# nktoan/h-edit

Hardware: AMD Instinct MI355X
Metric: edited images/sec (512^2, 50 steps, K Langevin) (higher is better)
Workload: dtype bf16

## Files before the change

h-edit_amd/csrc/c_api.hip:

```cpp
#include "../../include/hedit.h"
#include <exception>
#include <map>
#include <mutex>
#include <new>
#include <set>
#include <utility>

#include "common.h"
#include "kernels.h"

static thread_local std::string g_last_error;
void hedit_set_error(const std::string& msg) { g_last_error = msg; }

int hedit_abi_catch() noexcept {
  try {
    try {
      throw;
    } catch (const std::bad_alloc&) {
      g_last_error = "out of host memory inside libhedit_hip";
    } catch (const std::exception& e) {
      g_last_error = std::string("C++ exception inside libhedit_hip: ") + e.what();
    } catch (...) {
      g_last_error = "unknown C++ exception inside libhedit_hip";
    }
// ... 133 lines not shown
int hedit_k_gemm_plan_splits(int M, int N, int K, int chunk_kt) { return gemm_plan_splits(M, N, K, chunk_kt); }

int hedit_k_gemm(const void* A, const void* W, const float* bias, const void* residual, void* C, int M, int N,
                 int K, int lda, int ldc, int ldr, int mode, int Hin, int Win, int Cin, int Hout, int Wout,
                 int splits, void* partial_ws, void* stream) try {
  ARG_CHECK(A && W && C, "gemm args");
  GemmParams p{};
  p.A = reinterpret_cast<const bf16_t*>(A);
  p.W = reinterpret_cast<const bf16_t*>(W);
  p.M = M; p.N = N; p.K = K; p.lda = lda; p.mode = mode;
  p.Hin = Hin; p.Win = Win; p.Cin = Cin; p.Hout = Hout; p.Wout = Wout;
  p.bias = bias;
  p.residual = reinterpret_cast<const bf16_t*>(residual);
  p.ldr = ldr;
  p.C = reinterpret_cast<bf16_t*>(C);
  p.ldc = ldc;
  if (splits < 0) {
    const int kt = K / 64;
    const int s = gemm_pick_splits(M, N, K, -splits);
    p.chunk_kt = (kt + s - 1) / s;
    return gemm_launch(p, 1, nullptr, S(stream));
  }
  const int s = gemm_pick_splits(M, N, K, splits);
  return gemm_launch(p, s, reinterpret_cast<float*>(partial_ws), S(stream));
} catch (...) { return hedit_abi_catch(); }

int hedit_k_conv_gn(const void* A, const void* W, const float* bias, const void* residual, void* C, int M, int N, int K, int ldc,
                    int ldr, int mode, int Hin, int Win, int Cin, int Hout, int Wout, int splits, void* partial_ws, float* gn_part,
                    void* stream) try {
  ARG_CHECK(A && W && C && gn_part, "conv_gn args");
  GemmParams p{};
  p.A = reinterpret_cast<const bf16_t*>(A);
  p.W = reinterpret_cast<const bf16_t*>(W);
  p.M = M; p.N = N; p.K = K; p.lda = Cin; p.mode = mode;
  p.Hin = Hin; p.Win = Win; p.Cin = Cin; p.Hout = Hout; p.Wout = Wout;
  p.bias = bias;
  p.residual = reinterpret_cast<const bf16_t*>(residual);
  p.ldr = ldr;
  p.C = reinterpret_cast<bf16_t*>(C);
  p.ldc = ldc;
  p.gn_part = gn_part;
  if (splits < 0) {
    const int kt = K / 64;
    const int s = gemm_pick_splits(M, N, K, -splits);
    p.chunk_kt = (kt + s - 1) / s;
    return gemm_launch(p, 1, nullptr, S(stream));
  }
  const int s = gemm_pick_splits(M, N, K, splits);
  return gemm_launch(p, s, reinterpret_cast<float*>(partial_ws), S(stream));
} catch (...) { return hedit_abi_catch(); }

int hedit_k_groupnorm_from_parts(const void* x, void* y, const float* gamma, const float* beta, int B, int HW, int C, int G,
                                 float eps, int silu, const float* part_a, int ca, const float* part_b, int cb, void* ws,
                                 void* stream) try {
  ARG_CHECK(x && y && gamma && beta && part_a && ws, "groupnorm_from_parts args");
  return groupnorm_from_parts_launch(reinterpret_cast<const bf16_t*>(x), reinterpret_cast<bf16_t*>(y), gamma, beta, B, HW, C, G,
                                     eps, silu, part_a, ca, part_b, cb, reinterpret_cast<float*>(ws), S(stream));
} catch (...) { return hedit_abi_catch(); }

int hedit_k_pack_geglu(const float* w, const float* bias, void* w_packed_bf16, float* bias_packed, int inner, int K,
                       void* stream) try {
  ARG_CHECK(w && w_packed_bf16, "pack_geglu args");
  int rc = pack_geglu_rows_launch(w, reinterpret_cast<bf16_t*>(w_packed_bf16), nullptr, 2 * inner, K, S(stream));
  if (rc != HEDIT_OK || !bias) return rc;
  ARG_CHECK(bias_packed, "pack_geglu: bias_packed");
  return pack_geglu_rows_launch(bias, nullptr, bias_packed, 2 * inner, 1, S(stream));
} catch (...) { return hedit_abi_catch(); }

int hedit_k_gemm_geglu(const void* A, const void* w_packed, const float* bias_packed, void* C, int M, int inner, int K,
                       int lda, int ldc, void* stream) try {
  ARG_CHECK(A && w_packed && C, "gemm_geglu args");
  GemmParams p{};
  p.A = reinterpret_cast<const bf16_t*>(A);
  p.W = reinterpret_cast<const bf16_t*>(w_packed);
  p.M = M; p.N = 2 * inner; p.K = K; p.lda = lda; p.mode = 0;
  p.bias = bias_packed;
  p.C = reinterpret_cast<bf16_t*>(C);
  p.ldc = ldc;
  p.geglu = 1;
  return gemm_launch(p, 1, nullptr, S(stream));
} catch (...) { return hedit_abi_catch(); }

int hedit_k_ffn_channels(void) { return ffn_fused_channels(); }
size_t hedit_k_ffn_stream_bytes(int with_outer_layers) { return ffn_stream_bytes(with_outer_layers, with_outer_layers); }
size_t hedit_k_ffn_bias_bytes(void) { return ffn_bias_bytes(); }

int hedit_k_ffn_pack(const float* w1, const float* b1, const float* w2, const float* w_pre, const float* w_post, void* stream_out,
                     float* bias1_out, void* stream) try {
  ARG_CHECK(w1 && b1 && w2 && stream_out && bias1_out && ((w_pre == nullptr) == (w_post == nullptr)), "ffn_pack args");
  const int outer = w_pre != nullptr;
  bf16_t* so = reinterpret_cast<bf16_t*>(stream_out);
  int rc = ffn_pack_launch(w1, 1, outer, outer, so, S(stream));
  if (rc == HEDIT_OK) rc = ffn_pack_launch(w2, 2, outer, outer, so, S(stream));
  if (rc == HEDIT_OK && outer) rc = ffn_pack_launch(w_pre, 0, 1, 1, so, S(stream));
  if (rc == HEDIT_OK && outer) rc = ffn_pack_launch(w_post, 3, 1, 1, so, S(stream));
  if (rc != HEDIT_OK) return rc;
  return ffn_pack_bias_launch(b1, bias1_out, S(stream));
} catch (...) { return hedit_abi_catch(); }

int hedit_k_ffn_fused(const void* x, int64_t ldx, const float* gamma, const float* beta, float eps, const void* w_stream,
                      const float* bias1_packed, const float* bias2, void* out, int64_t ldo, int M, int C, void* stream) try {
  FfnParams f{};
  f.x = reinterpret_cast<const bf16_t*>(x); f.ldx = (long)ldx; f.gamma = gamma; f.beta = beta; f.eps = eps;
  f.stream = reinterpret_cast<const bf16_t*>(w_stream); f.bias1p = bias1_packed; f.bias2 = bias2;
  f.out = reinterpret_cast<bf16_t*>(out); f.ldo = (long)ldo; f.M = M; f.C = C;
  return ffn_fused_launch(f, S(stream));
} catch (...) { return hedit_abi_catch(); }

int hedit_k_ffn_chain(const void* a, int64_t lda, const void* t1, int64_t ldt1, const void* x, int64_t ldx, const float* bias_pre,
                      const float* gamma, const float* beta, float eps, const void* w_stream, const float* bias1_packed, const float* bias2,
                      const float* bias_post, void* out, int64_t ldo, int M, int C, void* stream) try {
  ARG_CHECK(a && t1 && x, "ffn_chain args");
  FfnParams f{};
  f.a = reinterpret_cast<const bf16_t*>(a); f.lda = (long)lda;
  f.x = reinterpret_cast<const bf16_t*>(t1); f.ldx = (long)ldt1;
  f.r2 = reinterpret_cast<const bf16_t*>(x); f.ldr2 = (long)ldx;
  f.bias_pre = bias_pre; f.bias_post = bias_post;
  f.gamma = gamma; f.beta = beta; f.eps = eps;
  f.stream = reinterpret_cast<const bf16_t*>(w_stream); f.bias1p = bias1_packed; f.bias2 = bias2;
  f.out = reinterpret_cast<bf16_t*>(out); f.ldo = (long)ldo; f.M = M; f.C = C;
  return ffn_fused_launch(f, S(stream));
} catch (...) { return hedit_abi_catch(); }

size_t hedit_k_lin_chain_stream_bytes(int n_out) { return lin_chain_stream_bytes(n_out == 3 ? 4 : 2); }

int hedit_k_lin_chain_pack(const float* w_pre, const float* w0, const float* w1, const float* w2, float scale0, void* stream_out,
                           void* stream) try {
  ARG_CHECK(w_pre && w0 && stream_out && ((w1 == nullptr) == (w2 == nullptr)), "lin_chain_pack args");
  const int layers = w1 ? 4 : 2;
  bf16_t* so = reinterpret_cast<bf16_t*>(stream_out);
  int rc = lin_chain_pack_launch(w_pre, 0, 1.f, layers, so, S(stream));
  if (rc == HEDIT_OK) rc = lin_chain_pack_launch(w0, 1, scale0, layers, so, S(stream));
  if (rc == HEDIT_OK && w1) rc = lin_chain_pack_launch(w1, 2, 1.f, layers, so, S(stream));
  if (rc == HEDIT_OK && w1) rc = lin_chain_pack_launch(w2, 3, 1.f, layers, so, S(stream));
  return rc;
} catch (...) { return hedit_abi_catch(); }

int hedit_k_lin_chain(const void* a, int64_t lda, const void* r1, int64_t ldr1, const float* gn_ss, int rows_per_image,
                      const float* bias_pre, const float* gamma, const float* beta, float eps, const void* w_stream, void* out_mid,
                      int64_t ldmid, void* out_q, int64_t ldq, void* out_k, int64_t ldk, void* out, int64_t ldo, int M, int C,
                      void* stream) try {
  LinChainParams c{};
  c.a = reinterpret_cast<const bf16_t*>(a); c.lda = (long)lda; c.r1 = reinterpret_cast<const bf16_t*>(r1); c.ldr1 = (long)ldr1;
  c.bias_pre = bias_pre; c.gamma = gamma; c.beta = beta; c.eps = eps; c.stream = reinterpret_cast<const bf16_t*>(w_stream);
  c.out_mid = reinterpret_cast<bf16_t*>(out_mid); c.ldmid = (long)ldmid; c.out = reinterpret_cast<bf16_t*>(out); c.ldo = (long)ldo;
  c.M = M; c.C = C; c.gn_ss = gn_ss; c.rows_per_image = rows_per_image;
  c.out_q = reinterpret_cast<bf16_t*>(out_q); c.ldq = (long)ldq; c.out_k = reinterpret_cast<bf16_t*>(out_k); c.ldk = (long)ldk;
  return lin_chain_launch(c, S(stream));
} catch (...) { return hedit_abi_catch(); }

int hedit_storage_is_f16(void) { return HEDIT_F16; }

int hedit_test_set_flags(int flags) try {
  ARG_CHECK(flags >= 0 && flags <= 15, "hedit_test_set_flags: bit 0 drained ring waits, bit 1 exact self-attention pass, bit 2 pixel-UNet GroupNorm statistics path flipped, bit 3 no persistent linear kernel");
  g_test_flags.store(flags, std::memory_order_relaxed);
  return HEDIT_OK;
} catch (...) { return hedit_abi_catch(); }

int hedit_k_lin_chain_sched(const void* a, int64_t lda, const void* r1, int64_t ldr1, const float* gn_ss, int rows_per_image,
                            const float* bias_pre, const float* gamma, const float* beta, float eps, const void* w_stream, void* out_mid,
                            int64_t ldmid, void* out_q, int64_t ldq, void* out_k, int64_t ldk, void* out, int64_t ldo, int M, int C,
                            int sched, void* stream) try {
  LinChainParams c{};
  c.a = reinterpret_cast<const bf16_t*>(a); c.lda = (long)lda; c.r1 = reinterpret_cast<const bf16_t*>(r1); c.ldr1 = (long)ldr1;
  c.bias_pre = bias_pre; c.gamma = gamma; c.beta = beta; c.eps = eps; c.stream = reinterpret_cast<const bf16_t*>(w_stream);
  c.out_mid = reinterpret_cast<bf16_t*>(out_mid); c.ldmid = (long)ldmid; c.out = reinterpret_cast<bf16_t*>(out); c.ldo = (long)ldo;
  c.M = M; c.C = C; c.gn_ss = gn_ss; c.rows_per_image = rows_per_image;
  c.out_q = reinterpret_cast<bf16_t*>(out_q); c.ldq = (long)ldq; c.out_k = reinterpret_cast<bf16_t*>(out_k); c.ldk = (long)ldk;
  return lin_chain_launch_sched(c, sched, S(stream));
} catch (...) { return hedit_abi_catch(); }

size_t hedit_k_groupnorm_ws_bytes(int B, int HW, int C) { return groupnorm_ws_bytes(B, HW, C); }

int hedit_k_groupnorm_affine(const void* x, const float* gamma, const float* beta, int B, int HW, int C, int G, float eps, void* ws,
                             float* ss_out, void* stream) try {
  ARG_CHECK(x && gamma && beta && ws && ss_out, "groupnorm_affine args");
  const float* ss = nullptr;
  int rc = groupnorm_affine_launch(reinterpret_cast<const bf16_t*>(x), gamma, beta, B, HW, C, G, eps, reinterpret_cast<float*>(ws), S(stream), &ss);
  if (rc != HEDIT_OK) return rc;
  HIP_TRY(hipMemcpyAsync(ss_out, ss, (size_t)B * C * 2 * sizeof(float), hipMemcpyDeviceToDevice, S(stream)));
  return HEDIT_OK;
} catch (...) { return hedit_abi_catch(); }

int hedit_k_groupnorm(const void* x, void* y, const float* gamma, const float* beta, int B, int HW, int C, int G,
                      float eps, int silu, void* ws, void* stream) try {
  ARG_CHECK(x && y && gamma && beta && ws, "groupnorm args");
  return groupnorm_launch(reinterpret_cast<const bf16_t*>(x), reinterpret_cast<bf16_t*>(y), gamma, beta, B, HW, C, G,
                          eps, silu, reinterpret_cast<float*>(ws), S(stream));
} catch (...) { return hedit_abi_catch(); }

int hedit_k_layernorm(const void* x, void* y, const float* gamma, const float* beta, int64_t rows, int C, float eps,
                      void* stream) try {
  ARG_CHECK(x && y && gamma && beta, "layernorm args");
  return layernorm_launch(reinterpret_cast<const bf16_t*>(x), reinterpret_cast<bf16_t*>(y), gamma, beta, (long)rows, C, eps, S(stream));
} catch (...) { return hedit_abi_catch(); }

int hedit_k_geglu(const void* x, void* y, int64_t rows, int inner, void* stream) try {
  ARG_CHECK(x && y, "geglu args");
  return geglu_launch(reinterpret_cast<const bf16_t*>(x), reinterpret_cast<bf16_t*>(y), (long)rows, inner, S(stream));
} catch (...) { return hedit_abi_catch(); }

int hedit_k_self_attn(const void* q, int ldq, const void* k, int ldk, const void* vt, int64_t ldvt, void* out, int ldo,
                      int B, int N, int heads, int d, const int32_t* qk_src, const int32_t* kv_src, void* stream) try {
  ARG_CHECK(q && k && vt && out, "self_attn args");
  SelfAttnParams p{};
  p.q = reinterpret_cast<const bf16_t*>(q); p.ldq = ldq;
  p.k = reinterpret_cast<const bf16_t*>(k); p.ldk = ldk;
  p.vt = reinterpret_cast<const bf16_t*>(vt); p.ldvt = (long)ldvt;
  p.out = reinterpret_cast<bf16_t*>(out); p.ldo = ldo;
  p.B = B; p.N = N; p.heads = heads; p.d = d; p.qk_src = qk_src; p.kv_src = kv_src;
  return self_attn_launch(p, S(stream));
} catch (...) { return hedit_abi_catch(); }

int hedit_k_cross_attn(const void* q, int ldq, const void* k, int ldk, const void* vt, int64_t ldvt, void* out, int ldo,
                       int B, int N, int heads, int d, const hedit_p2p_plan* plan, float* store, void* stream) try {
  ARG_CHECK(q && k && vt && out && plan, "cross_attn args");
  CrossAttnParams p{};
  p.q = reinterpret_cast<const bf16_t*>(q); p.ldq = ldq;
  p.k = reinterpret_cast<const bf16_t*>(k); p.ldk = ldk;
  p.vt = reinterpret_cast<const bf16_t*>(vt); p.ldvt = (long)ldvt;
  p.out = reinterpret_cast<bf16_t*>(out); p.ldo = ldo;
  p.B = B; p.N = N; p.heads = heads; p.d = d;
  p.n_pairs = plan->n_pairs; p.pair_src = plan->pair_src; p.pair_tar = plan->pair_tar;
  p.mixT = reinterpret_cast<const bf16_t*>(plan->mixT); p.bvec = plan->bvec;
  p.singles = plan->singles; p.n_single = plan->n_single;
  p.store = store;
  return cross_attn_launch(p, S(stream));
} catch (...) { return hedit_abi_catch(); }

int hedit_k_attn_probs(const void* q, int ldq, const void* k, int ldk, float* probs, int B, int N, int M, int kstride,
                       int heads, int d, void* stream) try {
  ARG_CHECK(q && k && probs, "attn_probs args");
  AttnProbsParams p{};
  p.q = reinterpret_cast<const bf16_t*>(q); p.ldq = ldq;
  p.k = reinterpret_cast<const bf16_t*>(k); p.ldk = ldk;
  p.probs = probs; p.B = B; p.N = N; p.M = M; p.kstride = kstride; p.heads = heads; p.d = d;
  return attn_probs_launch(p, S(stream));
} catch (...) { return hedit_abi_catch(); }

int hedit_k_attn_apply(const float* probs, const void* vt, int64_t ldvt, void* out, int ldo, int B, int N, int M,
                       int kstride, int heads, int d, void* stream) try {
  ARG_CHECK(probs && vt && out, "attn_apply args");
  AttnProbsParams p{};
  p.probs = const_cast<float*>(probs);
  p.vt = reinterpret_cast<const bf16_t*>(vt); p.ldvt = (long)ldvt;
  p.out = reinterpret_cast<bf16_t*>(out); p.ldo = ldo;
  p.B = B; p.N = N; p.M = M; p.kstride = kstride; p.heads = heads; p.d = d;
  return attn_apply_launch(p, S(stream));
} catch (...) { return hedit_abi_catch(); }

int hedit_k_pack_conv3x3(const float* w, void* out, int O, int I, void* stream) try {
  ARG_CHECK(w && out, "pack args");
  return pack_conv3x3_launch(w, reinterpret_cast<bf16_t*>(out), O, I, S(stream));
} catch (...) { return hedit_abi_catch(); }

int hedit_k_f32_to_bf16(const float* x, void* y, int64_t n, void* stream) try {
  ARG_CHECK(x && y, "cast args");
  return f32_to_bf16_launch(x, reinterpret_cast<bf16_t*>(y), (long)n, S(stream));
} catch (...) { return hedit_abi_catch(); }

int hedit_k_groupnorm_stats(const void* x, void* y, const float* gamma, const float* beta, int B, int HW, int C, int G,
                            float eps, int silu, void* ws, float* stats, void* stream) try {
  ARG_CHECK(x && y && gamma && beta && ws && stats, "groupnorm_stats args");
  return groupnorm_launch(reinterpret_cast<const bf16_t*>(x), reinterpret_cast<bf16_t*>(y), gamma, beta, B, HW, C, G,
                          eps, silu, reinterpret_cast<float*>(ws), S(stream), stats);
} catch (...) { return hedit_abi_catch(); }

size_t hedit_k_groupnorm_bwd_ws_bytes(int B, int HW, int C) { return groupnorm_bwd_ws_bytes(B, HW, C); }

int hedit_k_groupnorm_bwd(const void* x, const void* dy, const void* add, void* dx, const float* gamma, const float* beta,
                          const float* stats, int B, int HW, int C, int G, int silu, void* ws, void* stream) try {
  ARG_CHECK(x && dy && dx && gamma && beta && stats && ws, "groupnorm_bwd args");
  return groupnorm_bwd_launch(reinterpret_cast<const bf16_t*>(x), reinterpret_cast<const bf16_t*>(dy),
                              reinterpret_cast<const bf16_t*>(add), reinterpret_cast<bf16_t*>(dx), gamma, beta, stats, B, HW, C,
                              G, silu, reinterpret_cast<float*>(ws), S(stream));
} catch (...) { return hedit_abi_catch(); }

int hedit_k_softmax_rows(const float* s, void* p, int64_t rows, int N, float scale, void* stream) try {
  ARG_CHECK(s && p, "softmax_rows args");
  return softmax_rows_launch(s, reinterpret_cast<bf16_t*>(p), (long)rows, N, scale, S(stream));
} catch (...) { return hedit_abi_catch(); }

int hedit_k_softmax_blockdiag(const float* s, void* p, int64_t rows, int T, int ld, float scale, void* stream) try {
  ARG_CHECK(s && p, "softmax_blockdiag args");
  return softmax_blockdiag_launch(s, reinterpret_cast<bf16_t*>(p), (long)rows, T, ld, scale, S(stream));
} catch (...) { return hedit_abi_catch(); }

int hedit_k_softmax_bwd(const void* p, const float* dp, void* ds, int64_t rows, int N, float scale, void* stream) try {
  ARG_CHECK(p && dp && ds, "softmax_bwd args");
  return softmax_bwd_launch(reinterpret_cast<const bf16_t*>(p), dp, reinterpret_cast<bf16_t*>(ds), (long)rows, N, scale, S(stream));
} catch (...) { return hedit_abi_catch(); }

int hedit_k_transpose(const void* src, void* dst, int R, int C, void* stream) try {
  ARG_CHECK(src && dst, "transpose args");
  return transpose_bf16_launch(reinterpret_cast<const bf16_t*>(src), reinterpret_cast<bf16_t*>(dst), R, C, S(stream));
} catch (...) { return hedit_abi_catch(); }

int hedit_k_sum2x2(const void* du, void* dx, int B, int H, int W, int C, void* stream) try {
  ARG_CHECK(du && dx, "sum2x2 args");
  return sum2x2_launch(reinterpret_cast<const bf16_t*>(du), reinterpret_cast<bf16_t*>(dx), B, H, W, C, S(stream));
} catch (...) { return hedit_abi_catch(); }

int hedit_k_pack_conv3x3_dgrad(const float* w, void* out, int O, int I, void* stream) try {
  ARG_CHECK(w && out, "pack args");
  return pack_conv3x3_dgrad_launch(w, reinterpret_cast<bf16_t*>(out), O, I, S(stream));
} catch (...) { return hedit_abi_catch(); }

// ... 110 lines not shown
```

h-edit_amd/csrc/norm.hip:

```cpp
#include <stdlib.h>
#include "common.h"
#include "kernels.h"

namespace {


constexpr int GN_MAXV = 2;

__global__ __launch_bounds__(256) void gn_partial_kernel(const bf16_t* __restrict__ x, float* __restrict__ part,
                                                         int HW, int C, int G, int nslab) {
  extern __shared__ float lds[];
  const int CV = C / 8;
  const int slab = blockIdx.x, b = blockIdx.y;
  const int pix_per = (HW + nslab - 1) / nslab;
  const int p0 = slab * pix_per;
  int p1 = p0 + pix_per;
  if (p1 > HW) p1 = HW;
  const int R = CV <= 256 ? 256 / CV : 1;
  const int r = CV <= 256 ? threadIdx.x / CV : 0;
  const int cv0 = CV <= 256 ? threadIdx.x % CV : threadIdx.x;
  const bool active = r < R;
  float s[GN_MAXV][8], q[GN_MAXV][8];
#pragma unroll
  for (int v = 0; v < GN_MAXV; ++v)
// ... 407 lines not shown

__global__ __launch_bounds__(256) void pack_conv3x3_kernel(const float* __restrict__ w, bf16_t* __restrict__ out, int O, int I) {
  const long total = (long)O * 9 * I;
  for (long idx = (long)blockIdx.x * 256 + threadIdx.x; idx < total; idx += (long)gridDim.x * 256) {
    const int i = (int)(idx % I);
    const long t = idx / I;
    const int tap = (int)(t % 9);
    const int o = (int)(t / 9);
    out[idx] = f32_to_bf16(w[((long)o * I + i) * 9 + tap]);
  }
}

__global__ __launch_bounds__(256) void pack_geglu_rows_kernel(const float* __restrict__ w, bf16_t* __restrict__ ob, float* __restrict__ of,
                                                              int rows, int K) {
  const long total = (long)rows * K;
  const int half = rows / 2;
  for (long idx = (long)blockIdx.x * 256 + threadIdx.x; idx < total; idx += (long)gridDim.x * 256) {
    const int k = (int)(idx % K);
    const int r = (int)(idx / K);
    const int t = r >> 5, u = r & 31;
    const int src = u < 16 ? t * 16 + u : half + t * 16 + (u - 16);
    const float v = w[(long)src * K + k];
    if (ob) ob[idx] = f32_to_bf16(v);
    if (of) of[idx] = v;
  }
}

__global__ __launch_bounds__(256) void gemv_kernel(const bf16_t* __restrict__ W, const float* __restrict__ x, const float* __restrict__ b0,
                                                   const float* __restrict__ b1, float* __restrict__ out, int N, int K, int silu) {
  const int lane = threadIdx.x & 63;
  const int n = blockIdx.x * 4 + (threadIdx.x >> 6);
  if (n >= N) return;
  float acc = 0.f;
  for (int k = lane * 8; k < K; k += 512) {
    uint4 u = *reinterpret_cast<const uint4*>(W + (long)n * K + k);
    float w[8];
    unpack8(u, w);
#pragma unroll
    for (int j = 0; j < 8; ++j) {
      float xv = x[k + j];
      if (silu) xv = silu_f(xv);
      acc += w[j] * xv;
    }
  }
  acc = wave_sum(acc);
  if (lane == 0) out[n] = acc + (b0 ? b0[n] : 0.f) + (b1 ? b1[n] : 0.f);
}

__global__ void timestep_embed_kernel(float t, float* out, int dim) {
  const int half = dim / 2;
  for (int i = threadIdx.x; i < half; i += blockDim.x) {
    const float fr = expf(-9.210340371976184f * (float)i / (float)half);
    const float a = t * fr;
    out[i] = cosf(a);
    out[half + i] = sinf(a);
  }
}

__global__ void timestep_embed_ddpm_kernel(float t, float* out, int dim) {
  const int half = dim / 2;
  for (int i = threadIdx.x; i < half; i += blockDim.x) {
    const float fr = expf(-9.210340371976184f / (float)(half - 1) * (float)i);
    const float a = t * fr;
    out[i] = sinf(a);
    out[half + i] = cosf(a);
  }
  if ((dim & 1) && threadIdx.x == 0) out[dim - 1] = 0.f;
}

constexpr int CI_PIX = 128;
__global__ __launch_bounds__(256) void conv_in_kernel(const float* __restrict__ x, const float* __restrict__ w, const float* __restrict__ bias,
                                                      bf16_t* __restrict__ y, int B, int Cin, int H, int Wd, int Cout) {
  extern __shared__ float lds[];
  const int K = Cin * 9;
  float* sw = lds;
  float* sx = lds + (long)K * Cout;
  for (int i = threadIdx.x; i < K * Cout; i += 256) {
    const int co = i / K, k = i - co * K;
    sw[k * Cout + co] = w[i];
  }
  const long pix0 = (long)blockIdx.x * CI_PIX;
  const long npix = (long)B * H * Wd;
  for (int i = threadIdx.x; i < CI_PIX * K; i += 256) {
    const int k = i / CI_PIX, pl = i - k * CI_PIX;
    const long pix = pix0 + pl;
    float v = 0.f;
    if (pix < npix) {
      const int ox = (int)(pix % Wd), oy = (int)((pix / Wd) % H), b = (int)(pix / ((long)Wd * H));
      const int ci = k / 9, tap = k - ci * 9;
      const int iy = oy + tap / 3 - 1, ix = ox + tap % 3 - 1;
      if ((unsigned)iy < (unsigned)H && (unsigned)ix < (unsigned)Wd) v = x[(((long)b * Cin + ci) * H + iy) * Wd + ix];
    }
    sx[k * CI_PIX + pl] = v;
  }
  __syncthreads();
  const int CV = Cout / 8;
  for (int i = threadIdx.x; i < (CI_PIX / 4) * CV; i += 256) {
    const int pg = i / CV, cv = i - pg * CV;
    float acc[4][8];
#pragma unroll
    for (int q = 0; q < 4; ++q)
#pragma unroll
      for (int j = 0; j < 8; ++j) acc[q][j] = bias[cv * 8 + j];
    for (int k = 0; k < K; ++k) {
      const float4 xv = *reinterpret_cast<const float4*>(sx + k * CI_PIX + pg * 4);
      const float4 w0 = *reinterpret_cast<const float4*>(sw + k * Cout + cv * 8);
      const float4 w1 = *reinterpret_cast<const float4*>(sw + k * Cout + cv * 8 + 4);
      const float xq[4] = {xv.x, xv.y, xv.z, xv.w};
#pragma unroll
      for (int q = 0; q < 4; ++q) {
        acc[q][0] += xq[q] * w0.x; acc[q][1] += xq[q] * w0.y; acc[q][2] += xq[q] * w0.z; acc[q][3] += xq[q] * w0.w;
        acc[q][4] += xq[q] * w1.x; acc[q][5] += xq[q] * w1.y; acc[q][6] += xq[q] * w1.z; acc[q][7] += xq[q] * w1.w;
      }
    }
#pragma unroll
    for (int q = 0; q < 4; ++q) {
      const long pix = pix0 + pg * 4 + q;
      if (pix < npix) *reinterpret_cast<uint4*>(y + pix * Cout + cv * 8) = pack8(acc[q]);
    }
  }
}

__global__ __launch_bounds__(256) void conv_out_kernel(const bf16_t* __restrict__ x, const bf16_t* __restrict__ w, const float* __restrict__ bias,
                                                       float* __restrict__ y, int B, int H, int Wd, int C, int Cout) {
  const int lane = threadIdx.x & 63;
  const long pix = (long)blockIdx.x * 4 + (threadIdx.x >> 6);
  if (pix >= (long)B * H * Wd) return;
  const int ox = (int)(pix % Wd);
  const int oy = (int)((pix / Wd) % H);
  const int b = (int)(pix / ((long)Wd * H));
  const int CV = C / 8;
  float acc[4] = {0.f, 0.f, 0.f, 0.f};
  for (int idx = lane; idx < 9 * CV; idx += 64) {
    const int tap = idx / CV, cv = idx - tap * CV;
    const int iy = oy + tap / 3 - 1, ix = ox + tap % 3 - 1;
    if ((unsigned)iy >= (unsigned)H || (unsigned)ix >= (unsigned)Wd) continue;
    uint4 u = *reinterpret_cast<const uint4*>(x + (((long)b * H + iy) * Wd + ix) * C + cv * 8);
    float f[8];
    unpack8(u, f);
    for (int co = 0; co < Cout; ++co) {
      uint4 uw = *reinterpret_cast<const uint4*>(w + ((long)co * 9 + tap) * C + cv * 8);
      float ww[8];
      unpack8(uw, ww);
#pragma unroll
      for (int j = 0; j < 8; ++j) acc[co] += f[j] * ww[j];
    }
  }
  for (int co = 0; co < Cout; ++co) {
    float v = wave_sum(acc[co]);
    if (lane == 0) y[(((long)b * Cout + co) * H + oy) * Wd + ox] = v + bias[co];
  }
}

__global__ __launch_bounds__(256) void gn_small_kernel(const bf16_t* __restrict__ x, bf16_t* __restrict__ y,
                                                       const float* __restrict__ gamma, const float* __restrict__ beta,
                                                       int HW, int C, int G, float eps, int silu, float* __restrict__ stats) {
  extern __shared__ uint32_t gs_pairs[];
  __shared__ float red[8];
  const int g = blockIdx.x, b = blockIdx.y, tid = threadIdx.x;
  const int cpg = C / G, ppp = cpg / 2;
  const int npair = HW * ppp;
  const uint32_t* xin = reinterpret_cast<const uint32_t*>(x + (long)b * HW * C + g * cpg);
  float s = 0.f, q = 0.f;
  for (int i = tid; i < npair; i += 256) {
    const int pix = i / ppp, j = i - pix * ppp;
    const uint32_t u = xin[(long)pix * (C / 2) + j];
    gs_pairs[i] = u;
    const float a = st_lo(u), c = st_hi(u);
    s += a; s += c;
    q += a * a; q += c * c;
  }
  s = wave_sum(s);
  q = wave_sum(q);
  if ((tid & 63) == 0) { red[(tid >> 6) * 2] = s; red[(tid >> 6) * 2 + 1] = q; }
  __syncthreads();
  s = ((red[0] + red[2]) + red[4]) + red[6];
  q = ((red[1] + red[3]) + red[5]) + red[7];
  const float n = (float)HW * (float)cpg;
  const float m = s / n;
  float var = q / n - m * m;
  var = var < 0.f ? 0.f : var;
  const float rstd = rsqrtf(var + eps);
  if (stats && tid == 0) *reinterpret_cast<float2*>(stats + ((long)b * G + g) * 2) = make_float2(m, rstd);
  uint32_t* yout = reinterpret_cast<uint32_t*>(y + (long)b * HW * C + g * cpg);
  for (int i = tid; i < npair; i += 256) {
    const int pix = i / ppp, j = i - pix * ppp;
    const uint32_t u = gs_pairs[i];
    const int c0 = g * cpg + 2 * j;
    const float sc0 = rstd * gamma[c0], sc1 = rstd * gamma[c0 + 1];
    float a = st_lo(u) * sc0 + (beta[c0] - m * sc0);
    float c = st_hi(u) * sc1 + (beta[c0 + 1] - m * sc1);
    if (silu) { a = silu_f(a); c = silu_f(c); }
    yout[(long)pix * (C / 2) + j] = pack_bf16x2(a, c);
  }
}

__global__ __launch_bounds__(256) void gn_fold_kernel(const float* __restrict__ pa, int npa, const float* __restrict__ pb, int npb,
                                                      float* __restrict__ out, int units, int ppg) {
  __shared__ float red[8];
  const int g = blockIdx.x, b = blockIdx.y, tid = threadIdx.x;
  const int total = units * ppg;
  float s = 0.f, q = 0.f;
  for (int e = tid; e < total; e += 256) {
    const int u = e / ppg, j = e - u * ppg;
    const int pr = g * ppg + j;
    const long row = (long)b * units + u;
    const float2 v = pr < npa ? *reinterpret_cast<const float2*>(pa + (row * npa + pr) * 2)
                              : *reinterpret_cast<const float2*>(pb + (row * npb + (pr - npa)) * 2);
    s += v.x;
    q += v.y;
  }
  s = wave_sum(s);
  q = wave_sum(q);
  if ((tid & 63) == 0) { red[(tid >> 6) * 2] = s; red[(tid >> 6) * 2 + 1] = q; }
  __syncthreads();
  if (tid == 0) {
    s = ((red[0] + red[2]) + red[4]) + red[6];
    q = ((red[1] + red[3]) + red[5]) + red[7];
    *reinterpret_cast<float2*>(out + ((long)b * gridDim.x + g) * 2) = make_float2(s, q);
  }
}

int gn_nslab(int B, int HW, int C) {
  (void)B;
  const int CV = C / 8;
  const int R = CV <= 256 ? 256 / CV : 1;
  int n = HW / (R * 8);
  int cap = HW / 256;
  cap = cap < 32 ? 32 : (cap > 64 ? 64 : cap);
  if (HW >= 512 * 512) cap = 128;
  if (n > cap) n = cap;
  if (n < 1) n = 1;
  return n;
}

}

size_t groupnorm_ws_bytes(int B, int HW, int C) {
  const int nslab = gn_nslab(B, HW, C);
  return ((size_t)B * nslab * 64 * 2 + (size_t)B * C * 2) * sizeof(float);
}

int groupnorm_launch(const bf16_t* x, bf16_t* y, const float* gamma, const float* beta, int B, int HW,
                     int C, int G, float eps, int silu, float* ws, hipStream_t st, float* stats) {
  ARG_CHECK(C % 8 == 0 && C % G == 0 && G <= 64, "groupnorm: C % 8, C % G, G <= 64");
  ARG_CHECK(C / 8 <= 256 * GN_MAXV, "groupnorm: C too large");
  if (HW < 1024 && (C / G) % 2 == 0 && (size_t)HW * (C / G) * 2 <= 60 * 1024) {
    hipLaunchKernelGGL(gn_small_kernel, dim3(G, B), dim3(256), (size_t)HW * (C / G) * 2, st, x, y, gamma, beta, HW, C, G, eps, silu, stats);
    LAUNCH_CHECK();
    return HEDIT_OK;
  }
  const int nslab = gn_nslab(B, HW, C);
  float* part = ws;
  float* ss = ws + (size_t)B * nslab * 64 * 2;
  const int CV = C / 8;
  const int R = CV <= 256 ? 256 / CV : 1;
  const size_t lds = (size_t)R * C * 2 * sizeof(float);
  ARG_CHECK(lds <= 64 * 1024, "groupnorm: LDS");
  hipLaunchKernelGGL(gn_partial_kernel, dim3(nslab, B), dim3(256), lds, st, x, part, HW, C, G, nslab);
  LAUNCH_CHECK();
  const long total_v = (long)B * HW * CV;
  const bool rows_form = CV <= 256 && HW >= 1024;
  if (!rows_form || stats) {
    hipLaunchKernelGGL(gn_finalize_kernel, dim3(B), dim3(256), 0, st, part, gamma, beta, ss, HW, C, G, nslab, eps, stats);
    LAUNCH_CHECK();
  }
  if (rows_form) {
    int ns = (int)(4096 / (B > 0 ? B : 1)) + 1;
    const int max_ns = HW / (R * 8) > 0 ? HW / (R * 8) : 1;
    if (ns > max_ns) ns = max_ns;
    {
      int pix = HW / ns / (4 * R) * (4 * R);
      if (pix < 4 * R) pix = 4 * R;
      ns = (HW + pix - 1) / pix;
    }
    hipLaunchKernelGGL(gn_apply_rows_kernel, dim3(ns, B), dim3(256), 0, st, x, y, part, gamma, beta, HW, C, G, nslab, eps, silu, ns);
    LAUNCH_CHECK();
    return HEDIT_OK;
  }
  hipLaunchKernelGGL(gn_apply_kernel, dim3(ew_grid(total_v)), dim3(256), 0, st, x, y, ss, total_v, HW, C, silu);
  LAUNCH_CHECK();
  return HEDIT_OK;
}

bool groupnorm_from_parts_supported(int HW, int C, int G) {
  return HW >= 1024 && HW % 128 == 0 && C % 8 == 0 && C / 8 <= 256 && C % G == 0 && (C / G) % 2 == 0 && G <= 64;
}
size_t groupnorm_from_parts_ws_bytes(int B) { return (size_t)B * 64 * 2 * sizeof(float); }

int groupnorm_from_parts_launch(const bf16_t* x, bf16_t* y, const float* gamma, const float* beta, int B, int HW, int C, int G,
                                float eps, int silu, const float* part_a, int ca, const float* part_b, int cb, float* ws,
                                hipStream_t st) {
  ARG_CHECK(groupnorm_from_parts_supported(HW, C, G), "groupnorm_from_parts: shape");
  ARG_CHECK(part_a && ca > 0 && ca % 2 == 0 && cb >= 0 && cb % 2 == 0 && ca + cb == C && (cb == 0) == (part_b == nullptr),
            "groupnorm_from_parts: the pair statistics must cover the C channels");
  hipLaunchKernelGGL(gn_fold_kernel, dim3(G, B), dim3(256), 0, st, part_a, ca / 2, part_b, cb / 2, ws, HW / 128, C / G / 2);
  LAUNCH_CHECK();
  const int CV = C / 8, R = 256 / CV;
  int ns = (int)(4096 / (B > 0 ? B : 1)) + 1;
  const int max_ns = HW / (R * 8) > 0 ? HW / (R * 8) : 1;
  if (ns > max_ns) ns = max_ns;
  int pix = HW / ns / (4 * R) * (4 * R);
  if (pix < 4 * R) pix = 4 * R;
  ns = (HW + pix - 1) / pix;
  hipLaunchKernelGGL(gn_apply_rows_kernel, dim3(ns, B), dim3(256), 0, st, x, y, ws, gamma, beta, HW, C, G, 1, eps, silu, ns);
  LAUNCH_CHECK();
  return HEDIT_OK;
}

int groupnorm_affine_launch(const bf16_t* x, const float* gamma, const float* beta, int B, int HW, int C, int G, float eps,
                            float* ws, hipStream_t st, const float** ss_out) {
  ARG_CHECK(C % 8 == 0 && C % G == 0 && G <= 64, "groupnorm: C % 8, C % G, G <= 64");
  ARG_CHECK(C / 8 <= 256 * GN_MAXV, "groupnorm: C too large");
  const int nslab = gn_nslab(B, HW, C);
  float* part = ws;
  float* ss = ws + (size_t)B * nslab * 64 * 2;
  const int CV = C / 8;
  const int R = CV <= 256 ? 256 / CV : 1;
  const size_t lds = (size_t)R * C * 2 * sizeof(float);
  ARG_CHECK(lds <= 64 * 1024, "groupnorm: LDS");
  hipLaunchKernelGGL(gn_partial_kernel, dim3(nslab, B), dim3(256), lds, st, x, part, HW, C, G, nslab);
  LAUNCH_CHECK();
  hipLaunchKernelGGL(gn_finalize_kernel, dim3(B), dim3(256), 0, st, part, gamma, beta, ss, HW, C, G, nslab, eps, (float*)nullptr);
  LAUNCH_CHECK();
  *ss_out = ss;
  return HEDIT_OK;
}

static int ln_narrow_lanes(int C) {
  if (C % 64 == 0 && C / 64 <= LNN_MAXV) return 8;
  if (C % 128 == 0 && C / 128 <= LNN_MAXV) return 16;
  if (C % 256 == 0 && C / 256 <= LNN_MAXV) return 32;
  return 0;
}

bool splitk_reduce_ln_supported(int C) { return C % 8 == 0 && ln_narrow_lanes(C) != 0; }

int splitk_reduce_ln_launch(const float* partial, int splits, const float* bias, const bf16_t* residual, int ldr, bf16_t* out,
                            bf16_t* y, const float* gamma, const float* beta, long rows, int C, float eps, hipStream_t st) {
  const int lanes = ln_narrow_lanes(C);
  ARG_CHECK(lanes != 0 && splits >= 1, "splitk_reduce_ln: unsupported row width");
  const LnReduce rd{partial, splits, bias, residual, ldr};
  if (lanes == 8) hipLaunchKernelGGL((layernorm_narrow_kernel<8, true>), dim3(cdiv(rows, 32)), dim3(256), 0, st, out, y, gamma, beta, rows, C, eps, rd);
  else if (lanes == 16) hipLaunchKernelGGL((layernorm_narrow_kernel<16, true>), dim3(cdiv(rows, 16)), dim3(256), 0, st, out, y, gamma, beta, rows, C, eps, rd);
  else hipLaunchKernelGGL((layernorm_narrow_kernel<32, true>), dim3(cdiv(rows, 8)), dim3(256), 0, st, out, y, gamma, beta, rows, C, eps, rd);
  LAUNCH_CHECK();
  return HEDIT_OK;
}

int layernorm_launch(const bf16_t* x, bf16_t* y, const float* gamma, const float* beta, long rows, int C,
                     float eps, hipStream_t st) {
  ARG_CHECK(C % 8 == 0 && C / 8 <= 64 * LN_MAXV, "layernorm: C");
  const LnReduce none{};
  bf16_t* xx = const_cast<bf16_t*>(x);
  switch (ln_narrow_lanes(C)) {
    case 8:
      hipLaunchKernelGGL((layernorm_narrow_kernel<8, false>), dim3(cdiv(rows, 32)), dim3(256), 0, st, xx, y, gamma, beta, rows, C, eps, none);
      LAUNCH_CHECK();
      return HEDIT_OK;
    case 16:
      hipLaunchKernelGGL((layernorm_narrow_kernel<16, false>), dim3(cdiv(rows, 16)), dim3(256), 0, st, xx, y, gamma, beta, rows, C, eps, none);
      LAUNCH_CHECK();
      return HEDIT_OK;
    case 32:
      hipLaunchKernelGGL((layernorm_narrow_kernel<32, false>), dim3(cdiv(rows, 8)), dim3(256), 0, st, xx, y, gamma, beta, rows, C, eps, none);
      LAUNCH_CHECK();
      return HEDIT_OK;
    default: break;
  }
  hipLaunchKernelGGL(layernorm_kernel, dim3(cdiv(rows, 4)), dim3(256), 0, st, x, y, gamma, beta, rows, C, eps);
  LAUNCH_CHECK();
  return HEDIT_OK;
}

int geglu_launch(const bf16_t* x, bf16_t* y, long rows, int inner, hipStream_t st) {
  ARG_CHECK(inner % 8 == 0, "geglu: inner % 8");
  hipLaunchKernelGGL(geglu_kernel, dim3(ew_grid(rows * (inner / 8))), dim3(256), 0, st, x, y, rows, inner);
  LAUNCH_CHECK();
  return HEDIT_OK;
}

int concat_launch(const bf16_t* a, int ca, const bf16_t* b, int cb, bf16_t* y, long rows, hipStream_t st, const RowMap* b_map,
                  int rows_per_image) {
  ARG_CHECK(ca % 8 == 0 && cb % 8 == 0, "concat: channels % 8");
  if (b_map) {
    ARG_CHECK(rows_per_image > 0 && rows % rows_per_image == 0 && rows / rows_per_image <= HEDIT_ROWMAP_MAX, "concat: row map");
    hipLaunchKernelGGL(concat_mapped_kernel, dim3(ew_grid(rows * (((a ? ca : 0) + cb) / 8))), dim3(256), 0, st, a, ca, b, cb, y, rows,
                       rows_per_image, *b_map);
    LAUNCH_CHECK();
    return HEDIT_OK;
  }
  if (a == nullptr) {
    hipLaunchKernelGGL(concat_right_kernel, dim3(ew_grid(rows * (cb / 8))), dim3(256), 0, st, b, ca, cb, y, rows);
    LAUNCH_CHECK();
    return HEDIT_OK;
  }
  hipLaunchKernelGGL(concat_kernel, dim3(ew_grid(rows * ((ca + cb) / 8))), dim3(256), 0, st, a, ca, b, cb, y, rows);
  LAUNCH_CHECK();
  return HEDIT_OK;
}

// ... 241 lines not shown
```

h-edit_amd/csrc/unet.hip:

```cpp
#include <array>
#include <map>
#include <string>
#include <vector>

#include "exec.h"
#include "kernels.h"
#include "store.h"

namespace {

struct Res {
  int cin, cout, temb_off;
  float *n1g, *n1b, *n2g, *n2b, *conv2_b, *sc_b;
  bf16_t *conv1, *conv2, *sc_w;
  bf16_t *conv1_t = nullptr, *conv2_t = nullptr, *sc_t = nullptr;
};

struct Attn {
  int C;
  float *gn_g, *gn_b, *pin_b, *ln1g, *ln1b, *ln2g, *ln2b, *ln3g, *ln3b, *o1_b, *o2_b, *ff1_b, *ff2_b, *pout_b;
  bf16_t *pin, *w_qk, *w_v1, *w_o1, *w_q2, *w_k2, *w_v2, *w_o2, *ff1, *ff2, *pout;
  bf16_t *frs = nullptr, *k1s = nullptr, *ffs = nullptr;
  float* ff1_bp = nullptr;
  int ctx_off = 0;
// ... 425 lines not shown
      f.store_self_idx++;
    }
  }
  f.ar.free(qk);
  f.ar.free(vt);
  TRY(aalloc(f, &t1, M * C));
  TRY(aalloc(f, &q2, M * C));
  if (chain) {
    LinChainParams lc{};
    lc.a = ao; lc.lda = C; lc.r1 = t0; lc.ldr1 = C; lc.bias_pre = a.o1_b;
    lc.gamma = a.ln2g; lc.beta = a.ln2b; lc.eps = 1e-5f; lc.stream = a.k1s;
    lc.out_mid = t1; lc.ldmid = C; lc.out = q2; lc.ldo = C; lc.M = (int)M; lc.C = C;
    ProfScope ps(f, PK_LINEAR, 2.0 * M * 2.0 * C * C, 8.0 * M * C + 4.0 * C * C);
    chain_prof(f, ps, M, C, 2, 130);
    RUN(f, lin_chain_launch(lc, f.st));
  } else {
    TRY(aalloc(f, &tn, M * C));
    TRY(linear_ln(f, ao, (int)M, C, a.w_o1, C, a.o1_b, t0, t1, a.ln2g, a.ln2b, 1e-5f, tn));
    TRY(linear(f, tn, (int)M, C, a.w_q2, C, nullptr, nullptr, q2, C));
    f.ar.free(tn);
  }
  f.ar.free(ao);
  f.ar.free(t0);
  *t1_out = t1;
  *q2_out = q2;
  return HEDIT_OK;
}

int transformer_rest(Fwd& f, const Attn& a, const bf16_t* x, bf16_t* t1, bf16_t* q2, int H, int W, bf16_t** out,
                     bf16_t* dst = nullptr, int ldd = 0) {
  const int C = a.C, N = H * W, B = f.B, heads = f.h->cfg.heads, d = C / heads;
  const size_t M = (size_t)B * N;
  const hedit_p2p_plan* pl = (f.plan && f.plan->mode > 0) ? f.plan : nullptr;
  bf16_t *tn, *ao, *k2, *vt2, *t2, *gf, *t3, *y;
  const bool chain = a.ffs != nullptr;
  const int MC = B * HEDIT_CTXP;
  k2 = const_cast<bf16_t*>(f.k2_all) + a.ctx_off;
  vt2 = const_cast<bf16_t*>(f.vt2_all) + (size_t)a.ctx_off * MC;
  const int ldk2 = f.h->ctx_n;
  TRY(aalloc(f, &ao, M * C));
  {
    CrossAttnParams cp{};
    cp.q = q2; cp.ldq = C; cp.k = k2; cp.ldk = ldk2; cp.vt = vt2; cp.ldvt = MC; cp.out = ao; cp.ldo = C;
    cp.B = B; cp.N = N; cp.heads = heads; cp.d = d;
    const bool stored_layer = N <= 1024;
    if (pl) {
      cp.n_pairs = pl->n_pairs; cp.pair_src = pl->pair_src; cp.pair_tar = pl->pair_tar;
      cp.mixT = reinterpret_cast<const bf16_t*>(pl->mixT); cp.bvec = pl->bvec;
      cp.singles = pl->singles; cp.n_single = pl->n_single;
      cp.store = (pl->mode == 2 && stored_layer && pl->h_store && f.store_idx < pl->n_store) ? pl->h_store[f.store_idx] : nullptr;
    } else {
      cp.n_pairs = 0; cp.singles = f.h->iota; cp.n_single = B;
    }
    if (stored_layer) f.store_idx++;
    if (f.h->hook) {
      TRY(hooked_attention(f, cp.q, cp.ldq, cp.k, cp.ldk, cp.vt, cp.ldvt, ao, C, N, HEDIT_MAXW, HEDIT_CTXP, heads, d, 1));
    } else {
      ProfScope ps(f, PK_CROSS_ATTN, 4.0 * B * (double)N * HEDIT_MAXW * C, 4.0 * M * C + 4.0 * MC * C);
      RUN(f, cross_attn_launch(cp, f.st));
    }
  }
  f.ar.free(q2);
  if (chain) {
    if (dst) {
      y = dst;
    } else {
      TRY(aalloc(f, &y, M * C));
    }
    FfnParams fp{};
    fp.a = ao; fp.lda = C; fp.x = t1; fp.ldx = C; fp.r2 = x; fp.ldr2 = C;
    fp.bias_pre = a.o2_b; fp.bias_post = a.pout_b;
    fp.gamma = a.ln3g; fp.beta = a.ln3b; fp.eps = 1e-5f;
    fp.stream = a.ffs; fp.bias1p = a.ff1_bp; fp.bias2 = a.ff2_b; fp.out = y; fp.ldo = dst ? ldd : C; fp.M = (int)M; fp.C = C;
    {
      ProfScope ps(f, PK_LINEAR, 2.0 * M * 14.0 * C * C, 8.0 * M * C + 28.0 * C * C);
      chain_prof(f, ps, M, C, 14, 128);
      RUN(f, ffn_fused_launch(fp, f.st));
    }
    f.ar.free(ao);
    f.ar.free(t1);
    *out = y;
    return HEDIT_OK;
  }
  TRY(aalloc(f, &t2, M * C));
  TRY(aalloc(f, &tn, M * C));
  TRY(linear_ln(f, ao, (int)M, C, a.w_o2, C, a.o2_b, t1, t2, a.ln3g, a.ln3b, 1e-5f, tn));
  f.ar.free(ao);
  f.ar.free(t1);
  TRY(aalloc(f, &gf, M * 4 * C));
  {
    GemmParams gp{};
    gp.A = tn; gp.W = a.ff1; gp.M = (int)M; gp.N = 8 * C; gp.K = C; gp.lda = C; gp.mode = 0;
    gp.bias = a.ff1_b; gp.residual = nullptr; gp.ldr = 0; gp.C = gf; gp.ldc = 4 * C; gp.geglu = 1;
    ProfScope ps(f, PK_LINEAR, 2.0 * gp.M * gp.N * gp.K, gemm_alg_bytes(f, gp));
    RUN(f, gemm_launch(gp, 1, nullptr, f.st));
  }
  f.ar.free(tn);
  TRY(aalloc(f, &t3, M * C));
  TRY(linear(f, gf, (int)M, 4 * C, a.ff2, C, a.ff2_b, t2, t3, C));
  f.ar.free(gf);
  f.ar.free(t2);

  if (dst) {
    y = dst;
  } else {
    TRY(aalloc(f, &y, M * C));
  }
  TRY(linear(f, t3, (int)M, C, a.pout, C, a.pout_b, x, y, dst ? ldd : C));
  f.ar.free(t3);
  *out = y;
  return HEDIT_OK;
}

int transformer(Fwd& f, const Attn& a, const bf16_t* x, int H, int W, bf16_t** out, bf16_t* dst = nullptr, int ldd = 0) {
  bf16_t *t1, *q2;
  TRY(transformer_stem(f, a, x, H, W, &t1, &q2));
  return transformer_rest(f, a, x, t1, q2, H, W, out, dst, ldd);
}

struct Skip { bf16_t* p; int C; bool per_latent = false; };

bool stem_shareable(const hedit_unet* h, const hedit_p2p_plan* plan, int D, int B, int N0) {
  if (D >= B || h->hook || h->down.empty() || !h->down[0].has_attn) return false;
  const hedit_p2p_plan* pl = (plan && plan->mode > 0) ? plan : nullptr;
  if (!pl) return true;
  if (pl->feat_src && pl->feat_resblock <= 0) return false;
  if (pl->kv_src && pl->kv_first_block <= 0) return false;
  if (pl->qk_src && N0 <= (pl->qk_max_tokens > 0 ? pl->qk_max_tokens : 1024) && pl->qk_first_block <= 0) return false;
  if (pl->mode == 2 && pl->h_store_self && pl->n_store_self > 0 && N0 <= 1024) return false;
  return true;
}

int broadcast_stem(Fwd& f, size_t row_elems, bf16_t** x, bf16_t** t1, bf16_t** q2, int D) {
  bf16_t** narrow[3] = {x, t1, q2};
  bf16_t* wide[3];
  const void* src[3];
  void* dst[3];
  for (int i = 0; i < 3; ++i) {
    TRY(aalloc(f, &wide[i], (size_t)f.B * row_elems));
    src[i] = *narrow[i];
    dst[i] = wide[i];
  }
  {
    ProfScope ps(f, PK_OTHER, 0.0, 3.0 * (D + f.B) * (double)row_elems * sizeof(bf16_t));
    RUN(f, gather_rows_launch(src, dst, 3, f.B, (long)(row_elems * sizeof(bf16_t)), *f.map, f.st));
  }
  for (int i = 0; i < 3; ++i) {
    f.ar.free(*narrow[i]);
    *narrow[i] = wide[i];
  }
  return HEDIT_OK;
}

int forward_impl(hedit_unet* h, const float* x, float t, const float* ctx, int B, int H0, int W0,
                 const hedit_p2p_plan* plan, float* eps_out, void* ws, size_t ws_bytes, hipStream_t st,
                 bool dry, size_t* peak, int D = 0, const RowMap* map = nullptr) {
  const hedit_unet_cfg& c = h->cfg;
  Fwd f;
  f.h = h; f.B = B; f.st = st; f.plan = plan; f.map = map;
  f.ar.base = reinterpret_cast<char*>(ws); f.ar.cap = ws_bytes; f.ar.dry = dry;
  const int ch0 = c.block_out_channels[0];

  if (!dry && h->iota_cap < B) {
    hedit_set_error("batch larger than " + std::to_string(h->iota_cap) + " rows");
    return HEDIT_ERR_ARG;
  }

  bf16_t* ctxb;
  TRY(aalloc(f, &ctxb, (size_t)B * HEDIT_CTXP * c.cross_attention_dim));
  RUN(f, ctx_pad_launch(ctx, ctxb, B, c.cross_attention_dim, st));
  f.ctxb = ctxb;
  {
    const int MC = B * HEDIT_CTXP;
    bf16_t *k2a, *vt2a;
    TRY(aalloc(f, &k2a, (size_t)MC * h->ctx_n));
    TRY(aalloc(f, &vt2a, (size_t)MC * h->ctx_n));
    TRY(linear(f, ctxb, MC, c.cross_attention_dim, h->wk2_all, h->ctx_n, nullptr, nullptr, k2a, h->ctx_n));
    TRY(linear(f, h->wv2_all, h->ctx_n, c.cross_attention_dim, ctxb, MC, nullptr, nullptr, vt2a, MC, 2));
    f.k2_all = k2a;
    f.vt2_all = vt2a;
  }

  float *te0, *te1, *te2, *temb_all;
  TRY(aalloc(f, &te0, (size_t)ch0));
  TRY(aalloc(f, &te1, (size_t)h->temb_dim));
  TRY(aalloc(f, &te2, (size_t)h->temb_dim));
  TRY(aalloc(f, &temb_all, (size_t)h->temb_total));
  RUN(f, timestep_embed_launch(t, te0, ch0, st));
  RUN(f, gemv_launch(h->te1_w, te0, h->te1_b, nullptr, te1, h->temb_dim, ch0, 0, st));
  RUN(f, gemv_launch(h->te2_w, te1, h->te2_b, nullptr, te2, h->temb_dim, h->temb_dim, 1, st));
  RUN(f, gemv_launch(h->temb_w_all, te2, h->temb_b_all, h->conv1_b_all, temb_all, h->temb_total, h->temb_dim, 1, st));
  f.temb_all = temb_all;

  int H = H0, W = W0;
  const bool share = D > 0 && stem_shareable(h, plan, D, B, H0 * W0);
  float* xrows = nullptr;
  if (D > 0 && !share) {
    const size_t img = (size_t)c.in_channels * H * W;
    TRY(aalloc(f, &xrows, (size_t)B * img));
    const void* src[1] = {x};
    void* dst[1] = {xrows};
    ProfScope ps(f, PK_OTHER, 0.0, (double)(D + B) * img * sizeof(float));
    RUN(f, gather_rows_launch(src, dst, 1, B, (long)(img * sizeof(float)), *map, st));
    x = xrows;
  }
  bf16_t* cur;
  {
    BatchScope rows(f, share ? D : B);
    TRY(aalloc(f, &cur, (size_t)f.B * H * W * ch0));
    RUN(f, conv_in_launch(x, h->conv_in_w, h->conv_in_b, cur, f.B, c.in_channels, H, W, ch0, st));
  }
  if (xrows) f.ar.free(xrows);
  std::vector<Skip> skips;
  skips.push_back({cur, ch0, share});

  for (int i = 0; i < c.n_levels; ++i) {
    Block& blk = h->down[i];
    for (size_t j = 0; j < blk.res.size(); ++j) {
      const bool stem = share && i == 0 && j == 0;
      bf16_t *y, *t1 = nullptr, *q2 = nullptr;
      {
        BatchScope rows(f, stem ? D : B);
        TRY(resblock(f, blk.res[j], cur, H, W, &y));
        if (blk.has_attn) {
          f.place = 0;
          TRY(transformer_stem(f, blk.attn[j], y, H, W, &t1, &q2));
        }
      }
      cur = y;
      if (stem) TRY(broadcast_stem(f, (size_t)H * W * blk.ch, &cur, &t1, &q2, D));
      if (blk.has_attn) {
        bf16_t* z;
        TRY(transformer_rest(f, blk.attn[j], cur, t1, q2, H, W, &z));
        f.ar.free(cur);
        cur = z;
      }
      skips.push_back({cur, blk.ch});
    }
    if (blk.has_sampler) {
      bf16_t* y;
      TRY(aalloc(f, &y, (size_t)B * (H / 2) * (W / 2) * blk.ch));
      TRY(conv3x3(f, cur, H, W, blk.ch, blk.samp_w, blk.ch, blk.samp_b, nullptr, y, 2));
      H /= 2; W /= 2;
      cur = y;
      skips.push_back({cur, blk.ch});
    }
  }

  {
    bf16_t *y, *z, *w;
    TRY(resblock(f, h->mid_res[0], cur, H, W, &y));
    f.place = 1;
    TRY(transformer(f, h->mid_attn, y, H, W, &z));
    f.ar.free(y);
    TRY(resblock(f, h->mid_res[1], z, H, W, &w));
    f.ar.free(z);
    cur = w;
  }
  int cur_c = c.block_out_channels[c.n_levels - 1];

  bool in_cat = false;
  bf16_t* cat_next = nullptr;
  for (int i = 0; i < c.n_levels; ++i) {
    Block& blk = h->up[i];
    for (size_t j = 0; j < blk.res.size(); ++j) {
      Skip s = skips.back();
      skips.pop_back();
      bf16_t* cat;
      const size_t M = (size_t)B * H * W;
      if (in_cat) {
        cat = cat_next;
        { ProfScope ps(f, PK_OTHER, 0.0); RUN(f, concat_launch(nullptr, cur_c, s.p, s.C, cat, (long)M, st, s.per_latent ? f.map : nullptr, H * W)); }
      } else {
        TRY(aalloc(f, &cat, M * (cur_c + s.C)));
        { ProfScope ps(f, PK_OTHER, 0.0); RUN(f, concat_launch(cur, cur_c, s.p, s.C, cat, (long)M, st, s.per_latent ? f.map : nullptr, H * W)); }
        f.ar.free(cur);
      }
      f.ar.free(s.p);
      const bool last_res = j + 1 == blk.res.size();
      const bool to_cat = !last_res;
      bf16_t* dst = nullptr;
      int ldd = 0;
      if (to_cat) {
        ldd = blk.ch + skips.back().C;
        TRY(aalloc(f, &dst, M * ldd));
      }
      bf16_t* y;
      if (blk.has_attn) {
        TRY(resblock(f, blk.res[j], cat, H, W, &y));
        f.ar.free(cat);
        bf16_t* z;
        f.place = 2;
        TRY(transformer(f, blk.attn[j], y, H, W, &z, dst, ldd));
        f.ar.free(y);
        cur = z;
      } else {
        TRY(resblock(f, blk.res[j], cat, H, W, &y, dst, ldd));
        f.ar.free(cat);
        cur = y;
      }
      cur_c = blk.ch;
      in_cat = to_cat;
      cat_next = dst;
    }
    if (blk.has_sampler) {
      const size_t M4 = (size_t)B * H * W * 4;
      const int ldd = blk.ch + skips.back().C;
      bf16_t* dst;
      TRY(aalloc(f, &dst, M4 * ldd));
      TRY(conv3x3(f, cur, H, W, blk.ch, blk.samp_w, blk.ch, blk.samp_b, nullptr, dst, 3, ldd));
      f.ar.free(cur);
      H *= 2; W *= 2;
      cur = dst;
      in_cat = true;
      cat_next = dst;
    }
  }

  {
    bf16_t* a;
    TRY(aalloc(f, &a, (size_t)B * H * W * ch0));
    TRY(groupnorm(f, cur, a, h->gn_out_g, h->gn_out_b, H * W, ch0, 1e-5f, 1));
    if (c.out_channels != 4 || ch0 % 64 != 0) {
      RUN(f, conv_out_launch(a, h->conv_out_w, h->conv_out_b, eps_out, B, H, W, ch0, c.out_channels, st));
    } else {
      float* prod;
      const size_t M = (size_t)B * H * W;
      TRY(aalloc(f, &prod, M * 4));
      GemmParams p{};
      p.mode = 1; p.Hin = H; p.Win = W; p.Cin = ch0; p.Hout = H; p.Wout = W;
      p.A = a; p.W = h->conv_out_w; p.M = (int)M; p.N = 4; p.K = 9 * ch0; p.lda = ch0; p.raw_f32 = prod; p.ldc = 4;
      TRY(run_gemm(f, p));
      RUN(f, rows_to_nchw_launch(prod, h->conv_out_b, eps_out, B, (long)H * W, 4, 4, st));
// ... 25 lines not shown
    ARG_CHECK(cfg->block_out_channels[i] % 64 == 0, "block_out_channels % 64");
    ARG_CHECK(cfg->block_out_channels[i] % cfg->norm_num_groups == 0, "channels % groups");
    const int d = cfg->block_out_channels[i] / cfg->heads;
    ARG_CHECK(d == 32 || d == 40 || d == 64 || d == 80 || d == 160, "head dim must be one of 32,40,64,80,160");
  }
  TRY(gemm_prepare());
  if (grad) ARG_CHECK(cfg->in_channels <= 4, "the input-gradient pass needs in_channels <= 4");
  hedit_unet* h = new hedit_unet();
  h->cfg = *cfg;
  h->grad = grad;
  const int* ch = cfg->block_out_channels;
  const int L = cfg->layers_per_block, n = cfg->n_levels;
  h->temb_dim = ch[0] * 4;

  int total = 0;
  {
    int outc = ch[0];
    for (int i = 0; i < n; ++i) { outc = ch[i]; total += L * outc; }
    total += 2 * ch[n - 1];
    for (int i = 0; i < n; ++i) total += (L + 1) * ch[n - 1 - i];
  }
  h->temb_total = total;
  h->temb_w_all = dalloc<bf16_t>(h, (size_t)total * h->temb_dim);
  h->temb_b_all = dalloc<float>(h, total);
  h->conv1_b_all = dalloc<float>(h, total);

  h->conv_in_w = f32conv(h, "conv_in.weight", ch[0], cfg->in_channels, 3);
  if (grad) {
    h->conv_in_t = twin<bf16_t>(h, Pack::Conv3Dgrad, (size_t)4 * 9 * ch[0]);
    if (h->conv_in_t && hipMemset(h->conv_in_t, 0, (size_t)4 * 9 * ch[0] * sizeof(bf16_t)) != hipSuccess) h->alloc_failed = true;
  }
  h->conv_in_b = vec(h, "conv_in.bias", ch[0]);
  h->te1_w = lin(h, "time_embedding.linear_1.weight", h->temb_dim, ch[0]);
  h->te1_b = vec(h, "time_embedding.linear_1.bias", h->temb_dim);
  h->te2_w = lin(h, "time_embedding.linear_2.weight", h->temb_dim, h->temb_dim);
  h->te2_b = vec(h, "time_embedding.linear_2.bias", h->temb_dim);

  for (int i = 0; i < n; ++i) {
    if (cfg->down_has_attn[i]) h->ctx_n += L * ch[i];
    if (cfg->up_has_attn[i]) h->ctx_n += (L + 1) * ch[n - 1 - i];
  }
  h->ctx_n += ch[n - 1];
  h->wk2_all = dalloc<bf16_t>(h, (size_t)h->ctx_n * cfg->cross_attention_dim);
  h->wv2_all = dalloc<bf16_t>(h, (size_t)h->ctx_n * cfg->cross_attention_dim);
  if (ctx) h->wkv2_t = dalloc<bf16_t>(h, (size_t)2 * h->ctx_n * cfg->cross_attention_dim);

  int toff = 0;
  int outc = ch[0];
  for (int i = 0; i < n; ++i) {
    const int inc = outc;
    outc = ch[i];
    Block b;
    b.ch = outc;
    b.has_attn = cfg->down_has_attn[i] != 0;
    const std::string pre = "down_blocks." + std::to_string(i);
    for (int j = 0; j < L; ++j) {
      b.res.push_back(make_res(h, pre + ".resnets." + std::to_string(j), j == 0 ? inc : outc, outc, toff));
      if (b.has_attn) b.attn.push_back(make_attn(h, pre + ".attentions." + std::to_string(j), outc));
    }
    if (i != n - 1) {
      b.has_sampler = true;
      b.samp_w = conv3(h, pre + ".downsamplers.0.conv.weight", outc, outc);
      if (grad) b.samp_t = twin<bf16_t>(h, Pack::Conv3S2Dgrad, (size_t)outc * outc * 9);
      b.samp_b = vec(h, pre + ".downsamplers.0.conv.bias", outc);
    }
    h->down.push_back(b);
  }
  h->mid_attn = make_attn(h, "mid_block.attentions.0", ch[n - 1]);
  h->mid_res[0] = make_res(h, "mid_block.resnets.0", ch[n - 1], ch[n - 1], toff);
  h->mid_res[1] = make_res(h, "mid_block.resnets.1", ch[n - 1], ch[n - 1], toff);
  outc = ch[n - 1];
  for (int i = 0; i < n; ++i) {
    const int prev = outc;
    outc = ch[n - 1 - i];
    const int inp = ch[n - 1 - (i + 1 < n ? i + 1 : n - 1)];
    Block b;
    b.ch = outc;
    b.has_attn = cfg->up_has_attn[i] != 0;
    const std::string pre = "up_blocks." + std::to_string(i);
    for (int j = 0; j < L + 1; ++j) {
      const int skip = j == L ? inp : outc;
      const int rin = j == 0 ? prev : outc;
      b.res.push_back(make_res(h, pre + ".resnets." + std::to_string(j), rin + skip, outc, toff));
      if (b.has_attn) b.attn.push_back(make_attn(h, pre + ".attentions." + std::to_string(j), outc));
    }
    if (i != n - 1) {
      b.has_sampler = true;
      b.samp_w = conv3(h, pre + ".upsamplers.0.conv.weight", outc, outc);
      if (grad) b.samp_t = twin<bf16_t>(h, Pack::Conv3Dgrad, (size_t)outc * outc * 9);
      b.samp_b = vec(h, pre + ".upsamplers.0.conv.bias", outc);
    }
    h->up.push_back(b);
  }
  h->gn_out_g = vec(h, "conv_norm_out.weight", ch[0]);
  h->gn_out_b = vec(h, "conv_norm_out.bias", ch[0]);
  h->conv_out_w = conv3(h, "conv_out.weight", cfg->out_channels, ch[0]);
  if (grad) {
    h->conv_out_t = twin<float>(h, Pack::FlipOIHW, (size_t)cfg->out_channels * ch[0] * 9);
    h->zero_bias = dalloc<float>(h, ch[0]);
    if (h->zero_bias && hipMemset(h->zero_bias, 0, ch[0] * sizeof(float)) != hipSuccess) h->alloc_failed = true;
  }
  h->conv_out_b = vec(h, "conv_out.bias", cfg->out_channels);

  {
    constexpr int IOTA = 16384;
    std::vector<int32_t> v(IOTA);
    for (int i = 0; i < IOTA; ++i) v[i] = i;
    h->iota = dalloc<int32_t>(h, IOTA);
    if (h->iota && hipMemcpy(h->iota, v.data(), IOTA * sizeof(int32_t), hipMemcpyHostToDevice) != hipSuccess) h->alloc_failed = true;
    h->iota_cap = IOTA;
  }
  if (h->ctx_next != h->ctx_n || toff != total) {
    hedit_set_error(h->ctx_next != h->ctx_n ? "internal: stacked context-projection plan mismatch" : "internal: time-embedding plan mismatch");
    hedit_unet_destroy(h);
    return HEDIT_ERR_STATE;
  }
  return handle_created(h, out);
}

extern "C" {

int hedit_unet_create(const hedit_unet_cfg* cfg, hedit_unet** out) try {
  return create_impl(cfg, out, false);
} catch (...) { return hedit_abi_catch(); }

int hedit_unet_create_grad(const hedit_unet_cfg* cfg, hedit_unet** out) try {
  return create_impl(cfg, out, true);
} catch (...) { return hedit_abi_catch(); }

int hedit_unet_create_grad_ctx(const hedit_unet_cfg* cfg, hedit_unet** out) try {
  return create_impl(cfg, out, true, true);
} catch (...) { return hedit_abi_catch(); }

int hedit_unet_param_bf16_exact(const hedit_unet* h, int i) try {
  return store_param_bf16_exact(h, i);
} catch (...) { (void)hedit_abi_catch(); return 0; }

size_t hedit_unet_workspace_bytes(hedit_unet* h, int B, int height, int width) try {
  if (!h) return 0;
  const std::array<int, 4> key{B, height, width, h->hook ? 1 : 0};
  auto it = h->ws_cache.find(key);
  if (it != h->ws_cache.end()) return it->second;
  size_t need = 0;
  for (int D = 0; D <= (B <= HEDIT_ROWMAP_MAX ? B : 0); ++D) {
    size_t peak = 0;
    if (forward_impl(h, nullptr, 0.f, nullptr, B, height, width, nullptr, nullptr, nullptr, 0, nullptr, true, &peak, D) != HEDIT_OK) return 0;
    if (peak > need) need = peak;
  }
  need += 4096;
  h->ws_cache[key] = need;
  return need;
} catch (...) { (void)hedit_abi_catch(); return 0; }

static int forward_checks(hedit_unet* h, const float* x, const float* ctx, int B, int height, int width, const hedit_p2p_plan* plan,
                          float* eps_out, void* workspace) {
  ARG_CHECK(h && x && ctx && eps_out && workspace, "null");
  ARG_CHECK(B >= 1, "B");
  const int div = 1 << (h->cfg.n_levels - 1);
  ARG_CHECK(height % div == 0 && width % div == 0, "latent size must be divisible by 2^(levels-1)");
  const int lowest = (height / div) * (width / div);
  ARG_CHECK(lowest % 64 == 0, "lowest-resolution level must have a multiple of 64 tokens");
  TRY(store_require_loaded(h, "UNet"));
  ARG_CHECK(!(h->hook && plan && plan->mode > 0), "an attention hook excludes the in-kernel edits of a plan (pass plan = NULL)");
  if (plan && plan->mode > 0) {
    ARG_CHECK(plan->n_pairs >= 0 && plan->n_pairs + plan->n_single > 0, "plan rows");
    ARG_CHECK(plan->n_pairs == 0 || (plan->pair_src && plan->pair_tar && plan->mixT && plan->bvec), "plan tables");
  }
  return HEDIT_OK;
}

int hedit_unet_forward(hedit_unet* h, const float* x, float t, const float* ctx, int B, int height, int width,
                       const hedit_p2p_plan* plan, float* eps_out, void* workspace, size_t workspace_bytes,
                       void* stream) try {
  TRY(forward_checks(h, x, ctx, B, height, width, plan, eps_out, workspace));
  return forward_impl(h, x, t, ctx, B, height, width, plan, eps_out, workspace, workspace_bytes,
                      reinterpret_cast<hipStream_t>(stream), false, nullptr);
} catch (...) { return hedit_abi_catch(); }

int hedit_unet_forward_shared(hedit_unet* h, const float* x, int D, const int* row_latent, float t, const float* ctx, int B,
                              int height, int width, const hedit_p2p_plan* plan, float* eps_out, void* workspace,
                              size_t workspace_bytes, void* stream) try {
  TRY(forward_checks(h, x, ctx, B, height, width, plan, eps_out, workspace));
  ARG_CHECK(row_latent && D >= 1 && D <= 65535, "row map");
  if (B > HEDIT_ROWMAP_MAX) {
    hedit_set_error("batch larger than " + std::to_string(HEDIT_ROWMAP_MAX) + " rows (the row map of shared latents)");
    return HEDIT_ERR_ARG;
  }
  ARG_CHECK(reinterpret_cast<uintptr_t>(x) % 16 == 0, "x must be 16-byte aligned");
  RowMap map{};
  for (int r = 0; r < B; ++r) {
    ARG_CHECK(row_latent[r] >= 0 && row_latent[r] < D, "row_latent entries must lie in [0, D)");
    map.src[r] = (uint16_t)row_latent[r];
  }
  return forward_impl(h, x, t, ctx, B, height, width, plan, eps_out, workspace, workspace_bytes,
                      reinterpret_cast<hipStream_t>(stream), false, nullptr, D, &map);
} catch (...) { return hedit_abi_catch(); }

size_t hedit_unet_grad_workspace_bytes(hedit_unet* h, int B, int height, int width) try {
  if (!h || !h->grad || check_grad_shape(h, B, height, width) != HEDIT_OK) return 0;
  GradTape T;
  tape_init(T, h, B, height, width, nullptr, 0, nullptr, true);
  float dummy = 0.f;
  int rc = forward_keep_impl(h, T, nullptr, 0.f, nullptr, nullptr);
  if (rc == HEDIT_OK) rc = backward_impl(h, T, &dummy, &dummy);
  if (h->wkv2_t) {
    if (rc == HEDIT_OK) rc = backward_impl(h, T, &dummy, &dummy, &dummy);
    if (rc == HEDIT_OK) rc = backward_impl(h, T, &dummy, nullptr, &dummy);
  }
  return dry_run_bytes(rc, T.f.ar.peak);
} catch (...) { (void)hedit_abi_catch(); return 0; }

int hedit_unet_forward_keep(hedit_unet* h, const float* x, float t, const float* ctx, int B, int height, int width, float* eps,
                            void* workspace, size_t workspace_bytes, void* stream) try {
  ARG_CHECK(h && x && ctx && eps && workspace, "null");
  TRY(check_grad_shape(h, B, height, width));
  TRY(check_grad_handle(h, "hedit_unet_forward_keep"));
  drop_tape(h);
  GradTape* T = new GradTape();
  tape_init(*T, h, B, height, width, workspace, workspace_bytes, reinterpret_cast<hipStream_t>(stream), false);
  const int rc = forward_keep_impl(h, *T, x, t, ctx, eps);
  if (rc != HEDIT_OK) {
    delete T;
    return rc;
  }
  h->tape = T;
  h->tape_free = [](void* p) { delete reinterpret_cast<GradTape*>(p); };
  return HEDIT_OK;
} catch (...) { return hedit_abi_catch(); }

int hedit_unet_backward(hedit_unet* h, const float* d_eps, float* d_x, void* workspace, void* stream) try {
  ARG_CHECK(h && d_eps && d_x && workspace, "null");
  TRY(check_grad_handle(h, "hedit_unet_backward"));
  if (!h->tape) {
    hedit_set_error("hedit_unet_backward: no forward is being kept (call hedit_unet_forward_keep first)");
    return HEDIT_ERR_STATE;
  }
  GradTape* T = reinterpret_cast<GradTape*>(h->tape);
  if (T->ws != workspace) {
    hedit_set_error("hedit_unet_backward: not the workspace the kept forward ran in");
    return HEDIT_ERR_ARG;
  }
  T->f.st = reinterpret_cast<hipStream_t>(stream);
  const int rc = backward_impl(h, *T, d_eps, d_x);
  if (rc != HEDIT_OK) drop_tape(h);
  return rc;
} catch (...) { return hedit_abi_catch(); }

int hedit_unet_backward_ctx(hedit_unet* h, const float* d_eps, float* d_x, float* d_ctx, void* workspace, void* stream) try {
  ARG_CHECK(h && d_eps && d_ctx && workspace, "null");
  TRY(check_grad_handle(h, "hedit_unet_backward_ctx"));
  if (!h->wkv2_t) {
    hedit_set_error("hedit_unet_backward_ctx: this handle has no context-gradient weights (create it with hedit_unet_create_grad_ctx)");
    return HEDIT_ERR_STATE;
  }
  if (!h->tape) {
    hedit_set_error("hedit_unet_backward_ctx: no forward is being kept (call hedit_unet_forward_keep first)");
    return HEDIT_ERR_STATE;
  }
  GradTape* T = reinterpret_cast<GradTape*>(h->tape);
  if (T->ws != workspace) {
    hedit_set_error("hedit_unet_backward_ctx: not the workspace the kept forward ran in");
    return HEDIT_ERR_ARG;
  }
  T->f.st = reinterpret_cast<hipStream_t>(stream);
  const int rc = backward_impl(h, *T, d_eps, d_x, d_ctx);
  if (rc != HEDIT_OK) drop_tape(h);
  return rc;
} catch (...) { return hedit_abi_catch(); }

void hedit_unet_release(hedit_unet* h) try {
  if (h) drop_tape(h);
} catch (...) { (void)hedit_abi_catch(); }

int hedit_unet_vjp(hedit_unet* h, const float* x, float t, const float* ctx, const float* d_eps, int B, int height, int width,
                   float* d_x, float* eps, void* workspace, size_t workspace_bytes, void* stream) try {
  ARG_CHECK(h && x && ctx && d_eps && d_x && eps && workspace, "null");
  TRY(check_grad_shape(h, B, height, width));
  TRY(check_grad_handle(h, "hedit_unet_vjp"));
  drop_tape(h);
  GradTape T;
  tape_init(T, h, B, height, width, workspace, workspace_bytes, reinterpret_cast<hipStream_t>(stream), false);
  TRY(forward_keep_impl(h, T, x, t, ctx, eps));
  return backward_impl(h, T, d_eps, d_x);
} catch (...) { return hedit_abi_catch(); }

int hedit_prof_enable(hedit_unet* h, int on, int max_records) try {
  ARG_CHECK(h, "null");
  if (on && (int)h->prof_pool.size() < 2 * max_records) {
    const size_t want = (size_t)2 * max_records;
    while (h->prof_pool.size() < want) {
      hipEvent_t e;
      HIP_TRY(hipEventCreate(&e));
      h->prof_pool.push_back(e);
    }
  }
  h->prof_on = on != 0;
  return HEDIT_OK;
} catch (...) { return hedit_abi_catch(); }

int hedit_prof_reset(hedit_unet* h) try {
  ARG_CHECK(h, "null");
  h->prof_recs.clear();
  h->prof_next = 0;
  return HEDIT_OK;
} catch (...) { return hedit_abi_catch(); }

int hedit_prof_collect(hedit_unet* h, int kind, double* total_ms, double* total_flops, int64_t* count) try {
  ARG_CHECK(h && total_ms && total_flops && count && kind >= 0 && kind < PK_COUNT, "prof args");
  double ms = 0, fl = 0;
  int64_t n = 0;
  for (auto& r : h->prof_recs) {
    if (r.kind != kind) continue;
    float t = 0.f;
    HIP_TRY(hipEventElapsedTime(&t, h->prof_pool[r.e0], h->prof_pool[r.e1]));
    ms += t;
    fl += r.flops;
    ++n;
  }
  *total_ms = ms; *total_flops = fl; *count = n;
  return HEDIT_OK;
} catch (...) { return hedit_abi_catch(); }

int hedit_prof_records(hedit_unet* h, double* rows, int max_rows, int* n_rows) try {
  ARG_CHECK(h && rows && n_rows && max_rows >= 0, "prof args");
  int n = 0;
  for (auto& r : h->prof_recs) {
    if (n >= max_rows) break;
    float t = 0.f;
    HIP_TRY(hipEventElapsedTime(&t, h->prof_pool[r.e0], h->prof_pool[r.e1]));
    double* o = rows + (size_t)n * 8;
    o[0] = r.kind; o[1] = t; o[2] = r.flops; o[3] = r.bytes; o[4] = r.m; o[5] = r.n; o[6] = r.k; o[7] = r.tag;
    ++n;
  }
  *n_rows = n;
  return HEDIT_OK;
} catch (...) { return hedit_abi_catch(); }

int hedit_prof_collect_bytes(hedit_unet* h, int kind, double* total_bytes) try {
  ARG_CHECK(h && total_bytes && kind >= 0 && kind < PK_COUNT, "prof args");
  double b = 0;
  for (auto& r : h->prof_recs)
    if (r.kind == kind) b += r.bytes;
  *total_bytes = b;
  return HEDIT_OK;
} catch (...) { return hedit_abi_catch(); }

static void store_layers(const hedit_unet* h, int height, int width, std::vector<std::pair<int, int>>& v) {
  const hedit_unet_cfg& c = h->cfg;
// ... 42 lines not shown
```

h-edit_amd/hedit/_lib.py:

```python
import ctypes as C
import os

_HERE = os.path.dirname(os.path.abspath(__file__))
STORAGE = os.environ.get("HEDIT_STORAGE", "bf16").lower()
if STORAGE not in ("bf16", "f16"):
    raise ValueError(f"HEDIT_STORAGE must be bf16 or f16, not {STORAGE!r}")
LIB_PATH = os.path.join(_HERE, "libhedit_hip_f16.so" if STORAGE == "f16" else "libhedit_hip.so")
HEDIT_MAX_LEVELS = 8


class UnetCfg(C.Structure):
    _fields_ = [("in_channels", C.c_int), ("out_channels", C.c_int), ("sample_size", C.c_int),
                ("n_levels", C.c_int),
                ("block_out_channels", C.c_int * HEDIT_MAX_LEVELS),
                ("down_has_attn", C.c_int * HEDIT_MAX_LEVELS),
                ("up_has_attn", C.c_int * HEDIT_MAX_LEVELS),
                ("layers_per_block", C.c_int), ("cross_attention_dim", C.c_int),
                ("heads", C.c_int), ("norm_num_groups", C.c_int)]


class VaeCfg(C.Structure):
    _fields_ = [("in_channels", C.c_int), ("latent_channels", C.c_int), ("n_levels", C.c_int),
                ("block_out_channels", C.c_int * 4), ("layers_per_block", C.c_int),
                ("norm_num_groups", C.c_int)]


class DdpmCfg(C.Structure):
    _fields_ = [("in_channels", C.c_int), ("out_ch", C.c_int), ("ch", C.c_int), ("n_levels", C.c_int),
                ("ch_mult", C.c_int * 8), ("attn_level", C.c_int * 8), ("num_res_blocks", C.c_int),
                ("image_size", C.c_int)]


class VitCfg(C.Structure):
    _fields_ = [(n, C.c_int) for n in ("width", "layers", "heads", "patch_size", "input_resolution")]


class TextCfg(C.Structure):
    _fields_ = [(n, C.c_int) for n in ("width", "layers", "heads", "vocab_size", "context_length", "proj_dim")]


class ClipImgCfg(C.Structure):
    _fields_ = [(n, C.c_int) for n in ("width", "layers", "heads", "patch_size", "input_resolution", "embed_dim")]


class DinoCfg(C.Structure):
    _fields_ = [(n, C.c_int) for n in ("width", "layers", "heads", "patch_size", "input_resolution", "key_layer")]


class P2PPlan(C.Structure):
    _fields_ = [("mode", C.c_int), ("n_pairs", C.c_int),
                ("pair_src", C.c_void_p), ("pair_tar", C.c_void_p),
                ("singles", C.c_void_p), ("n_single", C.c_int),
                ("qk_src", C.c_void_p), ("mixT", C.c_void_p), ("bvec", C.c_void_p),
                ("h_store", C.POINTER(C.c_void_p)), ("n_store", C.c_int),
                ("kv_src", C.c_void_p), ("kv_first_block", C.c_int),
                ("qk_first_block", C.c_int), ("qk_max_tokens", C.c_int), ("feat_src", C.c_void_p), ("feat_resblock", C.c_int),
                ("h_store_self", C.POINTER(C.c_void_p)), ("n_store_self", C.c_int)]


class StepCoef(C.Structure):
    _fields_ = [(n, C.c_float) for n in ("sqrt_ab_t", "sqrt_1m_ab_t", "sqrt_ab_prev", "dir_coef",
                                         "noise_coef", "w_src", "w_hat", "w_tar", "coeff", "w_rec")]


def _family(name, cfg, finalizes, workspace_args):
    sigs = {"create": (C.c_int, ([C.POINTER(cfg)] if cfg else []) + [C.POINTER(C.c_void_p)]),
            "destroy": (None, [C.c_void_p]),
            "num_params": (C.c_int, [C.c_void_p]),
            "param_name": (C.c_char_p, [C.c_void_p, C.c_int]),
            "param_shape": (C.c_int, [C.c_void_p, C.c_int, C.POINTER(C.c_int), C.POINTER(C.c_int)]),
            "load": (C.c_int, [C.c_void_p, C.c_char_p, C.c_void_p, C.c_size_t, C.c_void_p]),
            "missing": (C.c_int, [C.c_void_p]),
            "workspace_bytes": (C.c_size_t, [C.c_void_p] + workspace_args)}
    if finalizes:
        sigs["finalize"] = (C.c_int, [C.c_void_p, C.c_void_p])
    return {f"hedit_{name}_{k}": v for k, v in sigs.items()}


_SIGS = {    "hedit_last_error": (C.c_char_p, []),
    "hedit_version": (C.c_int, []),
    **_family("unet", UnetCfg, False, [C.c_int] * 3),
    "hedit_unet_param_bf16_exact": (C.c_int, [C.c_void_p, C.c_int]),
    "hedit_unet_forward": (C.c_int, [C.c_void_p, C.c_void_p, C.c_float, C.c_void_p, C.c_int, C.c_int,
                                     C.c_int, C.POINTER(P2PPlan), C.c_void_p, C.c_void_p, C.c_size_t,
                                     C.c_void_p]),
    "hedit_unet_forward_shared": (C.c_int, [C.c_void_p, C.c_void_p, C.c_int, C.POINTER(C.c_int), C.c_float, C.c_void_p, C.c_int,
                                            C.c_int, C.c_int, C.POINTER(P2PPlan), C.c_void_p, C.c_void_p, C.c_size_t, C.c_void_p]),
    "hedit_unet_create_grad": (C.c_int, [C.POINTER(UnetCfg), C.POINTER(C.c_void_p)]),
    "hedit_unet_grad_workspace_bytes": (C.c_size_t, [C.c_void_p, C.c_int, C.c_int, C.c_int]),
    "hedit_unet_forward_keep": (C.c_int, [C.c_void_p, C.c_void_p, C.c_float, C.c_void_p, C.c_int, C.c_int, C.c_int, C.c_void_p,
                                          C.c_void_p, C.c_size_t, C.c_void_p]),
    "hedit_unet_backward": (C.c_int, [C.c_void_p, C.c_void_p, C.c_void_p, C.c_void_p, C.c_void_p]),
    "hedit_unet_create_grad_ctx": (C.c_int, [C.POINTER(UnetCfg), C.POINTER(C.c_void_p)]),
    "hedit_unet_backward_ctx": (C.c_int, [C.c_void_p, C.c_void_p, C.c_void_p, C.c_void_p, C.c_void_p, C.c_void_p]),
    "hedit_unet_release": (None, [C.c_void_p]),
    "hedit_unet_vjp": (C.c_int, [C.c_void_p, C.c_void_p, C.c_float, C.c_void_p, C.c_void_p, C.c_int, C.c_int, C.c_int, C.c_void_p,
                                 C.c_void_p, C.c_void_p, C.c_size_t, C.c_void_p]),
    "hedit_unet_set_attn_hook": (C.c_int, [C.c_void_p, C.c_void_p, C.c_void_p]),
    "hedit_unet_num_store_layers": (C.c_int, [C.c_void_p, C.c_int, C.c_int]),
    "hedit_unet_store_layer_info": (C.c_int, [C.c_void_p, C.c_int, C.c_int, C.c_int, C.POINTER(C.c_int),
                                              C.POINTER(C.c_int)]),
    "hedit_prof_enable": (C.c_int, [C.c_void_p, C.c_int, C.c_int]),
    "hedit_prof_reset": (C.c_int, [C.c_void_p]),
    "hedit_prof_collect": (C.c_int, [C.c_void_p, C.c_int, C.POINTER(C.c_double), C.POINTER(C.c_double),
                                     C.POINTER(C.c_int64)]),
    "hedit_prof_collect_bytes": (C.c_int, [C.c_void_p, C.c_int, C.POINTER(C.c_double)]),
    "hedit_prof_records": (C.c_int, [C.c_void_p, C.POINTER(C.c_double), C.c_int, C.POINTER(C.c_int)]),
    "hedit_step_base": (C.c_int, [C.c_void_p, C.c_void_p, C.c_void_p, C.c_void_p, C.c_int, C.c_int,
                                  C.c_int, C.POINTER(StepCoef), C.c_void_p]),
    "hedit_step_pair": (C.c_int, [C.c_void_p, C.c_void_p, C.c_void_p, C.c_void_p, C.c_void_p, C.c_int, C.c_int, C.c_int,
                                  C.POINTER(StepCoef), C.c_void_p]),
    "hedit_step_invert": (C.c_int, [C.c_void_p, C.c_void_p, C.c_void_p, C.c_void_p, C.c_void_p, C.c_int, C.c_int,
                                    C.POINTER(StepCoef), C.c_void_p]),
    "hedit_step_update": (C.c_int, [C.c_void_p, C.c_void_p, C.c_void_p, C.c_void_p, C.c_int64, C.c_void_p,
                                    C.c_void_p, C.c_void_p, C.c_int, C.c_int, C.c_int, C.POINTER(StepCoef),
                                    C.c_void_p]),
    "hedit_step_tweedie": (C.c_int, [C.c_void_p, C.c_void_p, C.c_int64, C.c_void_p, C.c_void_p, C.c_int, C.c_int,
                                     C.c_float, C.c_float, C.c_float, C.c_float, C.c_void_p]),
    "hedit_step_style": (C.c_int, [C.c_void_p, C.c_void_p, C.c_void_p, C.c_void_p, C.c_int64, C.c_void_p, C.c_void_p,
                                   C.c_void_p, C.c_int, C.c_int, C.c_float, C.c_float, C.c_float, C.c_float, C.c_void_p]),
    "hedit_step_ef_seed": (C.c_int, [C.c_void_p, C.c_void_p, C.c_int, C.c_int, C.c_float, C.c_float, C.c_float, C.c_void_p]),
    "hedit_step_ef_style": (C.c_int, [C.c_void_p, C.c_void_p, C.c_int64, C.c_void_p, C.c_void_p, C.c_void_p, C.c_void_p,
                                      C.c_int, C.c_int, C.c_float, C.c_float, C.c_void_p]),
    "hedit_local_blend": (C.c_int, [C.POINTER(C.c_void_p), C.c_int, C.c_int, C.c_void_p, C.c_void_p, C.c_void_p, C.c_int,
                                    C.c_int, C.c_int, C.c_int, C.c_float, C.c_void_p]),
    "hedit_local_blend_sub": (C.c_int, [C.POINTER(C.c_void_p), C.c_int, C.c_int, C.c_void_p, C.c_void_p, C.c_void_p, C.c_void_p,
                                        C.c_int, C.c_int, C.c_int, C.c_int, C.c_float, C.c_float, C.c_void_p]),
    **_family("ddpm", DdpmCfg, False, [C.c_int]),
    "hedit_ddpm_forward": (C.c_int, [C.c_void_p, C.c_void_p, C.c_float, C.c_int, C.c_void_p, C.c_void_p, C.c_size_t,
                                     C.c_void_p]),
    "hedit_ddpm_create_grad": (C.c_int, [C.POINTER(DdpmCfg), C.POINTER(C.c_void_p)]),
    "hedit_ddpm_grad_workspace_bytes": (C.c_size_t, [C.c_void_p, C.c_int]),
    "hedit_ddpm_forward_keep": (C.c_int, [C.c_void_p, C.c_void_p, C.c_float, C.c_int, C.c_void_p, C.c_void_p, C.c_size_t,
                                          C.c_void_p]),
    "hedit_ddpm_backward": (C.c_int, [C.c_void_p, C.c_void_p, C.c_void_p, C.c_void_p, C.c_void_p]),
    "hedit_ddpm_release": (None, [C.c_void_p]),
    "hedit_ddpm_vjp": (C.c_int, [C.c_void_p, C.c_void_p, C.c_float, C.c_void_p, C.c_int, C.c_void_p, C.c_void_p, C.c_void_p,
                                 C.c_size_t, C.c_void_p]),
    **_family("irse50", None, True, [C.c_int]),
    "hedit_irse50_features": (C.c_int, [C.c_void_p, C.c_void_p, C.c_int, C.c_void_p, C.c_void_p, C.c_size_t, C.c_void_p]),
    "hedit_irse50_cos_fwd_bwd": (C.c_int, [C.c_void_p, C.c_void_p, C.c_void_p, C.c_int, C.c_int, C.c_float, C.c_void_p,
                                           C.c_void_p, C.c_void_p, C.c_size_t, C.c_void_p]),
    **_family("lpips", None, True, [C.c_int] * 3),
    "hedit_lpips_feature_floats": (C.c_size_t, [C.c_int, C.c_int]),
    "hedit_lpips_source": (C.c_int, [C.c_void_p, C.c_void_p, C.c_int, C.c_int, C.c_int, C.c_void_p, C.c_void_p, C.c_size_t,
                                     C.c_void_p]),
    "hedit_lpips_fwd_bwd": (C.c_int, [C.c_void_p, C.c_void_p, C.c_void_p, C.c_int, C.c_int, C.c_int, C.c_int, C.c_float,
                                      C.c_void_p, C.c_void_p, C.c_void_p, C.c_size_t, C.c_void_p]),
    **_family("faceparse", None, True, [C.c_int] * 3),
    "hedit_faceparse_labels": (C.c_int, [C.c_void_p, C.c_void_p, C.c_int, C.c_int, C.c_int, C.c_int, C.c_void_p, C.c_void_p,
                                         C.c_size_t, C.c_void_p]),
    "hedit_face_mask_workspace_bytes": (C.c_size_t, [C.c_int, C.c_int, C.c_int]),
    "hedit_face_mask": (C.c_int, [C.c_void_p, C.c_int, C.c_int, C.c_int, C.c_int, C.c_float, C.c_int, C.c_void_p, C.c_void_p,
                                  C.c_void_p, C.c_size_t, C.c_void_p]),
    **_family("vit", VitCfg, True, [C.c_int]),
    "hedit_vit_gram": (C.c_int, [C.c_void_p, C.c_void_p, C.c_int, C.c_void_p, C.c_void_p, C.c_size_t, C.c_void_p]),
    "hedit_vit_gram_fwd_bwd": (C.c_int, [C.c_void_p, C.c_void_p, C.c_void_p, C.c_int, C.c_int, C.c_float, C.c_void_p, C.c_void_p,
                                         C.c_void_p, C.c_size_t, C.c_void_p]),
    **_family("text", TextCfg, True, [C.c_int] * 2),
    "hedit_text_encode": (C.c_int, [C.c_void_p, C.c_void_p, C.c_int, C.c_int, C.c_void_p, C.c_void_p, C.c_void_p, C.c_void_p,
                                    C.c_size_t, C.c_void_p]),
    **_family("clipimg", ClipImgCfg, True, [C.c_int]),
    "hedit_clipimg_set_slices": (C.c_int, [C.c_void_p, C.c_int]),
    "hedit_clipimg_encode": (C.c_int, [C.c_void_p, C.c_void_p, C.c_int, C.c_void_p, C.c_void_p, C.c_size_t, C.c_void_p]),
    **_family("sqlpips", None, True, [C.c_int] * 3),
    "hedit_sqlpips_distance": (C.c_int, [C.c_void_p, C.c_void_p, C.c_void_p, C.c_int, C.c_int, C.c_int, C.c_void_p, C.c_void_p,
                                         C.c_size_t, C.c_void_p]),
    **_family("dino", DinoCfg, True, [C.c_int] * 2),
    "hedit_dino_set_slices": (C.c_int, [C.c_void_p, C.c_int]),
    "hedit_dino_keys": (C.c_int, [C.c_void_p, C.c_void_p, C.c_int, C.c_int, C.c_void_p, C.c_void_p, C.c_size_t, C.c_void_p]),
    "hedit_dino_structure_distance": (C.c_int, [C.c_void_p, C.c_void_p, C.c_void_p, C.c_int, C.c_int, C.c_void_p, C.c_void_p, C.c_size_t,
                                                C.c_void_p]),
    "hedit_pixel_metrics_workspace_bytes": (C.c_size_t, [C.c_int, C.c_int, C.c_int]),
    "hedit_pixel_metrics": (C.c_int, [C.c_void_p, C.c_void_p, C.c_void_p, C.c_void_p, C.c_int, C.c_int, C.c_int, C.c_void_p, C.c_void_p,
                                      C.c_size_t, C.c_void_p]),
    **_family("vae", VaeCfg, False, [C.c_int] * 4),
    "hedit_vae_decode": (C.c_int, [C.c_void_p, C.c_void_p, C.c_int, C.c_int, C.c_int, C.c_void_p, C.c_void_p,
                                   C.c_size_t, C.c_void_p]),
    "hedit_vae_decode_vjp": (C.c_int, [C.c_void_p, C.c_void_p, C.c_void_p, C.c_int, C.c_int, C.c_int, C.c_void_p,
                                      C.c_void_p, C.c_void_p, C.c_size_t, C.c_void_p]),
    "hedit_vae_decode_keep": (C.c_int, [C.c_void_p, C.c_void_p, C.c_int, C.c_int, C.c_int, C.c_void_p, C.c_void_p,
                                       C.c_size_t, C.c_void_p]),
    "hedit_vae_decode_backward": (C.c_int, [C.c_void_p, C.c_void_p, C.c_void_p, C.c_void_p, C.c_void_p]),
    "hedit_vae_encode": (C.c_int, [C.c_void_p, C.c_void_p, C.c_int, C.c_int, C.c_int, C.c_void_p, C.c_void_p,
                                   C.c_size_t, C.c_void_p]),
    "hedit_axis_mix": (C.c_int, [C.c_void_p, C.c_void_p, C.c_void_p, C.c_void_p, C.c_int, C.c_int64, C.c_int, C.c_int, C.c_int,
                                 C.c_void_p]),
    "hedit_k_gemm_ws_bytes": (C.c_size_t, [C.c_int, C.c_int, C.c_int, C.c_int]),
    "hedit_k_gemm_canonical_chunk": (C.c_int, [C.c_int, C.c_int, C.c_int]),
    "hedit_k_gemm_plan_splits": (C.c_int, [C.c_int, C.c_int, C.c_int, C.c_int]),
    "hedit_k_gemm": (C.c_int, [C.c_void_p, C.c_void_p, C.c_void_p, C.c_void_p, C.c_void_p] + [C.c_int] * 13 +
                     [C.c_void_p, C.c_void_p]),
    "hedit_k_conv_gn": (C.c_int, [C.c_void_p, C.c_void_p, C.c_void_p, C.c_void_p, C.c_void_p] + [C.c_int] * 12 +
                        [C.c_void_p, C.c_void_p, C.c_void_p]),
    "hedit_k_groupnorm_from_parts": (C.c_int, [C.c_void_p, C.c_void_p, C.c_void_p, C.c_void_p, C.c_int, C.c_int, C.c_int, C.c_int,
                                               C.c_float, C.c_int, C.c_void_p, C.c_int, C.c_void_p, C.c_int, C.c_void_p, C.c_void_p]),
    "hedit_k_pack_geglu": (C.c_int, [C.c_void_p, C.c_void_p, C.c_void_p, C.c_void_p, C.c_int, C.c_int, C.c_void_p]),
    "hedit_k_gemm_geglu": (C.c_int, [C.c_void_p, C.c_void_p, C.c_void_p, C.c_void_p, C.c_int, C.c_int, C.c_int,
                                     C.c_int, C.c_int, C.c_void_p]),
    "hedit_test_set_flags": (C.c_int, [C.c_int]),
    "hedit_storage_is_f16": (C.c_int, []),
    "hedit_k_lin_chain_stream_bytes": (C.c_size_t, [C.c_int]),
    "hedit_k_lin_chain_pack": (C.c_int, [C.c_void_p, C.c_void_p, C.c_void_p, C.c_void_p, C.c_float, C.c_void_p, C.c_void_p]),
    "hedit_k_lin_chain": (C.c_int, [C.c_void_p, C.c_int64, C.c_void_p, C.c_int64, C.c_void_p, C.c_int, C.c_void_p, C.c_void_p, C.c_void_p,
                                    C.c_float, C.c_void_p, C.c_void_p, C.c_int64, C.c_void_p, C.c_int64, C.c_void_p, C.c_int64,
                                    C.c_void_p, C.c_int64, C.c_int, C.c_int, C.c_void_p]),
    "hedit_k_lin_chain_sched": (C.c_int, [C.c_void_p, C.c_int64, C.c_void_p, C.c_int64, C.c_void_p, C.c_int, C.c_void_p, C.c_void_p, C.c_void_p,
                                          C.c_float, C.c_void_p, C.c_void_p, C.c_int64, C.c_void_p, C.c_int64, C.c_void_p, C.c_int64,
                                          C.c_void_p, C.c_int64, C.c_int, C.c_int, C.c_int, C.c_void_p]),
    "hedit_k_groupnorm_affine": (C.c_int, [C.c_void_p, C.c_void_p, C.c_void_p, C.c_int, C.c_int, C.c_int, C.c_int, C.c_float, C.c_void_p,
                                           C.c_void_p, C.c_void_p]),
    "hedit_k_ffn_channels": (C.c_int, []),
    "hedit_k_ffn_stream_bytes": (C.c_size_t, [C.c_int]),
    "hedit_k_ffn_bias_bytes": (C.c_size_t, []),
    "hedit_k_ffn_pack": (C.c_int, [C.c_void_p, C.c_void_p, C.c_void_p, C.c_void_p, C.c_void_p, C.c_void_p, C.c_void_p, C.c_void_p]),
    "hedit_k_ffn_chain": (C.c_int, [C.c_void_p, C.c_int64, C.c_void_p, C.c_int64, C.c_void_p, C.c_int64, C.c_void_p, C.c_void_p, C.c_void_p,
                                    C.c_float, C.c_void_p, C.c_void_p, C.c_void_p, C.c_void_p, C.c_void_p, C.c_int64, C.c_int, C.c_int,
                                    C.c_void_p]),
    "hedit_k_ffn_fused": (C.c_int, [C.c_void_p, C.c_int64, C.c_void_p, C.c_void_p, C.c_float, C.c_void_p, C.c_void_p,
                                    C.c_void_p, C.c_void_p, C.c_int64, C.c_int, C.c_int, C.c_void_p]),
    "hedit_k_groupnorm_ws_bytes": (C.c_size_t, [C.c_int, C.c_int, C.c_int]),
    "hedit_k_groupnorm": (C.c_int, [C.c_void_p, C.c_void_p, C.c_void_p, C.c_void_p, C.c_int, C.c_int, C.c_int,
                                    C.c_int, C.c_float, C.c_int, C.c_void_p, C.c_void_p]),
    "hedit_k_layernorm": (C.c_int, [C.c_void_p, C.c_void_p, C.c_void_p, C.c_void_p, C.c_int64, C.c_int,
                                    C.c_float, C.c_void_p]),
    "hedit_k_geglu": (C.c_int, [C.c_void_p, C.c_void_p, C.c_int64, C.c_int, C.c_void_p]),
    "hedit_k_self_attn": (C.c_int, [C.c_void_p, C.c_int, C.c_void_p, C.c_int, C.c_void_p, C.c_int64, C.c_void_p,
                                    C.c_int, C.c_int, C.c_int, C.c_int, C.c_int, C.c_void_p, C.c_void_p, C.c_void_p]),
    "hedit_k_cross_attn": (C.c_int, [C.c_void_p, C.c_int, C.c_void_p, C.c_int, C.c_void_p, C.c_int64, C.c_void_p,
                                     C.c_int, C.c_int, C.c_int, C.c_int, C.c_int, C.POINTER(P2PPlan), C.c_void_p,
                                     C.c_void_p]),
    "hedit_k_attn_probs": (C.c_int, [C.c_void_p, C.c_int, C.c_void_p, C.c_int, C.c_void_p, C.c_int, C.c_int, C.c_int, C.c_int,
                                     C.c_int, C.c_int, C.c_void_p]),
    "hedit_k_attn_apply": (C.c_int, [C.c_void_p, C.c_void_p, C.c_int64, C.c_void_p, C.c_int, C.c_int, C.c_int, C.c_int, C.c_int,
                                     C.c_int, C.c_int, C.c_void_p]),
    "hedit_k_pack_conv3x3": (C.c_int, [C.c_void_p, C.c_void_p, C.c_int, C.c_int, C.c_void_p]),
    "hedit_k_f32_to_bf16": (C.c_int, [C.c_void_p, C.c_void_p, C.c_int64, C.c_void_p]),
    "hedit_k_groupnorm_stats": (C.c_int, [C.c_void_p, C.c_void_p, C.c_void_p, C.c_void_p, C.c_int, C.c_int, C.c_int,
                                          C.c_int, C.c_float, C.c_int, C.c_void_p, C.c_void_p, C.c_void_p]),
    "hedit_k_groupnorm_bwd_ws_bytes": (C.c_size_t, [C.c_int, C.c_int, C.c_int]),
# ... 75 lines not shown
```

h-edit_amd/hedit/engine.py:

```python
import ctypes as C

import torch

from . import _lib


def _f(x):
    return float(x)


class Schedule:

    def __init__(self, scheduler):
        self.s = scheduler
        self.ab = scheduler.alphas_cumprod.float().cpu()
        self.final = scheduler.final_alpha_cumprod.float().cpu() if isinstance(
            scheduler.final_alpha_cumprod, torch.Tensor) else torch.tensor(float(scheduler.final_alpha_cumprod))
        self.T = scheduler.num_inference_steps
        self.n_train = scheduler.config.num_train_timesteps

    def ab_prev(self, t):
        p = t - self.n_train // self.T
        return self.ab[p] if p >= 0 else self.final

    def variance(self, t):
        a_t, a_p = self.ab[t], self.ab_prev(t)
        return ((1 - a_p) / (1 - a_t)) * (1 - a_t / a_p)

    def full_coeff(self, t, t_prev, eta, ddim_inv):
        ab = self.ab
        sig, a = (1 - ab) ** 0.5, ab ** 0.5
        omega = eta * (sig[t_prev] / (sig[t] * a[t_prev])) * ((ab[t_prev] - ab[t]) ** 0.5)
        if ddim_inv:
            omega = 0
        return (1 - ab[t_prev] - omega ** 2) ** 0.5

    def edit_coeff(self, t, t_prev, eta, ddim_inv):
        ab = self.ab
        ratio = (ab ** 0.5)[t_prev] / (ab ** 0.5)[t]
        return self.full_coeff(t, t_prev, eta, ddim_inv) - ((1 - ab) ** 0.5)[t] * ratio

    def step_coef(self, t, t_prev, eta, ddim_inv, cfg, w_rec=0.0, coeff=None):
        a_t, a_p = self.ab[t], self.ab_prev(t)
        var = self.variance(t)
        c = _lib.StepCoef()
        c.sqrt_ab_t = _f(a_t ** 0.5)
        c.sqrt_1m_ab_t = _f((1 - a_t) ** 0.5)
        c.sqrt_ab_prev = _f(a_p ** 0.5)
        c.dir_coef = _f((1 - a_p) ** 0.5) if ddim_inv else _f((1 - a_p - (eta ** 2) * var) ** 0.5)
        c.noise_coef = 0.0 if eta <= 0 else (_f(eta) if ddim_inv else _f(eta * var ** 0.5))
        c.w_src, c.w_hat, c.w_tar = (float(v) for v in cfg)
        c.coeff = _f(self.edit_coeff(t, t_prev, eta, ddim_inv)) if coeff is None else _f(coeff)
        c.w_rec = float(w_rec)
        return c


class HEditEngine:
    def __init__(self, model, share_latents=True):
        self.model = model
        self.share_latents = share_latents
        self.unet = model.unet
        self.lib = _lib.lib()
        self.dev = model.unet.device
        self.style_chunk = 8

    def step_base(self, eps, xt, z, out, n, rows, coef):
        elems = xt[0].numel()
        _lib.check(self.lib.hedit_step_base(_lib.ptr(eps), _lib.ptr(xt), _lib.ptr(z), _lib.ptr(out), n, elems,
                                            rows, C.byref(coef), _lib.cur_stream()))

    def step_update(self, e_u_src, e_c_src, e_u_tar, e_c_tar, x_k, x_base, out, n, k_gt0, coef):
        elems = x_k[0].numel()
        for t_ in (e_u_src, e_c_src, e_u_tar, e_c_tar, x_k, x_base, out):
            assert t_.is_contiguous() and t_.dtype == torch.float32
        _lib.check(self.lib.hedit_step_update(_lib.ptr(e_u_src), _lib.ptr(e_c_src), _lib.ptr(e_u_tar),
                                              _lib.ptr(e_c_tar), elems, _lib.ptr(x_k), _lib.ptr(x_base),
                                              _lib.ptr(out), n, elems, int(k_gt0), C.byref(coef),
                                              _lib.cur_stream()))

    def style_step(self, e_u_src, e_c_src, e_u_tar, e_c_tar, x, tt, cfg_scales, image_encoder, weight):
        vae = self.model.vae
        if vae is None:
            raise RuntimeError("style guidance needs model.vae (hedit.vae.AutoencoderKL)")
        n, elems = x.shape[0], x[0].numel()
        ab = float(self.model.scheduler.alphas_cumprod[tt])
        sab, s1m = ab ** 0.5, (1.0 - ab) ** 0.5
        inv_scale = 1.0 / 0.18215
        for t_ in (e_u_src, e_c_src, e_u_tar, e_c_tar, x):
            assert t_.is_contiguous() and t_.dtype == torch.float32
        z0 = torch.empty_like(x)
        _lib.check(self.lib.hedit_step_tweedie(_lib.ptr(e_u_tar), _lib.ptr(e_c_tar), elems, _lib.ptr(x), _lib.ptr(z0),
                                               n, elems, float(cfg_scales[2]), sab, s1m, inv_scale, _lib.cur_stream()))
        g_z = torch.empty_like(x)
        for lo in range(0, n, self.style_chunk):
            hi = min(n, lo + self.style_chunk)
            g_z[lo:hi] = self._gram_grad(z0[lo:hi], image_encoder, lo)
        out = torch.empty_like(x)
        _lib.check(self.lib.hedit_step_style(_lib.ptr(e_u_src), _lib.ptr(e_c_src), _lib.ptr(e_u_tar), _lib.ptr(e_c_tar),
                                             elems, _lib.ptr(x), _lib.ptr(g_z), _lib.ptr(out), n, elems,
                                             float(cfg_scales[1]), float(cfg_scales[2]), inv_scale / sab, float(weight),
                                             _lib.cur_stream()))
        return out

    def _gram_grad(self, z0, image_encoder, lo):
        m = z0.shape[0]
        shared = not isinstance(image_encoder, (list, tuple))
        encs = [image_encoder] * m if shared else list(image_encoder[lo:lo + m])
        with torch.enable_grad():
            zc = z0.clone().requires_grad_(True)
            img = self.model.vae.decode(zc).sample
            if shared and hasattr(image_encoder, "gram_residual_norms"):
                loss = image_encoder.gram_residual_norms(img).sum()
            elif (not shared) and all(hasattr(e, "gram_residual_norms_each") for e in encs):
                loss = encs[0].gram_residual_norms_each(encs, img).sum()
            elif shared and hasattr(image_encoder, "gram_residuals"):
                loss = torch.linalg.norm(image_encoder.gram_residuals(img), dim=(1, 2)).sum()
            else:
                loss = sum(torch.linalg.norm(encs[i].get_gram_matrix_residual(img[i:i + 1])) for i in range(m))
            return torch.autograd.grad(outputs=loss, inputs=zc)[0]

    def ef_style_step(self, x, x_prev_tar, ctx_uncond, ctx_tar, t, w_tar, image_encoder, weight):
        unet, vae = self.unet, self.model.vae
        missing = [w for w, ok in (("model.unet built with its input-gradient pass (UNet2DConditionModel(grad=True))",
                                    getattr(unet, "grad", False)),
                                   ("model.vae (hedit.vae.AutoencoderKL)", vae is not None)) if not ok]
        if missing:
            raise RuntimeError("ef_style_step needs " + " and ".join(missing))
        n, elems = x.shape[0], x[0].numel()
        for t_ in (x, x_prev_tar, ctx_uncond, ctx_tar):
            assert t_.is_contiguous() and t_.dtype == torch.float32 and t_.shape[0] == n
        ab = float(self.model.scheduler.alphas_cumprod[int(t)])
        sab, s1m = ab ** 0.5, (1.0 - ab) ** 0.5
        inv_scale = 1.0 / 0.18215
        a = inv_scale / sab
        c = -a * s1m
        st = _lib.cur_stream
        out = torch.empty_like(x_prev_tar)
        for lo in range(0, n, self.style_chunk):
            hi = min(n, lo + self.style_chunk)
            m = hi - lo
            xc = x[lo:hi]
            ticket, eps = unet._keep(torch.cat([xc, xc]), float(t), torch.cat([ctx_uncond[lo:hi], ctx_tar[lo:hi]]))
            e_u, e_c = eps[:m], eps[m:]
            z0 = torch.empty_like(xc)
            _lib.check(self.lib.hedit_step_tweedie(_lib.ptr(e_u), _lib.ptr(e_c), elems, _lib.ptr(xc), _lib.ptr(z0), m, elems,
                                                   float(w_tar), sab, s1m, inv_scale, st()))
            g_z = self._gram_grad(z0, image_encoder, lo).contiguous()
            d_eps = torch.empty_like(eps)
            _lib.check(self.lib.hedit_step_ef_seed(_lib.ptr(g_z), _lib.ptr(d_eps), m, elems, float(w_tar), a, c, st()))
            if unet._ticket != ticket:
                raise RuntimeError("hedit.UNet2DConditionModel: the kept forward of this style step was dropped by a later model call")
            dx = torch.empty_like(eps)
            with torch.cuda.device(unet.device):
                _lib.check(self.lib.hedit_unet_backward(unet._h, _lib.ptr(d_eps), _lib.ptr(dx), _lib.ptr(unet._gws), st()))
            unet._release()
            _lib.check(self.lib.hedit_step_ef_style(_lib.ptr(e_u), _lib.ptr(e_c), elems, _lib.ptr(dx), _lib.ptr(g_z),
                                                    _lib.ptr(x_prev_tar[lo:hi]), _lib.ptr(out[lo:hi]), m, elems, a, float(weight),
                                                    st()))
        return out

    def encode(self, prompts):
        if getattr(self.model.text_encoder, "batch_invariant", False):
            tok = self.model.tokenizer(list(prompts), padding="max_length", max_length=self.model.tokenizer.model_max_length,
                                       truncation=True, return_tensors="pt")
            with torch.no_grad():
                return self.model.text_encoder(tok.input_ids)[0].float()
        out = []
        for p in prompts:
            tok = self.model.tokenizer([p], padding="max_length", max_length=self.model.tokenizer.model_max_length,
                                       truncation=True, return_tensors="pt")
            with torch.no_grad():
                out.append(self.model.text_encoder(tok.input_ids.to(self.dev))[0].float())
        return torch.cat(out)

    @torch.no_grad()
    def run(self, xT, zs, prompt_pairs, cfg_scales, controller=None, eta=1.0, p2p=True, implicit=True,
            K=1, w_rec=0.1, after_skip_steps=None, ddim_inv=False, ctx=None, fuse_src_pass=False,
            reuse_orig_eps=False, style=None, rec_pull=True):
        if style is not None and not (p2p and implicit):
            raise ValueError("style guidance is defined for the implicit P2P loop only (n-style h_edit.py)")
        sch = self.model.scheduler
        S = Schedule(sch)
        T = sch.num_inference_steps
        if after_skip_steps is None:
            after_skip_steps = T
        n = xT.shape[0]
        dev = self.dev
        xT = xT.to(device=dev, dtype=torch.float32)
        if zs is not None:
            zs = zs.to(device=dev, dtype=torch.float32).contiguous()
        if ctx is None:
            null = self.encode([""])
            src = self.encode([p[0] for p in prompt_pairs])
            tar = self.encode([p[1] for p in prompt_pairs])
        else:
            null, src, tar = (c.to(device=dev, dtype=torch.float32) for c in ctx)
        nulln = null.expand(n, -1, -1) if null.shape[0] == 1 else null
        ctx_base4 = torch.cat([nulln, nulln, src, src]).contiguous()
        ctx_base2 = torch.cat([nulln, src]).contiguous()
        ctx_edit = torch.cat([nulln, nulln, src, tar]).contiguous()
        ctx_src = src.contiguous()
        ctx_edit5 = torch.cat([nulln, nulln, src, tar, src]).contiguous() if fuse_src_pass else None

        ts = [int(v) for v in sch.timesteps]
        op = ts[-after_skip_steps:]
        ahead = ts[-(after_skip_steps + 1)] if after_skip_steps != T else -1
        xt = torch.cat([xT, xT]).contiguous()
        x_prev = torch.empty_like(xt)
        off = None

        from .p2p.ptp_classes import runs_in_python
        foreign = runs_in_python(controller)
        if foreign:
            if n != 1 or fuse_src_pass or reuse_orig_eps:
                raise ValueError("a foreign controller runs one image at a time, without fuse_src_pass / reuse_orig_eps "
                                 "(it sees the reference's 4-row batch)")
            if not callable(controller):
                raise TypeError("a foreign controller must be callable as controller(attn, is_cross, place_in_unet, save_attn)")
        step_cb = getattr(controller, "step_callback", None) if controller is not None else None
        if step_cb is not None and not callable(step_cb):
            raise TypeError("controller.step_callback must be callable as step_callback(x_t) -> x_t")

        share = self.share_latents

        def unet_rows(parts, blocks, t, ctx_rows, plan=None):
            if not share:
                return self.unet.forward_raw(torch.cat([parts[b] for b in blocks]), t, ctx_rows, plan)
            lat = parts[0] if len(parts) == 1 else torch.cat(parts)
            return self.unet.forward_raw(lat, t, ctx_rows, plan, row_latent=[b * n + j for b in blocks for j in range(n)])

        def p2p_pass(parts, blocks, t, save):
            rows = len(blocks) * n
            if foreign:
                return self.unet.forward_hooked(torch.cat([parts[b] for b in blocks]), t, ctx_edit, controller, save)
            plan = controller._plan(self.unet, rows, xT.shape[2], xT.shape[3], save) if controller is not None else None
            e = unet_rows(parts, blocks, t, ctx_edit5 if rows == 5 * n else ctx_edit, plan)
            if controller is not None:
                controller._after_pass(save)
            return e

        carry = None
        reuse = reuse_orig_eps and p2p and implicit
        for i, t in enumerate(op):
            idx = T - i - (T - after_skip_steps + 1)
            z = zs[idx] if zs is not None else None
            tt = op[i + 1] if i < len(op) - 1 else 0
            eta_i = float(eta[idx]) if isinstance(eta, (list, tuple)) else float(eta)
            coef = S.step_coef(t, tt, eta_i, ddim_inv, cfg_scales, w_rec)

            if (not p2p) and implicit and i == 0 and ahead != -1:
                xe = xt[n:]
                e = unet_rows([xe], (0, 0, 0, 0), t, ctx_edit, off)
                c0 = S.step_coef(t, tt, eta_i, ddim_inv, cfg_scales, w_rec, coeff=S.edit_coeff(ahead, t, eta_i, ddim_inv))
                new = torch.empty_like(xe)
                self.step_update(e[0:n], e[2 * n:3 * n], e[n:2 * n], e[3 * n:], xe, xe, new, n, False, c0)
                xt = torch.cat([xt[:n], new]).contiguous()

            if p2p and reuse and carry is not None:
                e2 = unet_rows([xt[n:]], (0, 0), t, ctx_base2, off)
                e = torch.cat([carry[0], e2[:n], carry[1], e2[n:]])
                self.step_base(e, xt, z, x_prev, n, 4, coef)
            elif p2p:
                e = unet_rows([xt[:n], xt[n:]], (0, 1, 0, 1), t, ctx_base4, off)
                self.step_base(e, xt, z, x_prev, n, 4, coef)
            else:
                e = unet_rows([xt[n:]], (0, 0), t, ctx_base2, off)
                self.step_base(e, xt, z, x_prev, n, 2, coef)
            x_orig, x_base = x_prev[:n], x_prev[n:]

            if not implicit:
                new = torch.empty_like(x_base)
                if p2p:
                    e_src = self.unet.forward_raw(xt[n:].contiguous(), t, ctx_src, off)
                    e = p2p_pass([xt[:n], xt[n:]], (0, 1, 0, 1), t, True)
                    self.step_update(e[n:2 * n], e_src, e[n:2 * n], e[3 * n:], x_base, x_base, new, n, False, coef)
                else:
                    e = unet_rows([xt[n:]], (0, 0, 0, 0), t, ctx_edit, off)
                    self.step_update(e[0:n], e[2 * n:3 * n], e[n:2 * n], e[3 * n:], x_base, x_base, new, n, False, coef)
                x_k = new
            else:
                x_k = x_base.clone()
                for k in range(K):
                    new = torch.empty_like(x_k)
                    if p2p:
                        save = not (k < K - 1 and K > 1)
                        if fuse_src_pass:
                            e = p2p_pass([x_orig, x_k], (0, 1, 0, 1, 1), tt, save)
                            e_src = e[4 * n:]
                        else:
                            e_src = self.unet.forward_raw(x_k, tt, ctx_src, off)
                            e = p2p_pass([x_orig, x_k], (0, 1, 0, 1), tt, save)
                        self.step_update(e[n:2 * n], e_src, e[n:2 * n], e[3 * n:4 * n], x_k, x_base, new, n,
                                         k > 0 and style is None and rec_pull, coef)
                        if style is not None and style[0] is not None:
                            with torch.enable_grad():
                                new = self.style_step(e[n:2 * n], e_src, e[n:2 * n], e[3 * n:4 * n], new, tt, cfg_scales,
                                                      style[0], style[1])
                        if reuse:
                            carry = (e[0:n], e[2 * n:3 * n])
                    else:
                        e = unet_rows([x_k], (0, 0, 0, 0), tt, ctx_edit, off)
                        self.step_update(e[0:n], e[2 * n:3 * n], e[n:2 * n], e[3 * n:], x_k, x_base, new, n, k > 0, coef)
                    x_k = new

            xt = torch.cat([x_orig, x_k]).contiguous()
            if step_cb is not None:
                xt = step_cb(xt)
        return xt[n:].clone(), xt[:n].clone()

    @torch.no_grad()
    def run_pnp(self, xT, zs, prompts, cfg_scales, eta=1.0, K=1, after_skip_steps=None, ddim_inv=True):
        from .plug_n_play.pnp_utils import register_time
        sch = self.model.scheduler
        S = Schedule(sch)
        T = sch.num_inference_steps
        if after_skip_steps is None:
            after_skip_steps = T
        dev = self.dev
        xT = xT.to(device=dev, dtype=torch.float32)
        n = xT.shape[0]
        pairs = [list(prompts[:2])] if isinstance(prompts[0], str) else [list(p[:2]) for p in prompts]
        if len(pairs) != n:
            raise ValueError("one [source, target] prompt pair per image expected")
        if zs is not None:
            zs = zs.to(device=dev, dtype=torch.float32).contiguous()
            if zs.dim() == 4:
                zs = zs[:, None]
        null = self.encode([""]).expand(n, -1, -1)
        src, tar = self.encode([p[0] for p in pairs]), self.encode([p[1] for p in pairs])
        ctx_base4 = torch.cat([null, null, src, src]).contiguous()
        ctx_k2 = torch.cat([null, src]).contiguous()
        ctx_pair = torch.cat([src, tar]).contiguous()
        editor = getattr(self.unet, "_attention_editor", None)
        ts = [int(v) for v in sch.timesteps]
        op = ts[-after_skip_steps:]
        xt = torch.cat([xT, xT]).contiguous()
        x_prev = torch.empty_like(xt)
        H, W = xT.shape[2], xT.shape[3]
        for i, t in enumerate(op):
            idx = T - i - (T - after_skip_steps + 1)
            z = zs[idx] if zs is not None else None
            tt = op[i + 1] if i < len(op) - 1 else 0
            eta_i = float(eta[idx]) if isinstance(eta, (list, tuple)) else float(eta)
            coef = S.step_coef(t, tt, eta_i, ddim_inv, cfg_scales, 0.0)
            register_time(self.model, t)
            e = self.unet.forward_raw(torch.cat([xt, xt]), t, ctx_base4, None)
            self.step_base(e, xt, z, x_prev, n, 4, coef)
            x_orig, x_base = x_prev[:n], x_prev[n:]
            x_k = x_base.clone()
            for _ in range(K):
                register_time(self.model, tt)
                e2 = self.unet.forward_raw(torch.cat([x_k, x_k]), tt, ctx_k2, None)
                plan = editor._plan(self.unet, 2 * n, H, W, True, n_images=n) if editor is not None else None
                ep = self.unet.forward_raw(torch.cat([x_orig, x_k]), tt, ctx_pair, plan)
                if editor is not None:
                    editor._after_pass(True)
                new = torch.empty_like(x_k)
                self.step_update(e2[0:n], e2[n:2 * n], e2[0:n], ep[n:2 * n].contiguous(), x_k, x_base, new, n, False, coef)
                x_k = new
            xt = torch.cat([x_orig, x_k]).contiguous()
        return xt[n:].clone(), xt[:n].clone()

    def step_pair(self, e_u, e_c, xt, z, out, n, kinds, coefs):
        elems = xt[0].numel()
        for t_ in (e_u, e_c, xt, out) + (() if z is None else (z,)):
            assert t_.is_contiguous() and t_.dtype == torch.float32
        arr = (_lib.StepCoef * kinds)(*coefs)
        _lib.check(self.lib.hedit_step_pair(_lib.ptr(e_u), _lib.ptr(e_c), _lib.ptr(xt), _lib.ptr(z), _lib.ptr(out), n, elems,
                                            kinds, arr, _lib.cur_stream()))

    def _pair_coefs(self, S, t, eta_i, ddim_inv, cfg_pair):
        return [S.step_coef(t, 0, eta_i, ddim_inv, (cfg_pair[0], 0.0, 0.0), coeff=0.0),
                S.step_coef(t, 0, 0.0 if ddim_inv else eta_i, ddim_inv, (cfg_pair[-1], 0.0, 0.0), coeff=0.0)]

    @torch.no_grad()
    def run_direct(self, xT, zs, prompt_pairs, cfg_pair, controller=None, eta=1.0, after_skip_steps=None, ddim_inv=False,
                   control=True):
        sch = self.model.scheduler
        S = Schedule(sch)
        T = sch.num_inference_steps
        if after_skip_steps is None:
            after_skip_steps = T
        n = xT.shape[0]
        dev = self.dev
        pairs = [list(p) for p in prompt_pairs]
        if len(pairs) != n or any(len(p) != len(pairs[0]) or len(p) not in (1, 2) for p in pairs):
            raise ValueError("one [source, target] pair (or one [target]) per image expected")
        kinds = len(pairs[0])
        if len(cfg_pair) != kinds:
            raise ValueError("one guidance weight per prompt expected")
        xT = xT.to(device=dev, dtype=torch.float32)
        if zs is not None:
            zs = zs.to(device=dev, dtype=torch.float32).contiguous()
        null = self.encode([""]).expand(n, -1, -1)
        tar = self.encode([p[-1] for p in pairs])
        if kinds == 2:
            ctx = torch.cat([null, null, self.encode([p[0] for p in pairs]), tar]).contiguous()
        else:
            ctx = torch.cat([null, tar]).contiguous()
        controlled = control and kinds == 2 and controller is not None

        from .p2p.ptp_classes import runs_in_python
        foreign = controlled and runs_in_python(controller)
        if foreign:
            if n != 1:
                raise ValueError("a foreign controller runs one image at a time (it sees the reference's 4-row batch)")
            if not callable(controller):
                raise TypeError("a foreign controller must be callable as controller(attn, is_cross, place_in_unet, save_attn)")
        step_cb = getattr(controller, "step_callback", None) if controller is not None else None
        if step_cb is not None and not callable(step_cb):
            raise TypeError("controller.step_callback must be callable as step_callback(x_t) -> x_t")

        ts = [int(v) for v in sch.timesteps]
        op = ts[-after_skip_steps:]
        xt = torch.cat([xT] * kinds).contiguous()
        H, W = xT.shape[2], xT.shape[3]
        for i, t in enumerate(op):
            idx = T - i - (T - after_skip_steps + 1)
            z = zs[idx] if zs is not None else None
            eta_i = float(eta[idx]) if isinstance(eta, (list, tuple)) else float(eta)
            x_in = torch.cat([xt, xt])
            if foreign:
                e = self.unet.forward_hooked(x_in, t, ctx, controller, True)
            elif controlled:
                e = self.unet.forward_raw(x_in, t, ctx, controller._plan(self.unet, 4 * n, H, W, True))
                controller._after_pass(True)
            else:
                e = self.unet.forward_raw(x_in, t, ctx, None)
            coefs = self._pair_coefs(S, t, eta_i, ddim_inv, cfg_pair)
            x_next = torch.empty_like(xt)
            self.step_pair(e[:kinds * n], e[kinds * n:], xt, z, x_next, n, kinds, coefs[:kinds])
            xt = x_next
            if kinds == 2 and step_cb is not None:
                xt = step_cb(xt)
        if kinds == 1:
            if step_cb is not None:
                xt = step_cb(xt)
            return xt.clone(), None
        return xt[n:].clone(), xt[:n].clone()

    @torch.no_grad()
    def run_direct_pnp(self, xT, zs, prompts, cfg_pair, eta=0.0, after_skip_steps=None, ddim_inv=False, uncond="null"):
        from .plug_n_play.pnp_utils import register_time
        if uncond not in ("null", "src"):
            raise ValueError("uncond must be 'null' or 'src'")
        sch = self.model.scheduler
        S = Schedule(sch)
        T = sch.num_inference_steps
        if after_skip_steps is None:
            after_skip_steps = T
        dev = self.dev
        xT = xT.to(device=dev, dtype=torch.float32)
        n = xT.shape[0]
        pairs = [list(prompts[:2])] if isinstance(prompts[0], str) else [list(p[:2]) for p in prompts]
        if len(pairs) != n:
            raise ValueError("one [source, target] prompt pair per image expected")
        if zs is not None:
            zs = zs.to(device=dev, dtype=torch.float32).contiguous()
            if zs.dim() == 4:
                zs = zs[:, None]
# ... 112 lines not shown
```

h-edit_amd/hedit/unet.py:

```python
import ctypes as C
import hashlib
import math

import torch

from . import _lib
from .native import NativeOwner

SD15_CONFIG = dict(in_channels=4, out_channels=4, sample_size=64,
                   block_out_channels=(320, 640, 1280, 1280),
                   down_block_types=("CrossAttnDownBlock2D", "CrossAttnDownBlock2D",
                                     "CrossAttnDownBlock2D", "DownBlock2D"),
                   up_block_types=("UpBlock2D", "CrossAttnUpBlock2D", "CrossAttnUpBlock2D",
                                   "CrossAttnUpBlock2D"),
                   layers_per_block=2, cross_attention_dim=768, attention_head_dim=8,
                   norm_num_groups=32)

TINY_CONFIG = dict(in_channels=4, out_channels=4, sample_size=32,
                   block_out_channels=(64, 128, 128),
                   down_block_types=("CrossAttnDownBlock2D", "CrossAttnDownBlock2D", "DownBlock2D"),
                   up_block_types=("UpBlock2D", "CrossAttnUpBlock2D", "CrossAttnUpBlock2D"),
                   layers_per_block=2, cross_attention_dim=64, attention_head_dim=2,
                   norm_num_groups=32)


class UNetOutput(dict):
    @property
    def sample(self):
        return self["sample"]


class AttnProcessor:
    controller = None


def random_state_dict(param_shapes, seed=0):
    sd = {}
    for name, shape in param_shapes.items():
        hsh = hashlib.sha256(f"{seed}:{name}".encode()).digest()
        g = torch.Generator().manual_seed(int.from_bytes(hsh[:7], "little"))
        if len(shape) >= 2:
            fan_in = 1
            for s in shape[1:]:
                fan_in *= s
            sd[name] = torch.randn(shape, generator=g) / math.sqrt(fan_in)
        elif "norm" in name and name.endswith("weight"):
            sd[name] = 1.0 + 0.1 * torch.randn(shape, generator=g)
        elif "norm" in name:
            sd[name] = 0.1 * torch.randn(shape, generator=g)
        else:
            sd[name] = 0.02 * torch.randn(shape, generator=g)
    return sd


class _EpsGrad(torch.autograd.Function):

    @staticmethod
    def forward(ctx, sample, enc, model, t):
        ctx.model = model
        ctx.ticket, eps = model._keep(sample.detach(), t, enc)
        ctx.shape = sample.shape
        ctx.enc_shape = enc.shape
        return eps

    @staticmethod
    def backward(ctx, g):
        m = ctx.model
        if m._ticket != ctx.ticket:
            raise RuntimeError("hedit.UNet2DConditionModel: the kept forward of this graph was dropped by a later model call")
        g = g.detach().to(dtype=torch.float32).contiguous()
        want_x, want_c = ctx.needs_input_grad[0], ctx.needs_input_grad[1]
        dx = torch.empty(ctx.shape, dtype=torch.float32, device=m.device) if want_x else None
        dc = torch.empty(ctx.enc_shape, dtype=torch.float32, device=m.device) if want_c else None
        with torch.cuda.device(m.device):
            if want_c:
                _lib.check(m._lib.hedit_unet_backward_ctx(m._h, _lib.ptr(g), _lib.ptr(dx) if want_x else None, _lib.ptr(dc),
                                                          _lib.ptr(m._gws), _lib.cur_stream()))
            elif want_x:
                _lib.check(m._lib.hedit_unet_backward(m._h, _lib.ptr(g), _lib.ptr(dx), _lib.ptr(m._gws), _lib.cur_stream()))
        return dx, dc, None, None


class UNet2DConditionModel(NativeOwner):
    _family, _finalizes = "unet", False
    _tickets = 0

    def __init__(self, config=None, device="cuda:0", grad=False):
        cfg = dict(SD15_CONFIG)
        cfg.update(config or {})
        self.config = cfg
        self.device = torch.device(device)
        if self.device.type != "cuda":
            raise RuntimeError("hedit.UNet2DConditionModel runs on the GPU only (HIP kernels)")
        self.in_channels = cfg["in_channels"]
        self.sample_size = cfg["sample_size"]
        c = _lib.UnetCfg()
        c.in_channels, c.out_channels, c.sample_size = cfg["in_channels"], cfg["out_channels"], cfg["sample_size"]
        ch = list(cfg["block_out_channels"])
        c.n_levels = len(ch)
        for i, v in enumerate(ch):
            c.block_out_channels[i] = v
            c.down_has_attn[i] = int(cfg["down_block_types"][i].startswith("CrossAttn"))
            c.up_has_attn[i] = int(cfg["up_block_types"][i].startswith("CrossAttn"))
        c.layers_per_block = cfg["layers_per_block"]
        c.cross_attention_dim = cfg["cross_attention_dim"]
        c.heads = cfg["attention_head_dim"]
        c.norm_num_groups = cfg["norm_num_groups"]
        self._cfg_struct = c
        if isinstance(grad, str) and grad != "context":
            raise ValueError(f'grad must be False, True or "context", got {grad!r}')
        self._native_build(self.device, None, c, create="create_grad_ctx" if grad == "context" else "create_grad" if grad else "create")
        self.grad = bool(grad)
        self.grad_context = grad == "context"
        self._ticket = 0
        self._gws = None
        self.param_shapes = self._native_param_shapes()
        self.bf16_exact = {name for i, name in enumerate(self.param_shapes) if self._lib.hedit_unet_param_bf16_exact(self._h, i)}
        self._procs = {n: AttnProcessor() for n in self._processor_names()}
        self.heads = cfg["attention_head_dim"]

    load_state_dict = NativeOwner._native_load

    def init_random(self, seed=0):
        sd = random_state_dict(self.param_shapes, seed)
        self.load_state_dict(sd)
        return sd

    def zero_grad(self, *a, **k):
        return None

    def _processor_names(self):
        cfg = self.config
        names = []
        L = cfg["layers_per_block"]
        for i, t in enumerate(cfg["down_block_types"]):
            if t.startswith("CrossAttn"):
                for j in range(L):
                    for a in ("attn1", "attn2"):
                        names.append(f"down_blocks.{i}.attentions.{j}.transformer_blocks.0.{a}.processor")
        for a in ("attn1", "attn2"):
            names.append(f"mid_block.attentions.0.transformer_blocks.0.{a}.processor")
        for i, t in enumerate(cfg["up_block_types"]):
            if t.startswith("CrossAttn"):
                for j in range(L + 1):
                    for a in ("attn1", "attn2"):
                        names.append(f"up_blocks.{i}.attentions.{j}.transformer_blocks.0.{a}.processor")
        return names

    @property
    def attn_processors(self):
        return dict(self._procs)

    def set_attn_processor(self, procs):
        if not isinstance(procs, dict):
            procs = {k: procs for k in self._procs}
        for k, p in procs.items():
            if k not in self._procs:
                raise KeyError(f"unknown attention processor name {k}")
            if not hasattr(p, "controller"):
                raise TypeError(
                    f"{type(p).__name__}: a processor is identified by its .controller (None = plain attention, a hedit "
                    "controller = in-kernel edit, any other callable = hooked through hedit_unet_set_attn_hook); processor "
                    "objects that re-implement the attention body itself cannot be run -- the body is the HIP kernels")
            c = p.controller
            if c is not None and not hasattr(c, "_plan") and not callable(c):
                raise TypeError(f"{type(c).__name__}: a foreign controller must be callable as "
                                "controller(attention_probs, is_cross, place_in_unet, save_attn)")
            self._procs[k] = p

    def _controller(self):
        ctrls = {id(p.controller): p.controller for p in self._procs.values() if p.controller is not None}
        if not ctrls:
            return None
        if len(ctrls) != 1 or any(p.controller is None for p in self._procs.values()):
            raise RuntimeError("all attention layers must share one controller "
                               "(use hedit.p2p.ptp_utils.register_attention_control)")
        return next(iter(ctrls.values()))

    def store_layers(self, height, width):
        n = self._lib.hedit_unet_num_store_layers(self._h, height, width)
        out = []
        tok, pl = C.c_int(), C.c_int()
        for i in range(n):
            _lib.check(self._lib.hedit_unet_store_layer_info(self._h, height, width, i, C.byref(tok), C.byref(pl)))
            out.append((tok.value, ("down", "mid", "up")[pl.value]))
        return out

    def _workspace(self, B, H, W):
        need = self._lib.hedit_unet_workspace_bytes(self._h, B, H, W)
        if need == 0:
            raise _lib.HipError("workspace planning failed: " + self._lib.hedit_last_error().decode())
        return self._grow("_ws", need, self.device)

    PROF_KINDS = ("conv3x3_gemm", "linear_gemm", "self_attn", "cross_attn", "norm", "other")

    def prof_enable(self, on, max_records=8192):
        _lib.check(self._lib.hedit_prof_enable(self._h, int(on), max_records))

    def prof_reset(self):
        _lib.check(self._lib.hedit_prof_reset(self._h))

    def prof_collect(self):
        torch.cuda.synchronize(self.device)
        out = {}
        ms, fl, n = C.c_double(), C.c_double(), C.c_int64()
        for i, k in enumerate(self.PROF_KINDS):
            _lib.check(self._lib.hedit_prof_collect(self._h, i, C.byref(ms), C.byref(fl), C.byref(n)))
            out[k] = (ms.value, fl.value, n.value)
        return out

    def prof_collect_bytes(self):
        out = {}
        b = C.c_double()
        for i, k in enumerate(self.PROF_KINDS):
            _lib.check(self._lib.hedit_prof_collect_bytes(self._h, i, C.byref(b)))
            out[k] = b.value
        return out

    def prof_records(self, max_rows=16384):
        import numpy as np
        torch.cuda.synchronize(self.device)
        rows = np.zeros((max_rows, 8), dtype=np.float64)
        n = C.c_int()
        _lib.check(self._lib.hedit_prof_records(self._h, rows.ctypes.data_as(C.POINTER(C.c_double)), max_rows, C.byref(n)))
        return rows[:n.value]

    def forward_raw(self, sample, t, ctx, plan=None, out=None, row_latent=None):
        B, Cc, H, W = sample.shape
        if row_latent is not None:
            B = len(row_latent)
        if sample.dtype != torch.float32 or ctx.dtype != torch.float32:
            raise TypeError("sample and encoder_hidden_states must be float32")
        if ctx.shape != (B, 77, self.config["cross_attention_dim"]):
            raise ValueError(f"encoder_hidden_states must be ({B}, 77, {self.config['cross_attention_dim']}), "
                             f"got {tuple(ctx.shape)}")
        sample = sample.contiguous()
        ctx = ctx.contiguous()
        if out is None:
            out = torch.empty(B, self.config["out_channels"], H, W, dtype=torch.float32, device=sample.device)
        ws = self._workspace(B, H, W)
        if row_latent is None:
            _lib.check(self._lib.hedit_unet_forward(
                self._h, _lib.ptr(sample), C.c_float(float(t)), _lib.ptr(ctx), B, H, W,
                C.byref(plan) if plan is not None else None, _lib.ptr(out), _lib.ptr(ws), ws.numel(),
                _lib.cur_stream()))
            return out
        if sample.data_ptr() % 16:
            sample = sample.clone()
        _lib.check(self._lib.hedit_unet_forward_shared(
            self._h, _lib.ptr(sample), sample.shape[0], (C.c_int * B)(*row_latent), C.c_float(float(t)), _lib.ptr(ctx), B, H, W,
            C.byref(plan) if plan is not None else None, _lib.ptr(out), _lib.ptr(ws), ws.numel(),
            _lib.cur_stream()))
        return out

    def _release(self):
        if self._ticket:
            self._lib.hedit_unet_release(self._h)
            self._ticket = 0

    def _keep(self, sample, t, ctx):
        sample, ctx = sample.contiguous(), ctx.detach().contiguous()
        B, _, H, W = sample.shape
        if ctx.shape != (B, 77, self.config["cross_attention_dim"]):
            raise ValueError(f"encoder_hidden_states must be ({B}, 77, {self.config['cross_attention_dim']}), got {tuple(ctx.shape)}")
        need = self._lib.hedit_unet_grad_workspace_bytes(self._h, B, H, W)
        if need == 0:
            raise _lib.HipError("gradient workspace planning failed: " + self._lib.hedit_last_error().decode())
        self._grow("_gws", need, self.device)
        eps = torch.empty(B, self.config["out_channels"], H, W, dtype=torch.float32, device=self.device)
        with torch.cuda.device(self.device):
            _lib.check(self._lib.hedit_unet_forward_keep(self._h, _lib.ptr(sample), C.c_float(float(t)), _lib.ptr(ctx), B, H, W,
                                                         _lib.ptr(eps), _lib.ptr(self._gws), self._gws.numel(), _lib.cur_stream()))
        UNet2DConditionModel._tickets += 1
        self._ticket = UNet2DConditionModel._tickets
        return self._ticket, eps

    _HOOK_T = C.CFUNCTYPE(C.c_int, C.c_void_p, C.c_void_p, C.c_int, C.c_int, C.c_int, C.c_int, C.c_int, C.c_int, C.c_void_p)

    def forward_hooked(self, sample, t, ctx, controller, save_attn=True, out=None):
        B, _, H, W = sample.shape
        state = {"exc": None}
        places = ("down", "mid", "up")

        def cb(_user, probs, bh, nq, nk, is_cross, place, _layer, _stream):
            try:
                off = int(probs) - self._ws.data_ptr()
                view = self._ws[off:off + bh * nq * nk * 4].view(torch.float32).view(bh, nq, nk)
                attn = view.clone()
                controller(attn, bool(is_cross), places[place], save_attn)
                view.copy_(attn)
                return 0
            except BaseException as e:
                state["exc"] = e
                return 1

        fn = self._HOOK_T(cb)
        _lib.check(self._lib.hedit_unet_set_attn_hook(self._h, C.cast(fn, C.c_void_p), None))
        try:
            try:
                return self.forward_raw(sample, t, ctx, None, out)
            except _lib.HipError:
                if state["exc"] is not None:
                    raise state["exc"]
                raise
        finally:
            _lib.check(self._lib.hedit_unet_set_attn_hook(self._h, None, None))

    def forward(self, sample, timestep=None, encoder_hidden_states=None, cross_attention_kwargs=None,
                return_dict=True):
        kw = dict(cross_attention_kwargs or {})
        use_controller = kw.pop("use_controller", True)
        save_attn = kw.pop("save_attn", True)
        use_editor = kw.pop("use_editor", True)
        if kw:
            raise TypeError(f"unsupported cross_attention_kwargs {sorted(kw)}")
        if isinstance(timestep, torch.Tensor):
            tt = timestep.reshape(-1)
            if tt.numel() > 1 and not bool((tt == tt[0]).all()):
                raise NotImplementedError("per-sample timesteps: the batch must share one timestep")
            t = float(tt[0])
        else:
            t = float(timestep)
        sample = sample.to(device=self.device, dtype=torch.float32)
        ctx = encoder_hidden_states.to(device=self.device, dtype=torch.float32)
        controller = self._controller() if use_controller else None
        if controller is None and use_editor:
            controller = getattr(self, "_attention_editor", None)
        if self.grad:
            self._release()
            ctx_grad = torch.is_grad_enabled() and encoder_hidden_states.requires_grad
            if ctx_grad and not self.grad_context:
                raise NotImplementedError("the gradient with respect to encoder_hidden_states (null-text inversion) is not "
                                          "implemented on this model: the input-gradient pass of grad=True differentiates the "
                                          "sample only (build the model with grad=\"context\")")
            if torch.is_grad_enabled() and (sample.requires_grad or ctx_grad):
                if controller is not None:
                    what = "an attention editor" if controller is getattr(self, "_attention_editor", None) else "a registered controller"
                    raise NotImplementedError(f"{what} is in the way: the input-gradient pass differentiates the plain network "
                                              "only (pass cross_attention_kwargs={'use_controller': False, 'use_editor': False})")
                return UNetOutput(sample=_EpsGrad.apply(sample, ctx, self, t))
        from .p2p.ptp_classes import runs_in_python
        if runs_in_python(controller):
            return UNetOutput(sample=self.forward_hooked(sample, t, ctx, controller, save_attn))
        plan = None
        if controller is not None:
            plan = controller._plan(self, sample.shape[0], sample.shape[2], sample.shape[3], save_attn)
        eps = self.forward_raw(sample, t, ctx, plan)
        if controller is not None:
            controller._after_pass(save_attn)
        return UNetOutput(sample=eps)

    __call__ = forward
```

include/hedit.h:

```cpp
#ifndef HEDIT_H
#define HEDIT_H
#include <stddef.h>
#include <stdint.h>

#ifdef __cplusplus
extern "C" {
#endif

#define HEDIT_MAX_LEVELS 8

typedef struct hedit_unet hedit_unet;

typedef struct {
  int in_channels, out_channels, sample_size;
  int n_levels;
  int block_out_channels[HEDIT_MAX_LEVELS];
  int down_has_attn[HEDIT_MAX_LEVELS];
  int up_has_attn[HEDIT_MAX_LEVELS];
  int layers_per_block;
  int cross_attention_dim;
  int heads;
  int norm_num_groups;
} hedit_unet_cfg;

typedef struct {
  int mode;
  int n_pairs;
  const int32_t* pair_src;
  const int32_t* pair_tar;
  const int32_t* singles;
  int n_single;
  const int32_t* qk_src;
  const void* mixT;
  const float* bvec;
  float* const* h_store;
  int n_store;
  const int32_t* kv_src;
  int kv_first_block;
  int qk_first_block, qk_max_tokens;
  const int32_t* feat_src;
  int feat_resblock;
  float* const* h_store_self;
  int n_store_self;
} hedit_p2p_plan;

typedef struct {
  float sqrt_ab_t, sqrt_1m_ab_t, sqrt_ab_prev, dir_coef, noise_coef;
  float w_src, w_hat, w_tar, coeff, w_rec;
} hedit_step_coef;

const char* hedit_last_error(void);
int hedit_version(void);

int hedit_unet_create(const hedit_unet_cfg* cfg, hedit_unet** out);
void hedit_unet_destroy(hedit_unet* h);
int hedit_unet_num_params(const hedit_unet* h);
const char* hedit_unet_param_name(const hedit_unet* h, int i);
int hedit_unet_param_shape(const hedit_unet* h, int i, int* ndim, int* dims4);
int hedit_unet_load(hedit_unet* h, const char* name, const float* w, size_t numel, void* stream);
int hedit_unet_param_bf16_exact(const hedit_unet* h, int i);
int hedit_unet_missing(const hedit_unet* h);
size_t hedit_unet_workspace_bytes(hedit_unet* h, int B, int height, int width);
int hedit_unet_forward(hedit_unet* h, const float* x, float t, const float* ctx, int B, int height,
                       int width, const hedit_p2p_plan* plan, float* eps_out, void* workspace,
                       size_t workspace_bytes, void* stream);
int hedit_unet_forward_shared(hedit_unet* h, const float* x, int D, const int* row_latent, float t, const float* ctx, int B,
                              int height, int width, const hedit_p2p_plan* plan, float* eps_out, void* workspace,
                              size_t workspace_bytes, void* stream);
typedef int (*hedit_attn_hook_fn)(void* user, float* probs, int batch_heads, int n_query, int n_key, int is_cross, int place,
                                  int layer, void* stream);
int hedit_unet_set_attn_hook(hedit_unet* h, hedit_attn_hook_fn fn, void* user);
int hedit_unet_num_store_layers(const hedit_unet* h, int height, int width);
int hedit_unet_store_layer_info(const hedit_unet* h, int height, int width, int i, int* tokens,
                                int* place );

int hedit_unet_create_grad(const hedit_unet_cfg* cfg, hedit_unet** out);
int hedit_unet_create_grad_ctx(const hedit_unet_cfg* cfg, hedit_unet** out);
int hedit_unet_backward_ctx(hedit_unet* h, const float* d_eps, float* d_x, float* d_ctx, void* workspace, void* stream);
size_t hedit_unet_grad_workspace_bytes(hedit_unet* h, int B, int height, int width);
int hedit_unet_forward_keep(hedit_unet* h, const float* x, float t, const float* ctx, int B, int height, int width, float* eps,
                            void* workspace, size_t workspace_bytes, void* stream);
int hedit_unet_backward(hedit_unet* h, const float* d_eps, float* d_x, void* workspace, void* stream);
void hedit_unet_release(hedit_unet* h);
int hedit_unet_vjp(hedit_unet* h, const float* x, float t, const float* ctx, const float* d_eps, int B, int height, int width,
                   float* d_x, float* eps, void* workspace, size_t workspace_bytes, void* stream);

int hedit_prof_enable(hedit_unet* h, int on, int max_records);
int hedit_prof_reset(hedit_unet* h);
int hedit_prof_collect(hedit_unet* h, int kind, double* total_ms, double* total_flops, int64_t* count);
int hedit_prof_collect_bytes(hedit_unet* h, int kind, double* total_bytes);
int hedit_prof_records(hedit_unet* h, double* rows, int max_rows, int* n_rows);

int hedit_step_base(const float* eps, const float* xt, const float* z, float* x_prev, int n_img,
                    int elems, int eps_rows_per_img, const hedit_step_coef* c, void* stream);
int hedit_step_pair(const float* e_u, const float* e_c, const float* xt, const float* z, float* x_next, int n_img,
                    int elems, int n_kinds, const hedit_step_coef* c, void* stream);
int hedit_step_invert(const float* e_u, const float* e_c, const float* xt, float* x_prev, float* z_out,
                      int n_img, int elems, const hedit_step_coef* c, void* stream);
int hedit_step_update(const float* e_u_src, const float* e_c_src, const float* e_u_tar,
                      const float* e_c_tar, int64_t stride_img, const float* x_k,
                      const float* x_base, float* x_out, int n_img, int elems, int k_gt0,
                      const hedit_step_coef* c, void* stream);
int hedit_step_tweedie(const float* e_u_tar, const float* e_c_tar, int64_t stride_img, const float* x, float* z0,
                       int n_img, int elems, float w_tar, float sqrt_ab, float sqrt_1m_ab, float inv_scale, void* stream);
int hedit_step_style(const float* e_u_src, const float* e_c_src, const float* e_u_tar, const float* e_c_tar,
                     int64_t stride_img, const float* x, const float* g_z, float* x_out, int n_img, int elems,
                     float w_hat, float w_tar, float chain, float weight, void* stream);
int hedit_step_ef_seed(const float* g_z, float* d_eps, int n_img, int elems, float w_tar, float a, float c, void* stream);
int hedit_step_ef_style(const float* e_u, const float* e_c, int64_t stride_img, const float* dx, const float* g_z,
                        const float* x_prev, float* x_out, int n_img, int elems, float a, float weight, void* stream);
int hedit_axis_mix(const float* in, float* out, const int32_t* idx, const float* val, int nnz, int64_t outer, int n_in, int n_out,
                   int inner, void* stream);
int hedit_local_blend(float* const* h_maps, int n_maps, int heads, const float* alpha_layers,
                      const int32_t* enabled, float* xt, int n_img, int C, int H, int W, float th,
                      void* stream);
int hedit_local_blend_sub(float* const* h_maps, int n_maps, int heads, const float* alpha_layers,
                          const float* substruct_layers, const int32_t* enabled, float* xt, int n_img, int C, int H,
                          int W, float th, float th_sub, void* stream);

typedef struct hedit_vae hedit_vae;
typedef struct hedit_vae_cfg {
  int in_channels;
  int latent_channels;
  int n_levels;
  int block_out_channels[4];
  int layers_per_block;
  int norm_num_groups;
} hedit_vae_cfg;
int hedit_vae_create(const hedit_vae_cfg* cfg, hedit_vae** out);
void hedit_vae_destroy(hedit_vae* h);
int hedit_vae_num_params(const hedit_vae* h);
const char* hedit_vae_param_name(const hedit_vae* h, int i);
int hedit_vae_param_shape(const hedit_vae* h, int i, int* ndim, int* dims4);
int hedit_vae_load(hedit_vae* h, const char* name, const float* dev_w, size_t numel, void* stream);
int hedit_vae_missing(const hedit_vae* h);
size_t hedit_vae_workspace_bytes(hedit_vae* h, int B, int latent_h, int latent_w, int encode);
int hedit_vae_decode(hedit_vae* h, const float* z, int B, int latent_h, int latent_w, float* image,
                     void* workspace, size_t workspace_bytes, void* stream);
int hedit_vae_decode_vjp(hedit_vae* h, const float* z, const float* d_image, int B, int latent_h, int latent_w,
                         float* d_z, float* image, void* workspace, size_t workspace_bytes, void* stream);
int hedit_vae_decode_keep(hedit_vae* h, const float* z, int B, int latent_h, int latent_w, float* image,
                          void* workspace, size_t workspace_bytes, void* stream);
int hedit_vae_decode_backward(hedit_vae* h, const float* d_image, float* d_z, void* workspace, void* stream);
int hedit_vae_encode(hedit_vae* h, const float* image, int B, int height, int width, float* mean,
                     void* workspace, size_t workspace_bytes, void* stream);

size_t hedit_k_gemm_ws_bytes(int M, int N, int K, int splits);
int hedit_k_gemm_canonical_chunk(int M_nominal, int N_nominal, int K);
int hedit_k_gemm_plan_splits(int M, int N, int K, int chunk_kt);
int hedit_k_gemm(const void* A, const void* W, const float* bias, const void* residual, void* C,
                 int M, int N, int K, int lda, int ldc, int ldr, int mode, int Hin, int Win,
                 int Cin, int Hout, int Wout, int splits, void* partial_ws, void* stream);
int hedit_k_conv_gn(const void* A, const void* W, const float* bias, const void* residual, void* C, int M, int N, int K, int ldc,
                    int ldr, int mode, int Hin, int Win, int Cin, int Hout, int Wout, int splits, void* partial_ws, float* gn_part,
                    void* stream);
int hedit_k_groupnorm_from_parts(const void* x, void* y, const float* gamma, const float* beta, int B, int HW, int C, int G,
                                 float eps, int silu, const float* part_a, int ca, const float* part_b, int cb, void* ws,
                                 void* stream);
int hedit_k_pack_geglu(const float* w, const float* bias, void* w_packed_bf16, float* bias_packed,
                       int inner, int K, void* stream);
int hedit_k_gemm_geglu(const void* A, const void* w_packed, const float* bias_packed, void* C, int M,
                       int inner, int K, int lda, int ldc, void* stream);
int hedit_k_ffn_channels(void);
size_t hedit_k_ffn_stream_bytes(int with_outer_layers);
size_t hedit_k_ffn_bias_bytes(void);
int hedit_k_ffn_pack(const float* w1, const float* b1, const float* w2, const float* w_pre, const float* w_post, void* stream_out,
                     float* bias1_out, void* stream);
int hedit_k_ffn_fused(const void* x, int64_t ldx, const float* gamma, const float* beta, float eps, const void* w_stream,
                      const float* bias1_packed, const float* bias2, void* out, int64_t ldo, int M, int C, void* stream);
int hedit_k_ffn_chain(const void* a, int64_t lda, const void* t1, int64_t ldt1, const void* x, int64_t ldx, const float* bias_pre,
                      const float* gamma, const float* beta, float eps, const void* w_stream, const float* bias1_packed,
                      const float* bias2, const float* bias_post, void* out, int64_t ldo, int M, int C, void* stream);
size_t hedit_k_lin_chain_stream_bytes(int n_out);
int hedit_k_lin_chain_pack(const float* w_pre, const float* w0, const float* w1, const float* w2, float scale0, void* stream_out,
                           void* stream);
int hedit_k_lin_chain(const void* a, int64_t lda, const void* r1, int64_t ldr1, const float* gn_ss, int rows_per_image,
                      const float* bias_pre, const float* gamma, const float* beta, float eps, const void* w_stream, void* out_mid,
                      int64_t ldmid, void* out_q, int64_t ldq, void* out_k, int64_t ldk, void* out, int64_t ldo, int M, int C,
                      void* stream);
int hedit_k_lin_chain_sched(const void* a, int64_t lda, const void* r1, int64_t ldr1, const float* gn_ss, int rows_per_image,
                            const float* bias_pre, const float* gamma, const float* beta, float eps, const void* w_stream, void* out_mid,
                            int64_t ldmid, void* out_q, int64_t ldq, void* out_k, int64_t ldk, void* out, int64_t ldo, int M, int C,
                            int sched, void* stream);
int hedit_storage_is_f16(void);
int hedit_test_set_flags(int flags);
size_t hedit_k_groupnorm_ws_bytes(int B, int HW, int C);
int hedit_k_groupnorm_affine(const void* x, const float* gamma, const float* beta, int B, int HW, int C, int G, float eps, void* ws,
                             float* ss_out, void* stream);
int hedit_k_groupnorm(const void* x, void* y, const float* gamma, const float* beta, int B, int HW,
                      int C, int G, float eps, int silu, void* ws, void* stream);
int hedit_k_layernorm(const void* x, void* y, const float* gamma, const float* beta, int64_t rows,
                      int C, float eps, void* stream);
int hedit_k_geglu(const void* x, void* y, int64_t rows, int inner, void* stream);
int hedit_k_self_attn(const void* q, int ldq, const void* k, int ldk, const void* vt, int64_t ldvt,
                      void* out, int ldo, int B, int N, int heads, int d, const int32_t* qk_src, const int32_t* kv_src,
                      void* stream);
int hedit_k_cross_attn(const void* q, int ldq, const void* k, int ldk, const void* vt, int64_t ldvt,
                       void* out, int ldo, int B, int N, int heads, int d,
                       const hedit_p2p_plan* plan, float* store, void* stream);
int hedit_k_attn_probs(const void* q, int ldq, const void* k, int ldk, float* probs, int B, int N, int M, int kstride,
                       int heads, int d, void* stream);
int hedit_k_attn_apply(const float* probs, const void* vt, int64_t ldvt, void* out, int ldo, int B, int N, int M,
                       int kstride, int heads, int d, void* stream);
int hedit_k_pack_conv3x3(const float* w_oihw, void* out, int O, int I, void* stream);
int hedit_k_f32_to_bf16(const float* x, void* y, int64_t n, void* stream);
int hedit_k_groupnorm_stats(const void* x, void* y, const float* gamma, const float* beta, int B, int HW, int C, int G,
                            float eps, int silu, void* ws, float* stats, void* stream);
size_t hedit_k_groupnorm_bwd_ws_bytes(int B, int HW, int C);
int hedit_k_groupnorm_bwd(const void* x, const void* dy, const void* add, void* dx, const float* gamma, const float* beta,
                          const float* stats, int B, int HW, int C, int G, int silu, void* ws, void* stream);
int hedit_k_softmax_rows(const float* s, void* p, int64_t rows, int N, float scale, void* stream);
int hedit_k_softmax_blockdiag(const float* s, void* p, int64_t rows, int T, int ld, float scale, void* stream);
int hedit_k_softmax_bwd(const void* p, const float* dp, void* ds, int64_t rows, int N, float scale, void* stream);
int hedit_k_transpose(const void* src, void* dst, int R, int C, void* stream);
int hedit_k_sum2x2(const void* du, void* dx, int B, int H, int W, int C, void* stream);
int hedit_k_pack_conv3x3_dgrad(const float* w_oihw, void* out, int O, int I, void* stream);
int hedit_k_pack_linear_t(const float* w, void* out, int O, int I, void* stream);
int hedit_k_flip_oihw(const float* w_oihw, float* out, int O, int I, int k, void* stream);
int hedit_k_pack_conv3x3_s2_dgrad(const float* w_oihw, void* out, int O, int I, void* stream);
int hedit_k_conv3x3_s2_dgrad(const void* dy, const void* w_packed, void* dx, int B, int Hin, int Win, int O, int I, void* stream);
int hedit_k_slice_add(const void* src, int ld, int off, int c, void* dst, int64_t rows, int accumulate, void* stream);
// ... 182 lines not shown
```

Measured before the change: 2.676.

## Bind precomputed text-context projections and widen one-launch GroupNorm loads

Adds a UNet context object that pads the prompt embeddings and projects the cross-attention keys and values once, so every denoising step and Langevin iteration reuses them instead of recomputing them per forward call. The engine now builds bound contexts for each prompt row set and passes them to forward. Separately, the small-image GroupNorm kernel now stages its input with vectorised, unrolled loads, precomputes per-channel scale and shift in LDS, and spreads images across blocks, with the old kernel kept behind a flag. This costs extra device memory for the cached contexts and adds template variants chosen by alignment.

```diff
diff --git a/h-edit_amd/csrc/c_api.hip b/h-edit_amd/csrc/c_api.hip
--- a/h-edit_amd/csrc/c_api.hip
+++ b/h-edit_amd/csrc/c_api.hip
@@ -309,7 +309,7 @@
 int hedit_storage_is_f16(void) { return HEDIT_F16; }
 
 int hedit_test_set_flags(int flags) try {
-  ARG_CHECK(flags >= 0 && flags <= 15, "hedit_test_set_flags: bit 0 drained ring waits, bit 1 exact self-attention pass, bit 2 pixel-UNet GroupNorm statistics path flipped, bit 3 no persistent linear kernel");
+  ARG_CHECK(flags >= 0 && flags <= 31, "hedit_test_set_flags: bit 0 drained ring waits, bit 1 exact self-attention pass, bit 2 pixel-UNet GroupNorm statistics path flipped, bit 3 no persistent linear kernel, bit 4 narrow one-launch GroupNorm");
   g_test_flags.store(flags, std::memory_order_relaxed);
   return HEDIT_OK;
 } catch (...) { return hedit_abi_catch(); }
diff --git a/h-edit_amd/csrc/norm.hip b/h-edit_amd/csrc/norm.hip
--- a/h-edit_amd/csrc/norm.hip
+++ b/h-edit_amd/csrc/norm.hip
@@ -583,9 +583,9 @@
   }
 }
 
-__global__ __launch_bounds__(256) void gn_small_kernel(const bf16_t* __restrict__ x, bf16_t* __restrict__ y,
-                                                       const float* __restrict__ gamma, const float* __restrict__ beta,
-                                                       int HW, int C, int G, float eps, int silu, float* __restrict__ stats) {
+__global__ __launch_bounds__(256) void gn_small_narrow_kernel(const bf16_t* __restrict__ x, bf16_t* __restrict__ y,
+                                                              const float* __restrict__ gamma, const float* __restrict__ beta,
+                                                              int HW, int C, int G, float eps, int silu, float* __restrict__ stats) {
   extern __shared__ uint32_t gs_pairs[];
   __shared__ float red[8];
   const int g = blockIdx.x, b = blockIdx.y, tid = threadIdx.x;
@@ -626,6 +626,91 @@
   }
 }
 
+template <int NW>
+using gs_vec = uint32_t __attribute__((ext_vector_type(NW)));
+constexpr int GS_U = 5;
+
+template <int NW>
+__global__ __launch_bounds__(256) void gn_small_kernel(const bf16_t* __restrict__ x, bf16_t* __restrict__ y,
+                                                       const float* __restrict__ gamma, const float* __restrict__ beta,
+                                                       int HW, int C, int G, int B, float eps, int silu, float* __restrict__ stats) {
+  typedef gs_vec<NW> V;
+  extern __shared__ uint4 gs_wide[];
+  __shared__ float red[8];
+  const int tid = threadIdx.x;
+  const int slot = blockIdx.x >> 3, slot_img = slot / G;
+  const int b = (blockIdx.x & 7) + 8 * slot_img, g = slot - slot_img * G;
+  if (b >= B) return;
+  const int cpg = C / G, ppp = cpg / 2, vpp = ppp / NW;
+  const int npair = HW * ppp, nvec = HW * vpp;
+  const int rowv = C / (2 * NW);
+  uint32_t* pairs = reinterpret_cast<uint32_t*>(gs_wide);
+  V* vecs = reinterpret_cast<V*>(gs_wide);
+  float* scale = reinterpret_cast<float*>(pairs + npair);
+  float* shift = scale + cpg;
+  const int dq = 256 / vpp, dr = 256 - dq * vpp;
+  {
+    const V* xin = reinterpret_cast<const V*>(x + (long)b * HW * C + g * cpg);
+    int pix = tid / vpp, k = tid - pix * vpp;
+    for (int v0 = tid; v0 < nvec; v0 += 256 * GS_U) {
+      V r[GS_U];
+#pragma unroll
+      for (int u = 0; u < GS_U; ++u) {
+        r[u] = V(0);
+        if (v0 + u * 256 < nvec) r[u] = xin[(long)pix * rowv + k];
+        pix += dq; k += dr;
+        if (k >= vpp) { k -= vpp; ++pix; }
+      }
+#pragma unroll
+      for (int u = 0; u < GS_U; ++u)
+        if (v0 + u * 256 < nvec) vecs[v0 + u * 256] = r[u];
+    }
+  }
+  __syncthreads();
+  float s = 0.f, q = 0.f;
+  for (int i = tid; i < npair; i += 256) {
+    const uint32_t u = pairs[i];
+    const float a = st_lo(u), c = st_hi(u);
+    s += a; s += c;
+    q += a * a; q += c * c;
+  }
+  s = wave_sum(s);
+  q = wave_sum(q);
+  if ((tid & 63) == 0) { red[(tid >> 6) * 2] = s; red[(tid >> 6) * 2 + 1] = q; }
+  __syncthreads();
+  s = ((red[0] + red[2]) + red[4]) + red[6];
+  q = ((red[1] + red[3]) + red[5]) + red[7];
+  const float n = (float)HW * (float)cpg;
+  const float m = s / n;
+  float var = q / n - m * m;
+  var = var < 0.f ? 0.f : var;
+  const float rstd = rsqrtf(var + eps);
+  if (stats && tid == 0) *reinterpret_cast<float2*>(stats + ((long)b * G + g) * 2) = make_float2(m, rstd);
+  for (int c = tid; c < cpg; c += 256) {
+    const float sc = rstd * gamma[g * cpg + c];
+    scale[c] = sc;
+    shift[c] = beta[g * cpg + c] - m * sc;
+  }
+  __syncthreads();
+  V* yout = reinterpret_cast<V*>(y + (long)b * HW * C + g * cpg);
+  int pix = tid / vpp, k = tid - pix * vpp;
+  for (int v = tid; v < nvec; v += 256) {
+    const V u = vecs[v];
+    V o;
+#pragma unroll
+    for (int w = 0; w < NW; ++w) {
+      const int c0 = 2 * (k * NW + w);
+      float a = st_lo(u[w]) * scale[c0] + shift[c0];
+      float c = st_hi(u[w]) * scale[c0 + 1] + shift[c0 + 1];
+      if (silu) { a = silu_f(a); c = silu_f(c); }
+      o[w] = pack_bf16x2(a, c);
+    }
+    yout[(long)pix * rowv + k] = o;
+    pix += dq; k += dr;
+    if (k >= vpp) { k -= vpp; ++pix; }
+  }
+}
+
 __global__ __launch_bounds__(256) void gn_fold_kernel(const float* __restrict__ pa, int npa, const float* __restrict__ pb, int npb,
                                                       float* __restrict__ out, int units, int ppg) {
   __shared__ float red[8];
@@ -677,7 +762,19 @@
   ARG_CHECK(C % 8 == 0 && C % G == 0 && G <= 64, "groupnorm: C % 8, C % G, G <= 64");
   ARG_CHECK(C / 8 <= 256 * GN_MAXV, "groupnorm: C too large");
   if (HW < 1024 && (C / G) % 2 == 0 && (size_t)HW * (C / G) * 2 <= 60 * 1024) {
-    hipLaunchKernelGGL(gn_small_kernel, dim3(G, B), dim3(256), (size_t)HW * (C / G) * 2, st, x, y, gamma, beta, HW, C, G, eps, silu, stats);
+    const int cpg = C / G;
+    const size_t lds = (size_t)HW * cpg * 2 + (size_t)cpg * 2 * sizeof(float);
+    if ((hedit_test_flags() & 16) || lds > 64 * 1024) {
+      hipLaunchKernelGGL(gn_small_narrow_kernel, dim3(G, B), dim3(256), (size_t)HW * cpg * 2, st, x, y, gamma, beta, HW, C, G, eps, silu, stats);
+      LAUNCH_CHECK();
+      return HEDIT_OK;
+    }
+    const uintptr_t al = (uintptr_t)x | (uintptr_t)y;
+    const int nw = (cpg * 2) % 16 == 0 && al % 16 == 0 ? 4 : ((cpg * 2) % 8 == 0 && al % 8 == 0 ? 2 : 1);
+    const dim3 grid((unsigned)((B + 7) / 8 * 8 * G));
+    if (nw == 4) hipLaunchKernelGGL(gn_small_kernel<4>, grid, dim3(256), lds, st, x, y, gamma, beta, HW, C, G, B, eps, silu, stats);
+    else if (nw == 2) hipLaunchKernelGGL(gn_small_kernel<2>, grid, dim3(256), lds, st, x, y, gamma, beta, HW, C, G, B, eps, silu, stats);
+    else hipLaunchKernelGGL(gn_small_kernel<1>, grid, dim3(256), lds, st, x, y, gamma, beta, HW, C, G, B, eps, silu, stats);
     LAUNCH_CHECK();
     return HEDIT_OK;
   }
diff --git a/h-edit_amd/csrc/unet.hip b/h-edit_amd/csrc/unet.hip
--- a/h-edit_amd/csrc/unet.hip
+++ b/h-edit_amd/csrc/unet.hip
@@ -601,9 +601,37 @@
   return HEDIT_OK;
 }
 
+int project_context(Fwd& f, const float* ctx) {
+  hedit_unet* h = f.h;
+  const hedit_unet_cfg& c = h->cfg;
+  const int MC = f.B * HEDIT_CTXP;
+  bf16_t *ctxb, *k2a, *vt2a;
+  TRY(aalloc(f, &ctxb, (size_t)MC * c.cross_attention_dim));
+  RUN(f, ctx_pad_launch(ctx, ctxb, f.B, c.cross_attention_dim, f.st));
+  f.ctxb = ctxb;
+  TRY(aalloc(f, &k2a, (size_t)MC * h->ctx_n));
+  TRY(aalloc(f, &vt2a, (size_t)MC * h->ctx_n));
+  TRY(linear(f, ctxb, MC, c.cross_attention_dim, h->wk2_all, h->ctx_n, nullptr, nullptr, k2a, h->ctx_n));
+  TRY(linear(f, h->wv2_all, h->ctx_n, c.cross_attention_dim, ctxb, MC, nullptr, nullptr, vt2a, MC, 2));
+  f.k2_all = k2a;
+  f.vt2_all = vt2a;
+  return HEDIT_OK;
+}
+
+}
+
+struct HEDIT_HANDLE hedit_unet_context {
+  const hedit_unet* owner = nullptr;
+  int B = 0;
+  void* buf = nullptr;
+  const bf16_t *ctxb = nullptr, *k2_all = nullptr, *vt2_all = nullptr;
+};
+
+namespace {
+
 int forward_impl(hedit_unet* h, const float* x, float t, const float* ctx, int B, int H0, int W0,
                  const hedit_p2p_plan* plan, float* eps_out, void* ws, size_t ws_bytes, hipStream_t st,
-                 bool dry, size_t* peak, int D = 0, const RowMap* map = nullptr) {
+                 bool dry, size_t* peak, int D = 0, const RowMap* map = nullptr, const hedit_unet_context* cx = nullptr) {
   const hedit_unet_cfg& c = h->cfg;
   Fwd f;
   f.h = h; f.B = B; f.st = st; f.plan = plan; f.map = map;
@@ -615,19 +643,10 @@
     return HEDIT_ERR_ARG;
   }
 
-  bf16_t* ctxb;
-  TRY(aalloc(f, &ctxb, (size_t)B * HEDIT_CTXP * c.cross_attention_dim));
-  RUN(f, ctx_pad_launch(ctx, ctxb, B, c.cross_attention_dim, st));
-  f.ctxb = ctxb;
-  {
-    const int MC = B * HEDIT_CTXP;
-    bf16_t *k2a, *vt2a;
-    TRY(aalloc(f, &k2a, (size_t)MC * h->ctx_n));
-    TRY(aalloc(f, &vt2a, (size_t)MC * h->ctx_n));
-    TRY(linear(f, ctxb, MC, c.cross_attention_dim, h->wk2_all, h->ctx_n, nullptr, nullptr, k2a, h->ctx_n));
-    TRY(linear(f, h->wv2_all, h->ctx_n, c.cross_attention_dim, ctxb, MC, nullptr, nullptr, vt2a, MC, 2));
-    f.k2_all = k2a;
-    f.vt2_all = vt2a;
+  if (cx) {
+    f.ctxb = cx->ctxb; f.k2_all = cx->k2_all; f.vt2_all = cx->vt2_all;
+  } else {
+    TRY(project_context(f, ctx));
   }
 
   float *te0, *te1, *te2, *temb_all;
@@ -959,7 +978,7 @@
   return need;
 } catch (...) { (void)hedit_abi_catch(); return 0; }
 
-static int forward_checks(hedit_unet* h, const float* x, const float* ctx, int B, int height, int width, const hedit_p2p_plan* plan,
+static int forward_checks(hedit_unet* h, const float* x, const void* ctx, int B, int height, int width, const hedit_p2p_plan* plan,
                           float* eps_out, void* workspace) {
   ARG_CHECK(h && x && ctx && eps_out && workspace, "null");
   ARG_CHECK(B >= 1, "B");
@@ -984,23 +1003,99 @@
                       reinterpret_cast<hipStream_t>(stream), false, nullptr);
 } catch (...) { return hedit_abi_catch(); }
 
+static int row_map_checks(const float* x, int D, const int* row_latent, int B, RowMap* map) {
+  ARG_CHECK(row_latent && D >= 1 && D <= 65535, "row map");
+  if (B > HEDIT_ROWMAP_MAX) {
+    hedit_set_error("batch larger than " + std::to_string(HEDIT_ROWMAP_MAX) + " rows (the row map of shared latents)");
+    return HEDIT_ERR_ARG;
+  }
+  ARG_CHECK(reinterpret_cast<uintptr_t>(x) % 16 == 0, "x must be 16-byte aligned");
+  for (int r = 0; r < B; ++r) {
+    ARG_CHECK(row_latent[r] >= 0 && row_latent[r] < D, "row_latent entries must lie in [0, D)");
+    map->src[r] = (uint16_t)row_latent[r];
+  }
+  return HEDIT_OK;
+}
+
 int hedit_unet_forward_shared(hedit_unet* h, const float* x, int D, const int* row_latent, float t, const float* ctx, int B,
                               int height, int width, const hedit_p2p_plan* plan, float* eps_out, void* workspace,
                               size_t workspace_bytes, void* stream) try {
   TRY(forward_checks(h, x, ctx, B, height, width, plan, eps_out, workspace));
-  ARG_CHECK(row_latent && D >= 1 && D <= 65535, "row map");
-  if (B > HEDIT_ROWMAP_MAX) {
-    hedit_set_error("batch larger than " + std::to_string(HEDIT_ROWMAP_MAX) + " rows (the row map of shared latents)");
-    return HEDIT_ERR_ARG;
-  }
-  ARG_CHECK(reinterpret_cast<uintptr_t>(x) % 16 == 0, "x must be 16-byte aligned");
   RowMap map{};
-  for (int r = 0; r < B; ++r) {
-    ARG_CHECK(row_latent[r] >= 0 && row_latent[r] < D, "row_latent entries must lie in [0, D)");
-    map.src[r] = (uint16_t)row_latent[r];
-  }
+  TRY(row_map_checks(x, D, row_latent, B, &map));
   return forward_impl(h, x, t, ctx, B, height, width, plan, eps_out, workspace, workspace_bytes,
                       reinterpret_cast<hipStream_t>(stream), false, nullptr, D, &map);
+} catch (...) { return hedit_abi_catch(); }
+
+int hedit_unet_context_create(hedit_unet* h, const float* ctx, int B, void* stream, hedit_unet_context** out) try {
+  ARG_CHECK(h && ctx && out, "null");
+  ARG_CHECK(B >= 1, "B");
+  TRY(store_require_loaded(h, "UNet"));
+  hipStream_t st = reinterpret_cast<hipStream_t>(stream);
+  hipStreamCaptureStatus cap = hipStreamCaptureStatusNone;
+  HIP_TRY(hipStreamIsCapturing(st, &cap));
+  if (cap != hipStreamCaptureStatusNone) {
+    hedit_set_error("hedit_unet_context_create allocates: not while the stream is capturing");
+    return HEDIT_ERR_STATE;
+  }
+  Fwd f;
+  f.h = h; f.B = B; f.st = st; f.plan = nullptr;
+  f.ar.dry = true;
+  TRY(project_context(f, nullptr));
+  const size_t bytes = f.ar.peak;
+  void* buf = nullptr;
+  if (hipMalloc(&buf, bytes) != hipSuccess) {
+    (void)hipGetLastError();
+    hedit_set_error("hedit_unet_context_create: out of device memory (" + std::to_string(bytes) + " bytes)");
+    return HEDIT_ERR_HIP;
+  }
+  Fwd g;
+  g.h = h; g.B = B; g.st = st; g.plan = nullptr;
+  g.ar.base = reinterpret_cast<char*>(buf); g.ar.cap = bytes;
+  const int rc = project_context(g, ctx);
+  if (rc != HEDIT_OK) {
+    (void)hipFree(buf);
+    return rc;
+  }
+  hedit_unet_context* cx = new hedit_unet_context();
+  cx->owner = h; cx->B = B; cx->buf = buf;
+  cx->ctxb = g.ctxb; cx->k2_all = g.k2_all; cx->vt2_all = g.vt2_all;
+  *out = cx;
+  return HEDIT_OK;
+} catch (...) { return hedit_abi_catch(); }
+
+void hedit_unet_context_destroy(hedit_unet_context* cx) try {
+  if (!cx) return;
+  (void)hipFree(cx->buf);
+  delete cx;
+} catch (...) { (void)hedit_abi_catch(); }
+
+static int context_checks(const hedit_unet* h, const hedit_unet_context* cx, int B) {
+  ARG_CHECK(cx, "null context");
+  ARG_CHECK(cx->owner == h, "the context was created on another UNet handle");
+  ARG_CHECK(cx->B == B, "the context was created for another number of rows");
+  ARG_CHECK(!h->hook, "an attention hook takes the fp32 context rows (hedit_unet_forward)");
+  return HEDIT_OK;
+}
+
+int hedit_unet_forward_bound(hedit_unet* h, const float* x, float t, const hedit_unet_context* cx, int B, int height, int width,
+                             const hedit_p2p_plan* plan, float* eps_out, void* workspace, size_t workspace_bytes,
+                             void* stream) try {
+  TRY(forward_checks(h, x, cx, B, height, width, plan, eps_out, workspace));
+  TRY(context_checks(h, cx, B));
+  return forward_impl(h, x, t, nullptr, B, height, width, plan, eps_out, workspace, workspace_bytes,
+                      reinterpret_cast<hipStream_t>(stream), false, nullptr, 0, nullptr, cx);
+} catch (...) { return hedit_abi_catch(); }
+
+int hedit_unet_forward_shared_bound(hedit_unet* h, const float* x, int D, const int* row_latent, float t,
+                                    const hedit_unet_context* cx, int B, int height, int width, const hedit_p2p_plan* plan,
+                                    float* eps_out, void* workspace, size_t workspace_bytes, void* stream) try {
+  TRY(forward_checks(h, x, cx, B, height, width, plan, eps_out, workspace));
+  TRY(context_checks(h, cx, B));
+  RowMap map{};
+  TRY(row_map_checks(x, D, row_latent, B, &map));
+  return forward_impl(h, x, t, nullptr, B, height, width, plan, eps_out, workspace, workspace_bytes,
+                      reinterpret_cast<hipStream_t>(stream), false, nullptr, D, &map, cx);
 } catch (...) { return hedit_abi_catch(); }
 
 size_t hedit_unet_grad_workspace_bytes(hedit_unet* h, int B, int height, int width) try {
diff --git a/h-edit_amd/hedit/_lib.py b/h-edit_amd/hedit/_lib.py
--- a/h-edit_amd/hedit/_lib.py
+++ b/h-edit_amd/hedit/_lib.py
@@ -86,6 +86,13 @@
                                      C.c_void_p]),
     "hedit_unet_forward_shared": (C.c_int, [C.c_void_p, C.c_void_p, C.c_int, C.POINTER(C.c_int), C.c_float, C.c_void_p, C.c_int,
                                             C.c_int, C.c_int, C.POINTER(P2PPlan), C.c_void_p, C.c_void_p, C.c_size_t, C.c_void_p]),
+    "hedit_unet_context_create": (C.c_int, [C.c_void_p, C.c_void_p, C.c_int, C.c_void_p, C.POINTER(C.c_void_p)]),
+    "hedit_unet_context_destroy": (None, [C.c_void_p]),
+    "hedit_unet_forward_bound": (C.c_int, [C.c_void_p, C.c_void_p, C.c_float, C.c_void_p, C.c_int, C.c_int,
+                                           C.c_int, C.POINTER(P2PPlan), C.c_void_p, C.c_void_p, C.c_size_t,
+                                           C.c_void_p]),
+    "hedit_unet_forward_shared_bound": (C.c_int, [C.c_void_p, C.c_void_p, C.c_int, C.POINTER(C.c_int), C.c_float, C.c_void_p, C.c_int,
+                                                  C.c_int, C.c_int, C.POINTER(P2PPlan), C.c_void_p, C.c_void_p, C.c_size_t, C.c_void_p]),
     "hedit_unet_create_grad": (C.c_int, [C.POINTER(UnetCfg), C.POINTER(C.c_void_p)]),
     "hedit_unet_grad_workspace_bytes": (C.c_size_t, [C.c_void_p, C.c_int, C.c_int, C.c_int]),
     "hedit_unet_forward_keep": (C.c_int, [C.c_void_p, C.c_void_p, C.c_float, C.c_void_p, C.c_int, C.c_int, C.c_int, C.c_void_p,
diff --git a/h-edit_amd/hedit/engine.py b/h-edit_amd/hedit/engine.py
--- a/h-edit_amd/hedit/engine.py
+++ b/h-edit_amd/hedit/engine.py
@@ -56,6 +56,8 @@
 
 
 class HEditEngine:
+    _bind_contexts = True
+
     def __init__(self, model, share_latents=True):
         self.model = model
         self.share_latents = share_latents
@@ -223,6 +225,16 @@
 
         share = self.share_latents
 
+        row_sets = {"base4": ctx_base4, "base2": ctx_base2, "edit": ctx_edit, "src": ctx_src, "edit5": ctx_edit5}
+        bound = {}
+
+        def rows_of(name):
+            if foreign or not self._bind_contexts:
+                return row_sets[name]
+            if name not in bound:
+                bound[name] = self.unet.make_context(row_sets[name])
+            return bound[name]
+
         def unet_rows(parts, blocks, t, ctx_rows, plan=None):
             if not share:
                 return self.unet.forward_raw(torch.cat([parts[b] for b in blocks]), t, ctx_rows, plan)
@@ -234,78 +246,82 @@
             if foreign:
                 return self.unet.forward_hooked(torch.cat([parts[b] for b in blocks]), t, ctx_edit, controller, save)
             plan = controller._plan(self.unet, rows, xT.shape[2], xT.shape[3], save) if controller is not None else None
-            e = unet_rows(parts, blocks, t, ctx_edit5 if rows == 5 * n else ctx_edit, plan)
+            e = unet_rows(parts, blocks, t, rows_of("edit5" if rows == 5 * n else "edit"), plan)
             if controller is not None:
                 controller._after_pass(save)
             return e
 
-        carry = None
-        reuse = reuse_orig_eps and p2p and implicit
-        for i, t in enumerate(op):
-            idx = T - i - (T - after_skip_steps + 1)
-            z = zs[idx] if zs is not None else None
-            tt = op[i + 1] if i < len(op) - 1 else 0
-            eta_i = float(eta[idx]) if isinstance(eta, (list, tuple)) else float(eta)
-            coef = S.step_coef(t, tt, eta_i, ddim_inv, cfg_scales, w_rec)
-
-            if (not p2p) and implicit and i == 0 and ahead != -1:
-                xe = xt[n:]
-                e = unet_rows([xe], (0, 0, 0, 0), t, ctx_edit, off)
-                c0 = S.step_coef(t, tt, eta_i, ddim_inv, cfg_scales, w_rec, coeff=S.edit_coeff(ahead, t, eta_i, ddim_inv))
-                new = torch.empty_like(xe)
-                self.step_update(e[0:n], e[2 * n:3 * n], e[n:2 * n], e[3 * n:], xe, xe, new, n, False, c0)
-                xt = torch.cat([xt[:n], new]).contiguous()
-
-            if p2p and reuse and carry is not None:
-                e2 = unet_rows([xt[n:]], (0, 0), t, ctx_base2, off)
-                e = torch.cat([carry[0], e2[:n], carry[1], e2[n:]])
-                self.step_base(e, xt, z, x_prev, n, 4, coef)
-            elif p2p:
-                e = unet_rows([xt[:n], xt[n:]], (0, 1, 0, 1), t, ctx_base4, off)
-                self.step_base(e, xt, z, x_prev, n, 4, coef)
-            else:
-                e = unet_rows([xt[n:]], (0, 0), t, ctx_base2, off)
-                self.step_base(e, xt, z, x_prev, n, 2, coef)
-            x_orig, x_base = x_prev[:n], x_prev[n:]
-
-            if not implicit:
-                new = torch.empty_like(x_base)
-                if p2p:
-                    e_src = self.unet.forward_raw(xt[n:].contiguous(), t, ctx_src, off)
-                    e = p2p_pass([xt[:n], xt[n:]], (0, 1, 0, 1), t, True)
-                    self.step_update(e[n:2 * n], e_src, e[n:2 * n], e[3 * n:], x_base, x_base, new, n, False, coef)
+        try:
+            carry = None
+            reuse = reuse_orig_eps and p2p and implicit
+            for i, t in enumerate(op):
+                idx = T - i - (T - after_skip_steps + 1)
+                z = zs[idx] if zs is not None else None
+                tt = op[i + 1] if i < len(op) - 1 else 0
+                eta_i = float(eta[idx]) if isinstance(eta, (list, tuple)) else float(eta)
+                coef = S.step_coef(t, tt, eta_i, ddim_inv, cfg_scales, w_rec)
+
+                if (not p2p) and implicit and i == 0 and ahead != -1:
+                    xe = xt[n:]
+                    e = unet_rows([xe], (0, 0, 0, 0), t, rows_of("edit"), off)
+                    c0 = S.step_coef(t, tt, eta_i, ddim_inv, cfg_scales, w_rec, coeff=S.edit_coeff(ahead, t, eta_i, ddim_inv))
+                    new = torch.empty_like(xe)
+                    self.step_update(e[0:n], e[2 * n:3 * n], e[n:2 * n], e[3 * n:], xe, xe, new, n, False, c0)
+                    xt = torch.cat([xt[:n], new]).contiguous()
+
+                if p2p and reuse and carry is not None:
+                    e2 = unet_rows([xt[n:]], (0, 0), t, rows_of("base2"), off)
+                    e = torch.cat([carry[0], e2[:n], carry[1], e2[n:]])
+                    self.step_base(e, xt, z, x_prev, n, 4, coef)
+                elif p2p:
+                    e = unet_rows([xt[:n], xt[n:]], (0, 1, 0, 1), t, rows_of("base4"), off)
+                    self.step_base(e, xt, z, x_prev, n, 4, coef)
                 else:
-                    e = unet_rows([xt[n:]], (0, 0, 0, 0), t, ctx_edit, off)
-                    self.step_update(e[0:n], e[2 * n:3 * n], e[n:2 * n], e[3 * n:], x_base, x_base, new, n, False, coef)
-                x_k = new
-            else:
-                x_k = x_base.clone()
-                for k in range(K):
-                    new = torch.empty_like(x_k)
+                    e = unet_rows([xt[n:]], (0, 0), t, rows_of("base2"), off)
+                    self.step_base(e, xt, z, x_prev, n, 2, coef)
+                x_orig, x_base = x_prev[:n], x_prev[n:]
+
+                if not implicit:
+                    new = torch.empty_like(x_base)
                     if p2p:
-                        save = not (k < K - 1 and K > 1)
-                        if fuse_src_pass:
-                            e = p2p_pass([x_orig, x_k], (0, 1, 0, 1, 1), tt, save)
-                            e_src = e[4 * n:]
+                        e_src = self.unet.forward_raw(xt[n:].contiguous(), t, rows_of("src"), off)
+                        e = p2p_pass([xt[:n], xt[n:]], (0, 1, 0, 1), t, True)
+                        self.step_update(e[n:2 * n], e_src, e[n:2 * n], e[3 * n:], x_base, x_base, new, n, False, coef)
+                    else:
+                        e = unet_rows([xt[n:]], (0, 0, 0, 0), t, rows_of("edit"), off)
+                        self.step_update(e[0:n], e[2 * n:3 * n], e[n:2 * n], e[3 * n:], x_base, x_base, new, n, False, coef)
+                    x_k = new
+                else:
+                    x_k = x_base.clone()
+                    for k in range(K):
+                        new = torch.empty_like(x_k)
+                        if p2p:
+                            save = not (k < K - 1 and K > 1)
+                            if fuse_src_pass:
+                                e = p2p_pass([x_orig, x_k], (0, 1, 0, 1, 1), tt, save)
+                                e_src = e[4 * n:]
+                            else:
+                                e_src = self.unet.forward_raw(x_k, tt, rows_of("src"), off)
+                                e = p2p_pass([x_orig, x_k], (0, 1, 0, 1), tt, save)
+                            self.step_update(e[n:2 * n], e_src, e[n:2 * n], e[3 * n:4 * n], x_k, x_base, new, n,
+                                             k > 0 and style is None and rec_pull, coef)
+                            if style is not None and style[0] is not None:
+                                with torch.enable_grad():
+                                    new = self.style_step(e[n:2 * n], e_src, e[n:2 * n], e[3 * n:4 * n], new, tt, cfg_scales,
+                                                          style[0], style[1])
+                            if reuse:
+                                carry = (e[0:n], e[2 * n:3 * n])
                         else:
-                            e_src = self.unet.forward_raw(x_k, tt, ctx_src, off)
-                            e = p2p_pass([x_orig, x_k], (0, 1, 0, 1), tt, save)
-                        self.step_update(e[n:2 * n], e_src, e[n:2 * n], e[3 * n:4 * n], x_k, x_base, new, n,
-                                         k > 0 and style is None and rec_pull, coef)
-                        if style is not None and style[0] is not None:
-                            with torch.enable_grad():
-                                new = self.style_step(e[n:2 * n], e_src, e[n:2 * n], e[3 * n:4 * n], new, tt, cfg_scales,
-                                                      style[0], style[1])
-                        if reuse:
-                            carry = (e[0:n], e[2 * n:3 * n])
-                    else:
-                        e = unet_rows([x_k], (0, 0, 0, 0), tt, ctx_edit, off)
-                        self.step_update(e[0:n], e[2 * n:3 * n], e[n:2 * n], e[3 * n:], x_k, x_base, new, n, k > 0, coef)
-                    x_k = new
-
-            xt = torch.cat([x_orig, x_k]).contiguous()
-            if step_cb is not None:
-                xt = step_cb(xt)
+                            e = unet_rows([x_k], (0, 0, 0, 0), tt, rows_of("edit"), off)
+                            self.step_update(e[0:n], e[2 * n:3 * n], e[n:2 * n], e[3 * n:], x_k, x_base, new, n, k > 0, coef)
+                        x_k = new
+
+                xt = torch.cat([x_orig, x_k]).contiguous()
+                if step_cb is not None:
+                    xt = step_cb(xt)
+        finally:
+            for cx in bound.values():
+                cx.close()
         return xt[n:].clone(), xt[:n].clone()
 
     @torch.no_grad()
diff --git a/h-edit_amd/hedit/unet.py b/h-edit_amd/hedit/unet.py
--- a/h-edit_amd/hedit/unet.py
+++ b/h-edit_amd/hedit/unet.py
@@ -5,6 +5,7 @@
 import torch
 
 from . import _lib
+from . import native
 from .native import NativeOwner
 
 SD15_CONFIG = dict(in_channels=4, out_channels=4, sample_size=64,
@@ -79,6 +80,25 @@
             elif want_x:
                 _lib.check(m._lib.hedit_unet_backward(m._h, _lib.ptr(g), _lib.ptr(dx), _lib.ptr(m._gws), _lib.cur_stream()))
         return dx, dc, None, None
+
+
+class UNetContext(NativeOwner):
+    _family, _finalizes = "unet_context", False
+
+    def __init__(self, model, ctx):
+        rows, _, dim = ctx.shape
+        if ctx.dtype != torch.float32 or ctx.shape != (rows, 77, model.config["cross_attention_dim"]):
+            raise ValueError(f"the context rows must be float32 (B, 77, {model.config['cross_attention_dim']}), got "
+                             f"{ctx.dtype} {tuple(ctx.shape)}")
+        ctx = ctx.detach().to(model.device).contiguous()
+        lib, h = model._lib, C.c_void_p()
+        with native._device_ctx(model.device):
+            _lib.check(lib.hedit_unet_context_create(model._h, _lib.ptr(ctx), rows, _lib.cur_stream(), C.byref(h)))
+            native._sync_stream()
+        self.rows = rows
+        self._h, self._lib, self._h_device = h, lib, model.device
+
+    close = NativeOwner._native_release
 
 
 class UNet2DConditionModel(NativeOwner):
@@ -225,30 +245,42 @@
         _lib.check(self._lib.hedit_prof_records(self._h, rows.ctypes.data_as(C.POINTER(C.c_double)), max_rows, C.byref(n)))
         return rows[:n.value]
 
+    def make_context(self, ctx_rows):
+        return UNetContext(self, ctx_rows)
+
     def forward_raw(self, sample, t, ctx, plan=None, out=None, row_latent=None):
         B, Cc, H, W = sample.shape
         if row_latent is not None:
             B = len(row_latent)
-        if sample.dtype != torch.float32 or ctx.dtype != torch.float32:
+        bound = isinstance(ctx, UNetContext)
+        if sample.dtype != torch.float32 or (not bound and ctx.dtype != torch.float32):
             raise TypeError("sample and encoder_hidden_states must be float32")
-        if ctx.shape != (B, 77, self.config["cross_attention_dim"]):
-            raise ValueError(f"encoder_hidden_states must be ({B}, 77, {self.config['cross_attention_dim']}), "
-                             f"got {tuple(ctx.shape)}")
+        if bound:
+            if ctx._h is None:
+                raise _lib.HipError("the UNetContext was closed")
+            ctx_arg = ctx._h
+        else:
+            if ctx.shape != (B, 77, self.config["cross_attention_dim"]):
+                raise ValueError(f"encoder_hidden_states must be ({B}, 77, {self.config['cross_attention_dim']}), "
+                                 f"got {tuple(ctx.shape)}")
+            ctx = ctx.contiguous()
+            ctx_arg = _lib.ptr(ctx)
         sample = sample.contiguous()
-        ctx = ctx.contiguous()
         if out is None:
             out = torch.empty(B, self.config["out_channels"], H, W, dtype=torch.float32, device=sample.device)
         ws = self._workspace(B, H, W)
         if row_latent is None:
-            _lib.check(self._lib.hedit_unet_forward(
-                self._h, _lib.ptr(sample), C.c_float(float(t)), _lib.ptr(ctx), B, H, W,
+            fwd = self._lib.hedit_unet_forward_bound if bound else self._lib.hedit_unet_forward
+            _lib.check(fwd(
+                self._h, _lib.ptr(sample), C.c_float(float(t)), ctx_arg, B, H, W,
                 C.byref(plan) if plan is not None else None, _lib.ptr(out), _lib.ptr(ws), ws.numel(),
                 _lib.cur_stream()))
             return out
         if sample.data_ptr() % 16:
             sample = sample.clone()
-        _lib.check(self._lib.hedit_unet_forward_shared(
-            self._h, _lib.ptr(sample), sample.shape[0], (C.c_int * B)(*row_latent), C.c_float(float(t)), _lib.ptr(ctx), B, H, W,
+        fwd = self._lib.hedit_unet_forward_shared_bound if bound else self._lib.hedit_unet_forward_shared
+        _lib.check(fwd(
+            self._h, _lib.ptr(sample), sample.shape[0], (C.c_int * B)(*row_latent), C.c_float(float(t)), ctx_arg, B, H, W,
             C.byref(plan) if plan is not None else None, _lib.ptr(out), _lib.ptr(ws), ws.numel(),
             _lib.cur_stream()))
         return out
diff --git a/include/hedit.h b/include/hedit.h
--- a/include/hedit.h
+++ b/include/hedit.h
@@ -67,6 +67,14 @@
 int hedit_unet_forward_shared(hedit_unet* h, const float* x, int D, const int* row_latent, float t, const float* ctx, int B,
                               int height, int width, const hedit_p2p_plan* plan, float* eps_out, void* workspace,
                               size_t workspace_bytes, void* stream);
+typedef struct hedit_unet_context hedit_unet_context;
+int hedit_unet_context_create(hedit_unet* h, const float* ctx, int B, void* stream, hedit_unet_context** out);
+void hedit_unet_context_destroy(hedit_unet_context* cx);
+int hedit_unet_forward_bound(hedit_unet* h, const float* x, float t, const hedit_unet_context* cx, int B, int height, int width,
+                             const hedit_p2p_plan* plan, float* eps_out, void* workspace, size_t workspace_bytes, void* stream);
+int hedit_unet_forward_shared_bound(hedit_unet* h, const float* x, int D, const int* row_latent, float t,
+                                    const hedit_unet_context* cx, int B, int height, int width, const hedit_p2p_plan* plan,
+                                    float* eps_out, void* workspace, size_t workspace_bytes, void* stream);
 typedef int (*hedit_attn_hook_fn)(void* user, float* probs, int batch_heads, int n_query, int n_key, int is_cross, int place,
                                   int layer, void* stream);
 int hedit_unet_set_attn_hook(hedit_unet* h, hedit_attn_hook_fn fn, void* user);
```

Measured after the change: 2.707 (median of 6 runs). 1.1% higher.
